# jlko/STOVE

Measured on AMD Instinct MI355X. Metric: frames/s (fwd+bwd) for 3-obj billiards 32x32 T=100, 1/2/4/8 GPU; ELBO delta vs ref, higher is better.
Workload: dtype f32 (encoder GEMMs: fp32 products as 3 sixteen-bit MFMAs on hi/lo-split operands -- half pieces forward, bf16 pieces backward -- fp32 accumulate)

## Files before the change

### include/stove_hip.h

```cpp
#ifndef STOVE_HIP_H
#define STOVE_HIP_H
#include <stddef.h>
#include <stdint.h>

#ifdef __cplusplus
extern "C" {
#endif

int stove_abi_version(void);
const char* stove_error_string(int code);

typedef struct StoveSpnTables {
  const int32_t* obj_scope;
  const int32_t* obj_leaf_slot;
  const float* obj_coef;
  const float* obj_wsum;
  const float* obj_wroot;
  const int32_t* bg_side;
  const float* bg_coef;
  const float* bg_wroot;
  const float* bg_dense;
} StoveSpnTables;

size_t stove_bg_dense_floats(void);
// ... 16 lines not shown

size_t stove_bgspn_saved_floats(int n);
int stove_bgspn_fwd(const StoveSpnTables* t, const float* inputs, const float* marg, float* ell, float* out,
                    int n, void* stream);
size_t stove_bgspn_bwd_ws_bytes(int n);
int stove_bgspn_bwd(const StoveSpnTables* t, const float* inputs, const float* marg, const float* ell, const float* out,
                    const float* dout, float* d_inputs, float* d_marg, StoveSpnTableGrads* g, void* ws, int n,
                    void* stream);

size_t stove_bgspn_saved_floats_d(int n, int n_pix);
int stove_bgspn_fwd_d(const StoveSpnTables* t, const float* inputs, const float* marg, float* ell, float* out, int n, int n_pix, void* stream);
size_t stove_bgspn_bwd_ws_bytes_d(int n, int n_pix);
int stove_bgspn_bwd_d(const StoveSpnTables* t, const float* inputs, const float* marg, const float* ell, const float* out, const float* dout,
                      float* d_inputs, float* d_marg, StoveSpnTableGrads* g, void* ws, int n, int n_pix, void* stream);

size_t stove_scene_saved_floats(int n_frames, int n_obj);
size_t stove_scene_fwd_floats(int n_frames, int n_obj, int with_grad);
int stove_scene_fwd(const StoveSpnTables* t, const float* frames, const float* z, int n_frames, int n_obj, int seq_frames,
                    int seq_stride, float overlap_beta, float* ll, float* parts, float* saved, void* stream);
size_t stove_scene_bwd_ws_bytes(int n_frames, int n_obj);
int stove_scene_bwd(const StoveSpnTables* t, const float* frames, const float* z, int n_frames, int n_obj, int seq_frames,
                    int seq_stride, float overlap_beta, const float* saved, const float* dll, float* dz, StoveSpnTableGrads* g,
                    void* ws, void* stream);
int stove_scene_bwd_overlap(const StoveSpnTables* t, const float* frames, const float* z, int n_frames, int n_obj, int seq_frames,
                    int seq_stride, float overlap_beta, const float* saved, const float* dll, float* dz, StoveSpnTableGrads* g,
                    void* ws, void* stream, void* param_stream);
size_t stove_objspn_saved_floats_any(int n, int R, int G, int S, int D, int Lmax);
size_t stove_objspn_bwd_ws_bytes_any(int n, int R, int G, int S, int D, int Lmax);
int stove_objspn_fwd_any(const float* inputs, const float* marg, const int* lscope, const float* coef, const float* wsum,
                         const float* wroot, float* saved, float* out, int n, int R, int G, int S, int D, int Lmax, void* stream);
int stove_objspn_bwd_any(const float* inputs, const float* marg, const int* lscope, const int* slot, const float* coef,
                         const float* wsum, const float* wroot, const float* saved, const float* dout, float* d_inputs,
                         float* d_marg, float* g_coef, float* g_wsum, float* g_wroot, void* ws, int n, int R, int G, int S, int D,
                         int Lmax, void* stream);
int stove_gauss_ll_fwd(const float* x, const float* marg, float* out, int n, int d, float mean, float scale, void* stream);
int stove_gauss_ll_bwd(const float* x, const float* marg, const float* dout, float* dx, float* dm, int n, int d, float mean, float scale,
                       void* stream);
size_t stove_scene_saved_floats_any(int n_frames, int n_obj, int n_pix, int with_grad);
size_t stove_scene_bwd_ws_bytes_any(int n_frames, int n_obj, int n_pix);
int stove_scene_fwd_any(const StoveSpnTables* t, const float* frames, const float* z, int n_frames, int n_obj, int seq_frames,
                        int seq_stride, int W, int H, int align_corners, float overlap_beta, float* ll, float* parts, float* saved,
                        void* stream, int with_grad);
int stove_scene_bwd_any(const StoveSpnTables* t, const float* frames, const float* z, int n_frames, int n_obj, int seq_frames,
                        int seq_stride, int W, int H, int align_corners, float overlap_beta, const float* saved, const float* dll,
                        float* dz, StoveSpnTableGrads* g, void* ws, void* stream, void* param_stream);
size_t stove_scene_saved_floats_ch(int n_frames, int n_obj, int channels, int W, int H, int R, int G, int S, int D, int Lmax, int with_grad);
size_t stove_scene_bwd_ws_bytes_ch(int n_frames, int n_obj, int channels, int W, int H, int R, int G, int S, int D, int Lmax);
int stove_scene_fwd_ch(const int32_t* lscope, const int32_t* slot, const float* coef, const float* wsum, const float* wroot, int R, int G, int S,
                       int D, int Lmax, const int32_t* bg_side, const float* bg_coef, const float* bg_wroot, size_t bg_coef_floats,
                       const float* frames, const float* z, int n_frames, int n_obj, int seq_frames, int seq_stride, int channels, int W, int H,
                       int pw, int ph, int align_corners, float overlap_beta, float* ll, float* parts, float* saved, void* stream, int with_grad);
int stove_scene_bwd_ch(const int32_t* lscope, const int32_t* slot, const float* coef, const float* wsum, const float* wroot, int R, int G, int S,
                       int D, int Lmax, const int32_t* bg_side, const float* bg_coef, const float* bg_wroot, size_t bg_coef_floats,
                       const float* frames, const float* z, int n_frames, int n_obj, int seq_frames, int seq_stride, int channels, int W, int H,
                       int pw, int ph, int align_corners, float overlap_beta, const float* saved, const float* dll, float* dz, float* g_coef,
                       float* g_wsum, float* g_wroot, float* g_bg_coef, float* g_bg_wroot, void* ws, void* stream, void* param_stream);
int stove_scene_fwd_from(const StoveSpnTables* t, const float* frames, const float* z, int n_frames, int n_obj, int seq_frames,
                         int seq_stride, float overlap_beta, float* ll, float* parts, float* saved, void* stream, void* fork_from,
                         int with_grad);
int stove_scene_bwd_from(const StoveSpnTables* t, const float* frames, const float* z, int n_frames, int n_obj, int seq_frames,
                         int seq_stride, float overlap_beta, const float* saved, const float* dll, float* dz,
                         StoveSpnTableGrads* g, void* ws, void* stream, void* param_stream, void* fork_from);

int stove_glimpse_mean(const float* x_color, const float* z, float* emb, int n_frames, int n_obj, int channels, void* stream);

int stove_objspn_mpe(const StoveSpnTables* t, const float* leaf_means, const float* inputs, float* xw, float* out,
                     int32_t* pick, int n, void* stream);

int stove_render_frames(const float* bg, const float* patches, int frames_per_patch, const float* z, float* out, int n_frames,
                        int n_obj, void* stream);

int stove_scene_glimpses(const float* frames, const float* z, int n_frames, int n_obj, float* tile,
                         float* patches, float* keep, void* stream);

size_t stove_gnn_param_floats(void);
size_t stove_gnn_grad_floats(void);
int stove_gnn_blocks(int B, int N);
int stove_gnn_fwd(const float* s_in, const float* params, float* result, float* pred, int B, int N, int sin_dim,
                  int lim_enc, int elu, void* stream);
size_t stove_gnn_bwd_ws_bytes(int B, int N);
int stove_gnn_bwd(const float* s_in, const float* params, const float* d_result, const float* d_pred, float* d_s_in,
                  float* g_params, void* ws, int B, int N, int sin_dim, int lim_enc, int elu, void* stream);

int stove_gnn_debug_stamps(const float* s_in, const float* params, const float* d_result, float* d_s_in, void* ws,
                           long long* stamps, int B, int N, int sin_dim, int lim_enc, int elu, void* stream);

size_t stove_dynloop_act_floats(int B, int Ts, int N);
int stove_dynloop_fwd(const float* z1, const float* zsup, const float* zsstd, const float* eps, const float* extra,
                      const float* params, float* z, float* zdyn, float* zdstd, float* mean, float* std_, float* pred,
                      float* act, int B, int Ts, int N, int sin_dim, int lim_enc, int elu, float pos_var, float vel_std, float lat_std,
                      void* stream);
size_t stove_dynloop_bwd_ws_bytes(int B, int N);
size_t stove_dynloop_bwd_ws_bytes_ts(int B, int Ts, int N);
int stove_dynloop_bwd(const float* z1, const float* zsup, const float* zsstd, const float* eps, const float* extra,
                      const float* params, const float* z, const float* act, const float* dz, const float* dzdyn,
                      const float* dmean, const float* dstd, const float* dpred, float* dz1, float* dzsup, float* dzsstd, float* dextra,
                      float* g_params, void* ws, int B, int Ts, int N, int sin_dim, int lim_enc, int elu, float pos_var,
                      float vel_std, float lat_std, void* stream);

int stove_dynloop_bwd_overlap(const float* z1, const float* zsup, const float* zsstd, const float* eps, const float* extra,
                              const float* params, const float* z, const float* act, const float* dz, const float* dzdyn,
                              const float* dmean, const float* dstd, const float* dpred, float* dz1, float* dzsup, float* dzsstd,
                              float* dextra, float* g_params, void* ws, int B, int Ts, int N, int sin_dim, int lim_enc, int elu,
                              float pos_var, float vel_std, float lat_std, void* stream, void* param_stream);


size_t stove_reward_head_param_floats(void);
size_t stove_reward_head_saved_floats(int items, int n_obj);
size_t stove_reward_head_bwd_ws_floats(int items);
int stove_reward_head_fwd(const float* pred, const float* params, float* reward, float* saved, int items, int n_obj, void* stream);
int stove_reward_head_bwd(const float* pred, const float* params, const float* reward, const float* saved, const float* d_reward, float* d_pred,
                          float* g_params, float* ws, int items, int n_obj, void* stream);

int stove_small_linear(const float* x, const float* W, const float* b, float* y, int rows, int in_dim, int out_dim, int w_transposed, void* stream);

int stove_rollout_fwd(const float* z_last, const float* extra, const float* params, float* z_pred, float* zstd, float* pred,
                      int B, int num, int A, int N, int sin_dim, int lim_enc, int elu, float pos_var, float vel_std,
                      float lat_std, void* stream);

size_t stove_gnn_param_floats_cl(int cl);
size_t stove_gnn_grad_floats_cl(int cl);
size_t stove_gnn_bwd_ws_bytes_cl(int cl, int B, int N);
int stove_gnn_fwd_cl(const float* s_in, const float* params, float* result, float* pred, int cl, int B, int N, int sin_dim,
                     int lim_enc, int elu, void* stream);
int stove_gnn_bwd_cl(const float* s_in, const float* params, const float* d_result, const float* d_pred, float* d_s_in,
                     float* g_params, void* ws, int cl, int B, int N, int sin_dim, int lim_enc, int elu, void* stream);
int stove_dynloop_fwd_cl(const float* z1, const float* zsup, const float* zsstd, const float* eps, const float* extra,
                         const float* params, float* z, float* zdyn, float* zdstd, float* mean, float* std_, float* pred,
                         int cl, int B, int Ts, int N, int sin_dim, int lim_enc, int elu, float pos_var, float vel_std, float lat_std,
                         void* stream);
int stove_dynloop_bwd_cl(const float* z1, const float* zsup, const float* zsstd, const float* eps, const float* extra,
                         const float* params, const float* z, const float* dz, const float* dzdyn, const float* dmean,
                         const float* dstd, const float* dpred, float* dz1, float* dzsup, float* dzsstd, float* dextra,
                         float* g_params, void* ws, int cl, int B, int Ts, int N, int sin_dim, int lim_enc, int elu, float pos_var,
                         float vel_std, float lat_std, void* stream);
int stove_rollout_fwd_cl(const float* z_last, const float* extra, const float* params, float* z_pred, float* zstd, float* pred,
                         int cl, int B, int num, int A, int N, int sin_dim, int lim_enc, int elu, float pos_var, float vel_std,
                         float lat_std, void* stream);

int stove_match_objects(const float* feat, long long* idx, float* perm, int B, int T, int N, int F, int mode, void* stream);

int stove_supair_state_fwd(const float* codes, const float* span_low, float* zc, float* pos, long long* idx, float* zfix,
                           unsigned char* hits, float* zl, float* sl, float* init6, int n, int T, int o, int skip, int fix,
                           int mode, void* stream);
int stove_supair_state_bwd(const float* zc, const long long* idx, const unsigned char* hits, const float* zfix, const float* g_zfix,
                           const float* g_zl, const float* g_sl, const float* g_init6, const float* span_low, float* gfix_ws,
                           float* g_codes, int n, int T, int o, int skip, void* stream);
int stove_supair_state_fwd2(const float* codes, const float* span_low, float* zc, float* pos, long long* idx, float* zfix,
                            unsigned char* hits, float* zl, float* sl, float* init, int init_ld, const float* lat_noise, int lat_dim,
                            int n, int T, int o, int skip, int fix, int mode, void* stream);
int stove_supair_state_bwd2(const float* zc, const long long* idx, const unsigned char* hits, const float* zfix, const float* g_zfix,
                            const float* g_zl, const float* g_sl, const float* g_init6, int init_ld, const float* span_low, float* gfix_ws,
                            float* g_codes, int n, int T, int o, int skip, void* stream);
int stove_zall_fwd(const float* zfix, const float* zs, float* zall, int n, int T, int o, int skip, void* stream);
int stove_zall_bwd(const float* zfix, const float* zs, const float* g_zall, const float* dz_in, float* g_zfix, float* g_zs, int n, int T, int o,
                   int skip, void* stream);
int stove_elbo_fwd(const float* zs, const float* mean, const float* std_, const float* zdyn, const float* lik, const float* trans_std16,
                   float* part_ws, float* out3, int n, int T, int o, int skip, void* stream);
int stove_elbo_bwd(const float* zs, const float* mean, const float* std_, const float* zdyn, const float* trans_std16, const float* g_out,
                   float* g_zs, float* g_mean, float* g_std, float* g_zdyn, float* g_lik, int n, int T, int o, int skip, void* stream);

void stove_debug_set_stamps(long long* device_buffer);

typedef struct StoveSpnArenaPlan {
  const int32_t* obj_mu;
  const int32_t* obj_rho;
  const int32_t* obj_sum;
  const int32_t* bg_mu;
  const int32_t* bg_rho;
  const int32_t* bg_gidx;
  int32_t obj_root, bg_root;
  float obj_vmin, obj_vmax, bg_vmin, bg_vmax;
} StoveSpnArenaPlan;
int stove_spn_bake(const float* arena, const StoveSpnArenaPlan* plan, float* obj_coef, float* obj_wsum, float* obj_wroot,
                   float* bg_coef, float* bg_wroot, void* stream);
int stove_spn_bake_bwd(const float* arena, const StoveSpnArenaPlan* plan, const StoveSpnTableGrads* g, float* grad_arena, void* stream);
int stove_arena_gather(const float* arena, const int32_t* src, float* image, int n, void* stream);
int stove_arena_scatter_add(const float* gimage, const int32_t* src, float* grad_arena, int n, void* stream);

int stove_sum_chunks(const float* parts, float* out, size_t n, int chunks, void* stream);

int stove_set_fork_stream(int device, void* stream, int restore_default);
int stove_set_overlap(int on);
int stove_set_tile_lds(int mode);
void* stove_event_list_begin(void);
int stove_event_list_end(void* list);
int stove_event_list_destroy(void* list);
int stove_stream_after(void* to, void* from);
int stove_capture_begin(void* stream);
int stove_capture_end(void* stream, void** graph_out, int* n_nodes);
int stove_graph_instantiate(void* graph, void** exec_out);
int stove_graph_launch(void* exec, void* stream);
int stove_graph_destroy(void* exec);

int stove_noise_normal(float* out, size_t n, unsigned long long* state, void* stream);

int stove_bw_transform(const float* x, float* out, int n_frames, int channels, int pixels, void* stream);
int stove_bw_transform_u8(const unsigned char* x, float* out, int n_frames, int channels, int pixels, void* stream);

size_t stove_colsum_ws_floats(int rows, int cols);
int stove_colsum(const float* a, float* out, float* ws, int rows, int cols, void* stream);
size_t stove_small_tn_ws_floats(int rows, int M, int N);
int stove_small_tn(const float* a, const float* b, float* out, float* ws, int rows, int M, int N, void* stream);
int stove_colsum2(const float* a, float* out, float* out2, int accumulate, float* ws, int rows, int cols, void* stream);

size_t stove_flat_adam_ws_bytes(int nseg);
int stove_flat_adam(float* params, const float* grads, float* exp_avg, float* exp_avg_sq, float* max_exp_avg_sq, size_t numel,
                    const int* seg_of4, const unsigned char* seg_trainable, float* seg_steps, int nseg, void* ws, float* grad_norm_out,
                    const float* hyper_dev, float lr, float beta1, float beta2, float eps, float max_norm, int clip, void* stream);

size_t stove_gemm_bf16_ws_floats(int M, int N, int splitk);
int stove_gemm_bf16(const float* A, const float* B, const float* bias, const float* add, float* C, int M, int N, int K, int lda, int ldb, int ldc,
                    int a_kmajor, int b_kmajor, int nsplit, int splitk, int tile, float* ws, void* stream);

int stove_lstm_cell_fwd(const float* gx, const float* gh, const float* c_prev, float* c, float* h, int n, int H, int fast, void* stream);
int stove_lstm_cell_bwd(const float* gx, const float* gh, const float* c_prev, const float* c, const float* dh,
                        const float* dc_in, float* dg, float* dc_out, float* dgx_sum, const float* dg_more, int n_more, int n, int H,
                        int fast, void* stream);
int stove_enc_head_fwd(const float* h, const float* W1, const float* b1, const float* W2, const float* b2, float* h1, float* codes, int rows,
                       int H, int HID, int OUT, int frames, int fc1_split, void* stream);
size_t stove_enc_head_bwd_ws_floats(int rows, int HID);
int stove_enc_head_bwd(const float* dcodes, const float* h1, const float* h, const float* W1, const float* W2, float* gh, float* gW1,
                       float* gb1, float* gW2, float* gb2, int accumulate, float* ws, int rows, int H, int HID, int OUT, int frames, void* stream);

void stove_profile_enable(int on);
size_t stove_profile_report(char* buf, size_t cap);

int stove_fill_words(void* p, uint32_t value, size_t n_words, void* stream);

int stove_selftest_wave_sum(const float* in, float* out, int n_waves, void* stream);

#ifdef __cplusplus
}
#endif
#endif
```

### stove_amd/_lib.py

```python
import ctypes
import os
from ctypes import POINTER, Structure, c_char_p, c_float, c_int, c_size_t, c_void_p

import torch

_HERE = os.path.dirname(os.path.abspath(__file__))
from . import settings as _settings

LIB_PATH = _settings.LIB_OVERRIDE or os.path.join(_HERE, 'libstove_hip.so')
_lib = None
ABI_VERSION = 7

class SpnTables(Structure):
    _fields_ = [('obj_scope', c_void_p), ('obj_leaf_slot', c_void_p), ('obj_coef', c_void_p),
                ('obj_wsum', c_void_p), ('obj_wroot', c_void_p),
                ('bg_side', c_void_p), ('bg_coef', c_void_p), ('bg_wroot', c_void_p), ('bg_dense', c_void_p)]


class SpnTableGrads(Structure):
    _fields_ = [('obj_coef', c_void_p), ('obj_wsum', c_void_p), ('obj_wroot', c_void_p),
                ('bg_coef', c_void_p), ('bg_wroot', c_void_p)]


class SpnArenaPlan(Structure):
    _fields_ = [('obj_mu', c_void_p), ('obj_rho', c_void_p), ('obj_sum', c_void_p),
                ('bg_mu', c_void_p), ('bg_rho', c_void_p), ('bg_gidx', c_void_p),
                ('obj_root', c_int), ('bg_root', c_int),
                ('obj_vmin', c_float), ('obj_vmax', c_float), ('bg_vmin', c_float), ('bg_vmax', c_float)]


def _declare(lib):
    P, I, F, S = c_void_p, c_int, c_float, c_size_t
    T, G = POINTER(SpnTables), POINTER(SpnTableGrads)
    A = POINTER(SpnArenaPlan)
    sig = {
        'stove_abi_version': (I, []),
        'stove_error_string': (c_char_p, [I]),
        'stove_selftest_wave_sum': (I, [P, P, I, P]),
        'stove_objspn_tile_floats': (S, [I]),
        'stove_objspn_fwd': (I, [T, P, P, P, P, I, P]),
        'stove_objspn_bwd_ws_bytes': (S, [I]),
        'stove_objspn_bwd': (I, [T, P, P, P, P, P, P, G, P, I, P]),
        'stove_bgspn_saved_floats': (S, [I]),
        'stove_bgspn_fwd': (I, [T, P, P, P, P, I, P]),
        'stove_bgspn_bwd_ws_bytes': (S, [I]),
        'stove_bgspn_bwd': (I, [T, P, P, P, P, P, P, P, G, P, I, P]),
        'stove_scene_saved_floats': (S, [I, I]),
        'stove_scene_fwd': (I, [T, P, P, I, I, I, I, F, P, P, P, P]),
        'stove_scene_fwd_from': (I, [T, P, P, I, I, I, I, F, P, P, P, P, P, I]),
        'stove_scene_fwd_floats': (S, [I, I, I]),
        'stove_scene_bwd_from': (I, [T, P, P, I, I, I, I, F, P, P, P, G, P, P, P, P]),
        'stove_scene_bwd_ws_bytes': (S, [I, I]),
        'stove_scene_bwd': (I, [T, P, P, I, I, I, I, F, P, P, P, G, P, P]),
        'stove_scene_bwd_overlap': (I, [T, P, P, I, I, I, I, F, P, P, P, G, P, P, P]),
        'stove_gauss_ll_fwd': (I, [P, P, P, I, I, F, F, P]),
        'stove_gauss_ll_bwd': (I, [P, P, P, P, P, I, I, F, F, P]),
        'stove_objspn_saved_floats_any': (S, [I, I, I, I, I, I]),
        'stove_objspn_bwd_ws_bytes_any': (S, [I, I, I, I, I, I]),
        'stove_objspn_fwd_any': (I, [P, P, P, P, P, P, P, P, I, I, I, I, I, I, P]),
        'stove_objspn_bwd_any': (I, [P, P, P, P, P, P, P, P, P, P, P, P, P, P, P, I, I, I, I, I, I, P]),
        'stove_scene_saved_floats_any': (S, [I, I, I, I]),
        'stove_scene_bwd_ws_bytes_any': (S, [I, I, I]),
        'stove_scene_fwd_any': (I, [T, P, P, I, I, I, I, I, I, I, F, P, P, P, P, I]),
        'stove_scene_bwd_any': (I, [T, P, P, I, I, I, I, I, I, I, F, P, P, P, G, P, P, P]),
        'stove_scene_saved_floats_ch': (S, [I] * 11),
        'stove_scene_bwd_ws_bytes_ch': (S, [I] * 10),
        'stove_scene_fwd_ch': (I, [P] * 5 + [I] * 5 + [P, P, P, S, P, P] + [I] * 10 + [F, P, P, P, P, I]),
        'stove_scene_bwd_ch': (I, [P] * 5 + [I] * 5 + [P, P, P, S, P, P] + [I] * 10 + [F] + [P] * 11),
        'stove_scene_glimpses': (I, [P, P, I, I, P, P, P, P]),
        'stove_gnn_param_floats': (S, []),
        'stove_gnn_grad_floats': (S, []),
        'stove_gnn_blocks': (I, [I, I]),
        'stove_gnn_fwd': (I, [P, P, P, P, I, I, I, I, I, P]),
        'stove_gnn_bwd_ws_bytes': (S, [I, I]),
        'stove_gnn_bwd': (I, [P, P, P, P, P, P, P, I, I, I, I, I, P]),
        'stove_dynloop_act_floats': (S, [I, I, I]),
        'stove_dynloop_fwd': (I, [P] * 13 + [I] * 6 + [F] * 3 + [P]),
        'stove_dynloop_bwd_ws_bytes': (S, [I, I]),
        'stove_dynloop_bwd': (I, [P] * 19 + [I] * 6 + [F] * 3 + [P]),
        'stove_dynloop_bwd_overlap': (I, [P] * 19 + [I] * 6 + [F] * 3 + [P, P]),
        'stove_rollout_fwd': (I, [P] * 6 + [I] * 7 + [F] * 3 + [P]),
        'stove_gnn_param_floats_cl': (S, [I]),
        'stove_gnn_grad_floats_cl': (S, [I]),
        'stove_gnn_bwd_ws_bytes_cl': (S, [I, I, I]),
        'stove_gnn_fwd_cl': (I, [P, P, P, P, I, I, I, I, I, I, P]),
        'stove_gnn_bwd_cl': (I, [P, P, P, P, P, P, P, I, I, I, I, I, I, P]),
        'stove_dynloop_fwd_cl': (I, [P] * 12 + [I] * 7 + [F] * 3 + [P]),
        'stove_dynloop_bwd_cl': (I, [P] * 18 + [I] * 7 + [F] * 3 + [P]),
        'stove_rollout_fwd_cl': (I, [P] * 6 + [I] * 8 + [F] * 3 + [P]),
        'stove_match_objects': (I, [P, P, P, I, I, I, I, I, P]),
        'stove_profile_enable': (None, [I]),
        'stove_lstm_cell_fwd': (I, [P, P, P, P, P, I, I, I, P]),
        'stove_lstm_cell_bwd': (I, [P] * 10 + [I, I, I, I, P]),
        'stove_gnn_debug_stamps': (I, [P, P, P, P, P, P, I, I, I, I, I, P]),
        'stove_profile_report': (S, [c_char_p, S]),
        'stove_spn_bake': (I, [P, A, P, P, P, P, P, P]),
        'stove_spn_bake_bwd': (I, [P, A, G, P, P]),
        'stove_debug_set_stamps': (None, [P]),
        'stove_glimpse_mean': (I, [P, P, P, I, I, I, P]),
        'stove_objspn_mpe': (I, [T, P, P, P, P, P, I, P]),
        'stove_render_frames': (I, [P, P, I, P, P, I, I, P]),
        'stove_enc_head_fwd': (I, [P, P, P, P, P, P, P, I, I, I, I, I, I, P]),
        'stove_enc_head_bwd_ws_floats': (S, [I, I]),
        'stove_enc_head_bwd': (I, [P, P, P, P, P, P, P, P, P, P, I, P, I, I, I, I, I, P]),
        'stove_colsum2': (I, [P, P, P, I, P, I, I, P]),
        'stove_small_tn_ws_floats': (S, [I, I, I]),
        'stove_small_tn': (I, [P, P, P, P, I, I, I, P]),
        'stove_dynloop_bwd_ws_bytes_ts': (S, [I, I, I]),
        'stove_bw_transform': (I, [P, P, I, I, I, P]),
        'stove_bw_transform_u8': (I, [P, P, I, I, I, P]),
        'stove_stream_after': (I, [P, P]),
        'stove_small_linear': (I, [P, P, P, P, I, I, I, I, P]),
        'stove_reward_head_param_floats': (S, []),
        'stove_reward_head_saved_floats': (S, [I, I]),
        'stove_reward_head_bwd_ws_floats': (S, [I]),
        'stove_reward_head_fwd': (I, [P, P, P, P, I, I, P]),
        'stove_reward_head_bwd': (I, [P] * 8 + [I, I, P]),
        'stove_set_fork_stream': (I, [I, P, I]),
        'stove_noise_normal': (I, [P, S, P, P]),
        'stove_bgspn_saved_floats_d': (S, [I, I]),
        'stove_bgspn_fwd_d': (I, [T, P, P, P, P, I, I, P]),
        'stove_bgspn_bwd_ws_bytes_d': (S, [I, I]),
        'stove_bgspn_bwd_d': (I, [T, P, P, P, P, P, P, P, G, P, I, I, P]),
        'stove_set_overlap': (I, [I]),
        'stove_set_tile_lds': (I, [I]),
        'stove_event_list_begin': (P, []),
        'stove_event_list_end': (I, [P]),
        'stove_event_list_destroy': (I, [P]),
        'stove_fill_words': (I, [P, ctypes.c_uint32, S, P]),
        'stove_capture_begin': (I, [P]),
        'stove_capture_end': (I, [P, POINTER(c_void_p), POINTER(c_int)]),
        'stove_graph_instantiate': (I, [P, POINTER(c_void_p)]),
        'stove_graph_launch': (I, [P, P]),
        'stove_graph_destroy': (I, [P]),
        'stove_colsum_ws_floats': (S, [I, I]),
        'stove_colsum': (I, [P, P, P, I, I, P]),
        'stove_sum_chunks': (I, [P, P, S, I, P]),
        'stove_flat_adam_ws_bytes': (S, [I]),
        'stove_gemm_bf16_ws_floats': (S, [I, I, I]),
        'stove_gemm_bf16': (I, [P, P, P, P, P] + [I] * 11 + [P, P]),
        'stove_flat_adam': (I, [P] * 5 + [S, P, P, P, I, P, P, P, F, F, F, F, F, I, P]),
        'stove_supair_state_fwd': (I, [P] * 10 + [I] * 6 + [P]),
        'stove_supair_state_bwd': (I, [P] * 11 + [I] * 4 + [P]),
        'stove_bg_dense_floats': (S, []),
        'stove_bg_dense': (I, [P, P, P, P]),
        'stove_supair_state_fwd2': (I, [P] * 10 + [I, P, I] + [I] * 6 + [P]),
        'stove_supair_state_bwd2': (I, [P] * 8 + [I] + [P] * 3 + [I] * 4 + [P]),
        'stove_zall_fwd': (I, [P, P, P, I, I, I, I, P]),
        'stove_zall_bwd': (I, [P, P, P, P, P, P, I, I, I, I, P]),
        'stove_elbo_fwd': (I, [P] * 8 + [I] * 4 + [P]),
        'stove_elbo_bwd': (I, [P] * 11 + [I] * 4 + [P]),
        'stove_arena_gather': (I, [P, P, P, I, P]),
        'stove_arena_scatter_add': (I, [P, P, P, I, P]),
    }
    for name, (res, args) in sig.items():
        fn = getattr(lib, name)
        fn.restype = res
        fn.argtypes = args


def load():
    global _lib
    if _lib is None:
        if not os.path.exists(LIB_PATH):
            raise RuntimeError(
                f'{LIB_PATH} is missing: build it with `python -m stove_amd.build` '
                '(hipcc --offload-arch=gfx950). stove_amd has no CPU fallback.')
        lib = ctypes.CDLL(LIB_PATH)
        _declare(lib)
        if lib.stove_abi_version() != ABI_VERSION:
            raise RuntimeError(f'{LIB_PATH} has ABI version {lib.stove_abi_version()}, this binding needs {ABI_VERSION}: '
                               'rebuild it with `python -m stove_amd.build --force`')
        from . import settings
        lib.stove_set_overlap(1 if settings.OVERLAP else 0)
        if settings.LIB_OVERRIDE:
            import sys
            sys.stderr.write('[stove_amd] STOVE_LIB: loaded %s\n' % LIB_PATH)
        _lib = lib
    return _lib


def check(code, what):
    if code != 0:
        msg = load().stove_error_string(code)
        raise RuntimeError(f'{what} failed: hipError {code} ({msg.decode() if msg else "?"})')


def ptr(t):
    if t is None:
        return None
    if not t.is_cuda:
        raise RuntimeError('stove_amd HIP ops need tensors on a GPU (cuda:N); there is no CPU path')
    if not t.is_contiguous():
        raise RuntimeError('stove_amd HIP ops need contiguous tensors')
    return t.data_ptr()


_FORCED_STREAM = None


def stream():
    return _FORCED_STREAM if _FORCED_STREAM is not None else torch.cuda.current_stream().cuda_stream


def force_stream(handle):
    global _FORCED_STREAM
    prev, _FORCED_STREAM = _FORCED_STREAM, handle
    return prev


def profile_report(wall=False):
    lib = load()
    buf = ctypes.create_string_buffer(1 << 16)
    lib.stove_profile_report(buf, len(buf))
    out = {}
    for line in buf.value.decode().splitlines():
        name, ms, cnt, cover = line.split('\t')
        name = name.strip('()').split('<')[0].split('::')[-1]
        tot, c, w = out.get(name, (0.0, 0, 0.0))
        out[name] = (tot + float(ms), c + int(cnt), w + float(cover))
    return out if wall else {k: v[:2] for k, v in out.items()}
```

### stove_amd/arena.py

```python
import ctypes

import torch
import torch.distributed as dist

from . import _lib, ops
from . import settings as _settings


def _unique_params(module):
    seen, out = set(), []
    for name, p in module.named_parameters():
        if id(p) not in seen:
            seen.add(id(p))
            out.append((name, p))
    return out


class ParamArena:
    ALIGN = 4

    def __init__(self, model, world_size=None):
        named = _unique_params(model)
        if not named:
            raise ValueError('model has no parameters')
        dev, dt = named[0][1].device, named[0][1].dtype
        for n, p in named:
            if p.device != dev or p.dtype != dt:
                raise ValueError('parameter %s is %s/%s, arena is %s/%s' % (n, p.device, p.dtype, dev, dt))
        self.model = model
        self.names = [n for n, _ in named]
        self.params = [p for _, p in named]
        self.offset, off = {}, 0
        for p in self.params:
            self.offset[id(p)] = off
            off += (p.numel() + self.ALIGN - 1) // self.ALIGN * self.ALIGN
        self.numel = off
        self.data = torch.zeros(off, dtype=dt, device=dev)
        self.grad = torch.zeros(off, dtype=dt, device=dev)
        with torch.no_grad():
            for p in self.params:
                o, n = self.offset[id(p)], p.numel()
                self.data[o:o + n].copy_(p.data.reshape(-1))
                p.data = self.data[o:o + n].view(p.shape)
        self._on_gpu_params = dev.type == 'cuda' and dt == torch.float32
        self._bind_grads()
        if world_size is None:
            world_size = dist.get_world_size() if dist.is_initialized() else 1
        self.world_size = world_size
        self._spn = self._gnn = None
        sup = model if hasattr(model, 'obj_spn') else getattr(model, 'sup', None)
        dyn = model if hasattr(model, 'param_image') else getattr(model, 'dyn', None)
        self._on_gpu = dev.type == 'cuda' and dt == torch.float32
        if sup is not None and hasattr(sup, 'obj_spn'):
            self._plan_spn(sup)
            sup._arena = self
        if dyn is not None and hasattr(dyn, 'param_image'):
            self._plan_gnn(dyn)
            dyn._arena = self

    def _bind_grads(self):
        for p in self.params:
            if not p.requires_grad:
                p.grad = None
                if self._on_gpu_params:
                    ops.register_grad_view(p, None)
                continue
            o, n = self.offset[id(p)], p.numel()
            g = p.grad
            if g is None or g.data_ptr() != self.grad.data_ptr() + self.grad.element_size() * o:
                p.grad = self.grad[o:o + n].view(p.shape)
            if self._on_gpu_params:
                ops.register_grad_view(p, p.grad)

    def view_of(self, p, flat=None):
        o = self.offset[id(p)]
        return (self.data if flat is None else flat)[o:o + p.numel()].view(p.shape)

    def check(self):
        es = self.data.element_size()
        for p in (self.params[0], self.params[-1]):
            o = self.offset[id(p)]
            if p.data_ptr() != self.data.data_ptr() + es * o:
                raise RuntimeError('ParamArena: parameter storage was rebound (model.to()/type() after the arena '
                                   'was built?) -- build a new ParamArena')
            if p.requires_grad and (p.grad is None or p.grad.data_ptr() != self.grad.data_ptr() + es * o):
                raise RuntimeError('ParamArena: gradient views were detached -- use arena.zero_grad() instead of '
                                   'optimizer.zero_grad() / p.grad = None')

    def zero_grad(self):
        self.grad.zero_()
        self._bind_grads()

    def drop_prefetched(self):
        self._pre = None

    zero = zero_grad

    def pack(self):
        return self.grad

    def all_reduce(self, force=False):
        if self.world_size <= 1 and not force:
            return
        dist.all_reduce(self.grad, op=dist.ReduceOp.SUM)
        if self.world_size > 1:
            self.grad.div_(self.world_size)

    def sync(self, src=0):
        if self.world_size > 1:
            dist.broadcast(self.data, src)
        self.drop_prefetched()

    def clip_grad_norm_(self, max_norm):
        total = torch.linalg.vector_norm(self.grad)
        self.grad.mul_(torch.clamp(max_norm / (total + 1e-6), max=1.0))
        return total

    def _plan_spn(self, sup):
        obj, bg = sup.obj_spn, sup.bg_spn
        if obj._kind != 'obj' or bg._kind != 'bg' or bg.num_dims != 1024:
            return
        dev = self.data.device
        off = self.offset
        oleaves, osums = list(obj.vector_list[0]), list(obj.vector_list[2])
        lo, so = obj._plan_cpu['leaf_order'].tolist(), obj._plan_cpu['sum_order'].tolist()
        bleaves = list(bg.vector_list[0])

        def i32(v):
            return torch.tensor(v, dtype=torch.int32, device=dev)
        t = {'obj_mu': i32([off[id(oleaves[i].means)] for i in lo]),
             'obj_rho': i32([off[id(oleaves[i].sigma_params)] for i in lo]),
             'obj_sum': i32([off[id(osums[i].params)] for i in so]),
             'bg_mu': i32([off[id(v.means)] for v in bleaves]),
             'bg_rho': i32([off[id(v.sigma_params)] for v in bleaves]),
             'bg_gidx': bg._plan_cpu['gidx'].to(torch.int32).reshape(-1).to(dev)}
        plan = _lib.SpnArenaPlan()
        for k, v in t.items():
            setattr(plan, k, v.data_ptr())
        plan.obj_root = off[id(obj.output_vector.params)]
        plan.bg_root = off[id(bg.output_vector.params)]
        plan.obj_vmin, plan.obj_vmax = obj.args.gauss_min_sigma, obj.args.gauss_max_sigma
        plan.bg_vmin, plan.bg_vmax = bg.args.gauss_min_sigma, bg.args.gauss_max_sigma
        opl, bpl = obj._plan(dev), bg._plan(dev)
        self._spn = {'plan': plan, 'keep': t, 'ints': (opl['scope'], opl['leaf_slot'], bpl['side']),
                     'params': list(obj.parameters()) + list(bg.parameters())}

    @property
    def has_spn(self):
        return self._on_gpu and self._spn is not None

    def prefetch_images(self, cores=(0,)):
        if not self._on_gpu or not _settings.OVERLAP:
            return
        dev = self.data.device
        main, side = torch.cuda.current_stream(dev), ops._side_stream(dev, 'pre')
        side.wait_stream(main)
        with torch.cuda.stream(side):
            pre = {}
            if self.has_spn:
                pre['spn'] = self._bake_spn()
            if self.has_gnn:
                for k in cores:
                    pre[('gnn', k)] = self._gather_gnn(k)
            ev = torch.cuda.Event()
            ev.record(side)
        self._pre = (pre, ev, side)

    def _take(self, key):
        pre = getattr(self, '_pre', None)
        if pre is None or key not in pre[0]:
            return None
        out = pre[0].pop(key)
        torch.cuda.current_stream(self.data.device).wait_event(pre[1])
        for t in (out if isinstance(out, tuple) else (out,)):
            t.record_stream(torch.cuda.current_stream(self.data.device))
        return out

    def spn_tables(self):
        self.check()
        bufs = self._take('spn')
        if bufs is None:
            bufs = self._bake_spn()
        oc, ow, orr, bc, bw, dense = bufs
        scope, slot, side = self._spn['ints']
        return ((oc.view(24, 25, 10, 3), ow.view(12, 100, 10), orr.view(6, 100), scope, slot),
                (bc.view(3, 1024, 6, 3), bw.view(3, 36), side, dense))

    def _bake_spn(self):
        lib = _lib.load()
        dev = self.data.device
        with torch.cuda.device(dev):
            buf = torch.empty(18000 + 12000 + 600 + 55296 + 108, dtype=torch.float32, device=dev)
            oc, ow, orr, bc, bw = torch.split(buf, [18000, 12000, 600, 55296, 108])
            _lib.check(lib.stove_spn_bake(self.data.data_ptr(), ctypes.byref(self._spn['plan']), oc.data_ptr(), ow.data_ptr(),
                                          orr.data_ptr(), bc.data_ptr(), bw.data_ptr(), _lib.stream()), 'stove_spn_bake')
            dense = torch.empty(lib.stove_bg_dense_floats(), dtype=torch.float32, device=dev)
            _lib.check(lib.stove_bg_dense(self._spn['ints'][2].data_ptr(), bc.data_ptr(), dense.data_ptr(), _lib.stream()), 'stove_bg_dense')
        return oc, ow, orr, bc, bw, dense

    def spn_sink(self, grads):
        req = [p.requires_grad for p in self._spn['params']]
        if not any(req):
            return
        if not all(req):
            raise RuntimeError('ParamArena: the SPN parameters must be frozen or trainable together')
        self.check()
        lib = _lib.load()
        g = _lib.SpnTableGrads()
        g.obj_coef, g.obj_wsum, g.obj_wroot, g.bg_coef, g.bg_wroot = [x.data_ptr() for x in grads]
        with torch.cuda.device(self.data.device):
            _lib.check(lib.stove_spn_bake_bwd(self.data.data_ptr(), ctypes.byref(self._spn['plan']), ctypes.byref(g),
                                              self.grad.data_ptr(), _lib.stream()), 'stove_spn_bake_bwd')

    def _plan_gnn(self, dyn):
        dev = self.data.device

        def index_of(p):
            return (self.offset[id(p)] + torch.arange(p.numel(), dtype=torch.float64)).view(p.shape)
        self._gnn = {}
        for k in range(3):
            w, v, wt = dyn.param_image(k, leaf=index_of, pad_value=-1.0)
            if dyn.c.cl == 32:
                pf, pt = ops.gnn_pack_perms(torch.device('cpu'))
                image = torch.cat([w, wt, v, w[pf], wt[pt]])
            else:
                image = torch.cat([w, wt, v])
            self._gnn[k] = (image.to(torch.int32).to(dev), torch.cat([w, v]).to(torch.int32).to(dev))
        self._gnn_params = [p for n, p in dyn.named_parameters()
                            if n.split('.')[0] in ('state_enc', 'self_cores', 'rel_cores', 'att_net', 'affector', 'out')]

    @property
    def has_gnn(self):
        return self._on_gpu and self._gnn is not None

    def gnn_image(self, core_idx=0):
        self.check()
        img = self._take(('gnn', core_idx))
        return img if img is not None else self._gather_gnn(core_idx)

    def _gather_gnn(self, core_idx):
        lib = _lib.load()
        src = self._gnn[core_idx][0]
        with torch.cuda.device(self.data.device):
            img = torch.empty(src.numel(), dtype=torch.float32, device=self.data.device)
            _lib.check(lib.stove_arena_gather(self.data.data_ptr(), src.data_ptr(), img.data_ptr(), src.numel(), _lib.stream()),
                       'stove_arena_gather')
        return img

    def gnn_sink(self, g, core_idx=0):
        req = [p.requires_grad for p in self._gnn_params]
        if not any(req):
            return
        if not all(req):
            raise RuntimeError('ParamArena: the GNN core parameters must be frozen or trainable together')
        self.check()
        lib = _lib.load()
        src = self._gnn[core_idx][1]
        with torch.cuda.device(self.data.device):
            _lib.check(lib.stove_arena_scatter_add(g.data_ptr(), src.data_ptr(), self.grad.data_ptr(), src.numel(), _lib.stream()),
                       'stove_arena_scatter_add')
```

### stove_amd/csrc/arena.hip

```cpp
#include "common.h"

namespace stove {

struct SpnArenaPlan {
  const int* obj_mu;
  const int* obj_rho;
  const int* obj_sum;
  const int* bg_mu;
  const int* bg_rho;
  const int* bg_gidx;
  int obj_root, bg_root;
  float obj_vmin, obj_vmax, bg_vmin, bg_vmax;
};

__device__ __forceinline__ void leaf_coef(float mu, float rho, float vmin, float vmax, float* abc) {
  const float v = vmin + (vmax - vmin) * (1.0f / (1.0f + expf(-rho)));
  const float iv = 1.0f / v;
  abc[0] = -0.5f * iv;
  abc[1] = mu * iv;
  abc[2] = -0.5f * mu * mu * iv - 0.5f * logf(6.283185307179586f * v);
}
__device__ __forceinline__ void leaf_coef_bwd(float mu, float rho, float vmin, float vmax, const float* g, float* dmu, float* drho) {
  const float s = 1.0f / (1.0f + expf(-rho));
  const float v = vmin + (vmax - vmin) * s;
  const float iv = 1.0f / v;
  *dmu = g[1] * iv - g[2] * mu * iv;
  const float dv = g[0] * 0.5f * iv * iv - g[1] * mu * iv * iv + g[2] * (0.5f * mu * mu * iv * iv - 0.5f * iv);
  *drho = dv * (vmax - vmin) * s * (1.0f - s);
}

constexpr int kAObjLeaves = 24, kAObjS = 25, kAObjG = 10, kAObjSums = 12, kAObjK = 10;
constexpr int kABgR = 3, kABgPix = 1024, kABgG = 6;
constexpr int kAObjCoef = kAObjLeaves * kAObjS * kAObjG;
constexpr int kABgCoef = kABgR * kABgPix * kABgG;
constexpr int kASoftBlocks = (kAObjSums * kAObjK + 2 + 3) / 4;

__device__ __forceinline__ void softmax_col(const float* __restrict__ p, float* __restrict__ w, int n, int ld) {
  const int lane = lane_id();
  float m = -3.0e38f;
  for (int k = lane; k < n; k += 64) m = fmaxf(m, p[k * ld]);
  for (int o = 32; o > 0; o >>= 1) m = fmaxf(m, __shfl_xor(m, o));
  float s = 0.0f;
  for (int k = lane; k < n; k += 64) s += expf(p[k * ld] - m);
  s = wave_sum(s);
  const float inv = 1.0f / s;
  for (int k = lane; k < n; k += 64) w[k * ld] = expf(p[k * ld] - m) * inv;
}
__device__ __forceinline__ void softmax_col_bwd(const float* __restrict__ p, const float* __restrict__ g, float* __restrict__ dp, int n, int ld) {
  const int lane = lane_id();
  float m = -3.0e38f;
  for (int k = lane; k < n; k += 64) m = fmaxf(m, p[k * ld]);
  for (int o = 32; o > 0; o >>= 1) m = fmaxf(m, __shfl_xor(m, o));
  float s = 0.0f, d = 0.0f;
  for (int k = lane; k < n; k += 64) {
    const float e = expf(p[k * ld] - m);
    s += e;
    d = fmaf(e, g[k * ld], d);
  }
  s = wave_sum(s);
  d = wave_sum(d);
  const float inv = 1.0f / s, dot = d * inv;
  for (int k = lane; k < n; k += 64) dp[k * ld] += expf(p[k * ld] - m) * inv * (g[k * ld] - dot);
}

__global__ __launch_bounds__(256) void spn_bake_k(const float* __restrict__ arena, SpnArenaPlan pl, float* __restrict__ obj_coef,
                                                  float* __restrict__ obj_wsum, float* __restrict__ obj_wroot,
                                                  float* __restrict__ bg_coef, float* __restrict__ bg_wroot, int n_elem_blocks) {
  if ((int)blockIdx.x < n_elem_blocks) {
    const int t = blockIdx.x * 256 + threadIdx.x;
    if (t < kAObjCoef) {
      const int q = t / (kAObjS * kAObjG), rem = t % (kAObjS * kAObjG);
      leaf_coef(arena[pl.obj_mu[q] + rem], arena[pl.obj_rho[q] + rem], pl.obj_vmin, pl.obj_vmax, obj_coef + (size_t)t * 3);
    } else if (t < kAObjCoef + kABgCoef) {
      const int u = t - kAObjCoef;
      const int rp = u / kABgG, g = u % kABgG;
      const int gi = pl.bg_gidx[rp];
      const int leaf = gi >> 9, row = gi & 511;
      leaf_coef(arena[pl.bg_mu[leaf] + row * kABgG + g], arena[pl.bg_rho[leaf] + row * kABgG + g], pl.bg_vmin, pl.bg_vmax,
                bg_coef + (size_t)u * 3);
    }
    return;
  }
  const int col = ((int)blockIdx.x - n_elem_blocks) * 4 + wave_id();
  if (col < kAObjSums * kAObjK + 2) {
    if (col < kAObjSums * kAObjK) {
      const int node = col / kAObjK, s = col % kAObjK;
      softmax_col(arena + pl.obj_sum[node] + s, obj_wsum + (size_t)node * 100 * kAObjK + s, 100, kAObjK);
    } else if (col == kAObjSums * kAObjK) {
      softmax_col(arena + pl.obj_root, obj_wroot, 600, 1);
    } else {
      softmax_col(arena + pl.bg_root, bg_wroot, kABgR * kABgG * kABgG, 1);
    }
  }
}

__global__ __launch_bounds__(256) void spn_bake_bwd_k(const float* __restrict__ arena, SpnArenaPlan pl,
                                                      const float* __restrict__ g_obj_coef, const float* __restrict__ g_obj_wsum,
                                                      const float* __restrict__ g_obj_wroot, const float* __restrict__ g_bg_coef,
                                                      const float* __restrict__ g_bg_wroot, float* __restrict__ garena,
                                                      int n_elem_blocks) {
  if ((int)blockIdx.x < n_elem_blocks) {
    const int t = blockIdx.x * 256 + threadIdx.x;
    if (t < kAObjCoef) {
      const int q = t / (kAObjS * kAObjG), rem = t % (kAObjS * kAObjG);
      float dmu, drho;
      leaf_coef_bwd(arena[pl.obj_mu[q] + rem], arena[pl.obj_rho[q] + rem], pl.obj_vmin, pl.obj_vmax, g_obj_coef + (size_t)t * 3, &dmu, &drho);
      garena[pl.obj_mu[q] + rem] += dmu;
      garena[pl.obj_rho[q] + rem] += drho;
    } else if (t < kAObjCoef + kABgCoef) {
      const int u = t - kAObjCoef;
      const int rp = u / kABgG, g = u % kABgG;
      const int gi = pl.bg_gidx[rp];
      const int leaf = gi >> 9, row = gi & 511;
      const int om = pl.bg_mu[leaf] + row * kABgG + g, orh = pl.bg_rho[leaf] + row * kABgG + g;
      float dmu, drho;
      leaf_coef_bwd(arena[om], arena[orh], pl.bg_vmin, pl.bg_vmax, g_bg_coef + (size_t)u * 3, &dmu, &drho);
      garena[om] += dmu;
      garena[orh] += drho;
    }
    return;
  }
  const int col = ((int)blockIdx.x - n_elem_blocks) * 4 + wave_id();
  if (col < kAObjSums * kAObjK + 2) {
    if (col < kAObjSums * kAObjK) {
      const int node = col / kAObjK, s = col % kAObjK;
      softmax_col_bwd(arena + pl.obj_sum[node] + s, g_obj_wsum + (size_t)node * 100 * kAObjK + s, garena + pl.obj_sum[node] + s, 100, kAObjK);
    } else if (col == kAObjSums * kAObjK) {
      softmax_col_bwd(arena + pl.obj_root, g_obj_wroot, garena + pl.obj_root, 600, 1);
    } else {
      softmax_col_bwd(arena + pl.bg_root, g_bg_wroot, garena + pl.bg_root, kABgR * kABgG * kABgG, 1);
    }
  }
}

__global__ void arena_gather_k(const float* __restrict__ arena, const int* __restrict__ src, float* __restrict__ image, int n) {
  const int i = blockIdx.x * blockDim.x + threadIdx.x;
  if (i < n) image[i] = src[i] >= 0 ? arena[src[i]] : 0.0f;
}
__global__ void arena_scatter_add_k(const float* __restrict__ gimage, const int* __restrict__ src, float* __restrict__ garena, int n) {
  const int i = blockIdx.x * blockDim.x + threadIdx.x;
  if (i < n && src[i] >= 0) garena[src[i]] += gimage[i];
}

}

namespace stove {

struct AdamHyper {
  float lr, b1, b2, eps, max_norm;
};
constexpr int ADAM_SCAN_BLOCKS = 256;

__global__ __launch_bounds__(256) void grad_scan_k(const float* __restrict__ g, const int* __restrict__ seg_of4, int* __restrict__ flags,
                                                   float* __restrict__ part, int n4) {
  float acc = 0.0f;
  for (int i = blockIdx.x * 256 + threadIdx.x; i < n4; i += ADAM_SCAN_BLOCKS * 256) {
    const float4 v = reinterpret_cast<const float4*>(g)[i];
    acc += v.x * v.x + v.y * v.y + v.z * v.z + v.w * v.w;
    if (v.x != 0.0f || v.y != 0.0f || v.z != 0.0f || v.w != 0.0f) flags[seg_of4[i]] = 1;
  }
  __shared__ float red[4];
  acc = wave_sum(acc);
  if ((threadIdx.x & 63) == 0) red[threadIdx.x >> 6] = acc;
  __syncthreads();
  if (threadIdx.x == 0) part[blockIdx.x] = (red[0] + red[1]) + (red[2] + red[3]);
}

__global__ __launch_bounds__(256) void flat_adam_k(float* __restrict__ p, const float* __restrict__ g, float* __restrict__ m, float* __restrict__ v,
                                                   float* __restrict__ vmax, const int* __restrict__ seg_of4,
                                                   const unsigned char* __restrict__ trainable, const float* __restrict__ steps,
                                                   const int* __restrict__ flags, const float* __restrict__ part, float* __restrict__ norm_out,
                                                   const float* __restrict__ hyper_dev, AdamHyper k, int clip, int n4) {
  if (hyper_dev != nullptr) {
    k.lr = hyper_dev[0]; k.b1 = hyper_dev[1]; k.b2 = hyper_dev[2]; k.eps = hyper_dev[3]; k.max_norm = hyper_dev[4];
  }
  __shared__ float s_norm;
  if (threadIdx.x < 64) {
    float t = (part[threadIdx.x] + part[threadIdx.x + 64]) + (part[threadIdx.x + 128] + part[threadIdx.x + 192]);
    t = wave_sum(t);
    if (threadIdx.x == 0) {
      s_norm = sqrtf(t);
      if (blockIdx.x == 0 && norm_out != nullptr) norm_out[0] = s_norm;
    }
  }
  __syncthreads();
  const int i = blockIdx.x * 256 + threadIdx.x;
  if (i >= n4) return;
  const int seg = seg_of4[i];
  if (trainable[seg] == 0 || flags[seg] == 0) return;
  const float coef = clip ? fminf(1.0f, k.max_norm / (s_norm + 1e-6f)) : 1.0f;
  const double t = (double)steps[seg] + 1.0;
  const float bc1 = (float)(1.0 - pow((double)k.b1, t));
  const float sqrt_bc2 = (float)sqrt(1.0 - pow((double)k.b2, t));
  const float4 g4 = reinterpret_cast<const float4*>(g)[i];
  float4 p4 = reinterpret_cast<float4*>(p)[i], m4 = reinterpret_cast<float4*>(m)[i], v4 = reinterpret_cast<float4*>(v)[i];
  float4 x4 = vmax != nullptr ? reinterpret_cast<float4*>(vmax)[i] : v4;
  const float step = k.lr / bc1;
#define STOVE_ADAM1(c)                                           \
  {                                                              \
    const float gg = g4.c * coef;                                \
    m4.c = m4.c + (1.0f - k.b1) * (gg - m4.c);                   \
    v4.c = k.b2 * v4.c + (1.0f - k.b2) * gg * gg;                \
    x4.c = vmax != nullptr ? fmaxf(x4.c, v4.c) : v4.c;           \
    p4.c -= step * m4.c / (sqrtf(x4.c) / sqrt_bc2 + k.eps);      \
  }
  STOVE_ADAM1(x) STOVE_ADAM1(y) STOVE_ADAM1(z) STOVE_ADAM1(w)
#undef STOVE_ADAM1
  reinterpret_cast<float4*>(p)[i] = p4;
  reinterpret_cast<float4*>(m)[i] = m4;
  reinterpret_cast<float4*>(v)[i] = v4;
  if (vmax != nullptr) reinterpret_cast<float4*>(vmax)[i] = x4;
}

__global__ void adam_tick_k(const unsigned char* __restrict__ trainable, float* __restrict__ steps, int* __restrict__ flags, int nseg, int sticky) {
  const int s = blockIdx.x * blockDim.x + threadIdx.x;
  if (s >= nseg) return;
  if (trainable[s] != 0 && flags[s] != 0) steps[s] += 1.0f;
  if (!sticky) flags[s] = 0;
}

__global__ void sum_chunks4_k(const float* __restrict__ part, float* __restrict__ out, int n4, int chunks, int accumulate = 0,
                              const float* __restrict__ bias4 = nullptr, int cols4 = 0, const float* __restrict__ add4 = nullptr) {
  const int i = blockIdx.x * blockDim.x + threadIdx.x;
  if (i >= n4) return;
  float4 a = reinterpret_cast<const float4*>(part)[i];
  if (add4 != nullptr) {
    const float4 b = reinterpret_cast<const float4*>(add4)[i];
    a.x += b.x; a.y += b.y; a.z += b.z; a.w += b.w;
  }
  if (bias4 != nullptr) {
    const float4 b = reinterpret_cast<const float4*>(bias4)[i % cols4];
    a.x += b.x; a.y += b.y; a.z += b.z; a.w += b.w;
  }
  if (accumulate) {
    const float4 o = reinterpret_cast<const float4*>(out)[i];
    a.x += o.x; a.y += o.y; a.z += o.z; a.w += o.w;
  }
  for (int c = 1; c < chunks; ++c) {
    const float4 b = reinterpret_cast<const float4*>(part)[(size_t)c * n4 + i];
    a.x += b.x; a.y += b.y; a.z += b.z; a.w += b.w;
  }
  reinterpret_cast<float4*>(out)[i] = a;
}

__global__ __launch_bounds__(256) void sum_chunks4_par_k(const float* __restrict__ part, float* __restrict__ out, int n4, int chunks, int accumulate) {
  __shared__ float4 red[4][64];
  const int e = threadIdx.x & 63, q = threadIdx.x >> 6;
  const int i = blockIdx.x * 64 + e;
  float4 a = {0.0f, 0.0f, 0.0f, 0.0f};
  if (i < n4)
    for (int c = q; c < chunks; c += 4) {
      const float4 b = reinterpret_cast<const float4*>(part)[(size_t)c * n4 + i];
      a.x += b.x; a.y += b.y; a.z += b.z; a.w += b.w;
    }
  red[q][e] = a;
  __syncthreads();
  if (q == 0 && i < n4) {
    float4 t = red[0][e];
#pragma unroll
    for (int k = 1; k < 4; ++k) {
      t.x += red[k][e].x; t.y += red[k][e].y; t.z += red[k][e].z; t.w += red[k][e].w;
    }
    if (accumulate) {
      const float4 o = reinterpret_cast<const float4*>(out)[i];
      t.x += o.x; t.y += o.y; t.z += o.z; t.w += o.w;
    }
    reinterpret_cast<float4*>(out)[i] = t;
  }
}

__global__ __launch_bounds__(256) void small_tn_part_k(const float* __restrict__ a, const float* __restrict__ b, float* __restrict__ part,
                                                        int rows, int M, int N, int rows_per_chunk) {
  const int t = threadIdx.x;
  if (t >= M * N) return;
  const int m = t / N, n = t % N;
  const int r0 = blockIdx.x * rows_per_chunk;
  const int r1 = r0 + rows_per_chunk < rows ? r0 + rows_per_chunk : rows;
  float s0 = 0.0f, s1 = 0.0f;
  int r = r0;
  for (; r + 1 < r1; r += 2) {
    s0 = fmaf(a[(size_t)r * M + m], b[(size_t)r * N + n], s0);
    s1 = fmaf(a[(size_t)(r + 1) * M + m], b[(size_t)(r + 1) * N + n], s1);
  }
  if (r < r1) s0 = fmaf(a[(size_t)r * M + m], b[(size_t)r * N + n], s0);
  part[(size_t)blockIdx.x * M * N + t] = s0 + s1;
}

__global__ __launch_bounds__(256) void colsum_part_k(const float* __restrict__ a, float* __restrict__ part, int rows, int cols4, int rows_per_chunk) {
  const int c4 = blockIdx.y * 256 + threadIdx.x;
  if (c4 >= cols4) return;
  const int r0 = blockIdx.x * rows_per_chunk;
  const int r1 = r0 + rows_per_chunk < rows ? r0 + rows_per_chunk : rows;
  float4 s0 = {0.0f, 0.0f, 0.0f, 0.0f}, s1 = s0;
  int r = r0;
  for (; r + 1 < r1; r += 2) {
    const float4 u = reinterpret_cast<const float4*>(a)[(size_t)r * cols4 + c4];
    const float4 v = reinterpret_cast<const float4*>(a)[(size_t)(r + 1) * cols4 + c4];
    s0.x += u.x; s0.y += u.y; s0.z += u.z; s0.w += u.w;
    s1.x += v.x; s1.y += v.y; s1.z += v.z; s1.w += v.w;
  }
  if (r < r1) {
    const float4 u = reinterpret_cast<const float4*>(a)[(size_t)r * cols4 + c4];
    s0.x += u.x; s0.y += u.y; s0.z += u.z; s0.w += u.w;
  }
  s0.x += s1.x; s0.y += s1.y; s0.z += s1.z; s0.w += s1.w;
  reinterpret_cast<float4*>(part)[(size_t)blockIdx.x * cols4 + c4] = s0;
}

__global__ __launch_bounds__(256) void colsum_narrow_part_k(const float* __restrict__ a, float* __restrict__ part, int rows, int cols, int cpad,
                                                            int rows_per_chunk) {
  __shared__ float red[256];
  const int c = threadIdx.x % cpad, rr = threadIdx.x / cpad, nslot = 256 / cpad;
  const int r0 = blockIdx.x * rows_per_chunk;
  const int r1 = r0 + rows_per_chunk < rows ? r0 + rows_per_chunk : rows;
  float s = 0.0f;
  if (c < cols)
    for (int r = r0 + rr; r < r1; r += nslot) s += a[(size_t)r * cols + c];
  red[threadIdx.x] = s;
  __syncthreads();
  if (rr == 0 && c < cols) {
    float t = 0.0f;
    for (int q = 0; q < nslot; ++q) t += red[q * cpad + c];
    part[(size_t)blockIdx.x * cols + c] = t;
  }
}

__global__ void bw_transform_k(const float* __restrict__ x, float* __restrict__ out, int N, int C, int P4) {
  const int i = blockIdx.x * blockDim.x + threadIdx.x;
  if (i >= N * P4) return;
  const int n = i / P4, p = i % P4;
  float4 s = reinterpret_cast<const float4*>(x)[((size_t)n * C) * P4 + p];
  for (int c = 1; c < C; ++c) {
    const float4 v = reinterpret_cast<const float4*>(x)[((size_t)n * C + c) * P4 + p];
    s.x += v.x; s.y += v.y; s.z += v.z; s.w += v.w;
  }
  s.x = fminf(fmaxf(s.x, 0.0f), 1.0f);
  s.y = fminf(fmaxf(s.y, 0.0f), 1.0f);
  s.z = fminf(fmaxf(s.z, 0.0f), 1.0f);
  s.w = fminf(fmaxf(s.w, 0.0f), 1.0f);
  reinterpret_cast<float4*>(out)[i] = s;
}

__global__ void bw_transform_u8_k(const unsigned char* __restrict__ x, float* __restrict__ out, int N, int C, int P4) {
  const int i = blockIdx.x * blockDim.x + threadIdx.x;
  if (i >= N * P4) return;
  const int n = i / P4, p = i % P4;
  float4 s = make_float4(0.f, 0.f, 0.f, 0.f);
  for (int c = 0; c < C; ++c) {
    const uchar4 v = reinterpret_cast<const uchar4*>(x)[((size_t)n * C + c) * P4 + p];
    const float4 f = make_float4((float)v.x / 255.0f, (float)v.y / 255.0f, (float)v.z / 255.0f, (float)v.w / 255.0f);
    if (c == 0) s = f;
    else { s.x += f.x; s.y += f.y; s.z += f.z; s.w += f.w; }
  }
  s.x = fminf(fmaxf(s.x, 0.0f), 1.0f);
  s.y = fminf(fmaxf(s.y, 0.0f), 1.0f);
  s.z = fminf(fmaxf(s.z, 0.0f), 1.0f);
  s.w = fminf(fmaxf(s.w, 0.0f), 1.0f);
  reinterpret_cast<float4*>(out)[i] = s;
}

}
```

### stove_amd/csrc/capi.hip

```cpp
#include "../../include/stove_hip.h"
#include <algorithm>

#include "common.h"
#include <string.h>
#include <stdlib.h>
#include <math.h>
#include <atomic>
#include <type_traits>
#include "validate.h"
static_assert(stove_validate::kStoveInvalidValue == (int)hipErrorInvalidValue, "validate.h returns hipErrorInvalidValue");
#define STOVE_VALIDATE(expr)                      \
  do {                                            \
    const int v__ = stove_validate::expr;         \
    if (v__) return v__;                          \
  } while (0)
#include "spn_obj.hip"
#include "spn_obj_generic.hip"
#include "spn_bg.hip"
#include "spn_bg_generic.hip"
#include "scene.hip"
#include "scene_fused.hip"
#include "scene_colour.hip"
#include "gnn.hip"
#include "match.hip"
// ... 931 lines not shown
#define STOVE_ROLL_LAUNCH(ELU_)                         \
  do {                                                  \
    if (N == 3) STOVE_ROLL_LAUNCH_N(4, ELU_, 3);        \
    else if (N <= 4) STOVE_ROLL_LAUNCH_N(4, ELU_, 0);   \
    else STOVE_ROLL_LAUNCH_N(6, ELU_, 0);               \
  } while (0)
    if (elu) STOVE_ROLL_LAUNCH(true);
    else STOVE_ROLL_LAUNCH(false);
#undef STOVE_ROLL_LAUNCH
#undef STOVE_ROLL_LAUNCH_N
    STOVE_LAUNCH_CHECK();
    return 0;
  }
  int rc = gnn_lds_attr((const void*)rollout_fwd_k);
  if (rc) return rc;
  STOVE_LAUNCH(rollout_fwd_k, dim3(stove_gnn_blocks(B, N)), dim3(256), kGnnLdsFloats * sizeof(float), (hipStream_t)stream,
                     z_last, extra, params, z_pred, zstd, pred, B, num, A < 1 ? 1 : A, N, gnn_group_for(B, N), sin_dim, lim_enc, elu, kc);
  STOVE_LAUNCH_CHECK();
  return 0;
}

size_t stove_gnn_param_floats_cl(int cl) { return cl == 16 ? GC<16>::kParams : (cl == 64 ? GC<64>::kParams : 0); }
size_t stove_gnn_grad_floats_cl(int cl) { return cl == 16 ? GC<16>::kGrads : (cl == 64 ? GC<64>::kGrads : 0); }
size_t stove_gnn_bwd_ws_bytes_cl(int cl, int B, int N) {
  if (B < 1 || N < 1 || N > 6) return 0;
  if (cl == 16) return (size_t)cl_blocks<16>(B, N) * GC<16>::kGrads * sizeof(float);
  if (cl == 64) return (size_t)cl_blocks<64>(B, N) * GC<64>::kGrads * sizeof(float);
  return 0;
}

int stove_gnn_fwd_cl(const float* s_in, const float* params, float* result, float* pred, int cl, int B, int N, int sin_dim,
                     int lim_enc, int elu, void* stream) {
  STOVE_VALIDATE(gnn_fwd_cl(s_in, params, result, cl, B, N, sin_dim));
  if (B == 0) return 0;
  return with_cl(cl, [&](auto w) {
    constexpr int CL = decltype(w)::value;
    int rc = cl_lds_attr<CL>((const void*)gnn_cl_step_fwd_k<CL>);
    if (rc) return rc;
    STOVE_LAUNCH(gnn_cl_step_fwd_k<CL>, dim3(cl_blocks<CL>(B, N)), dim3(256), GC<CL>::kLdsFloats * sizeof(float), (hipStream_t)stream,
                 s_in, params, result, pred, B, N, cl_group_for<CL>(B, N), sin_dim, lim_enc, elu);
    STOVE_LAUNCH_CHECK();
    return 0;
  });
}

int stove_gnn_bwd_cl(const float* s_in, const float* params, const float* d_result, const float* d_pred, float* d_s_in,
                     float* g_params, void* ws, int cl, int B, int N, int sin_dim, int lim_enc, int elu, void* stream) {
  hipStream_t st = (hipStream_t)stream;
  STOVE_VALIDATE(gnn_bwd_cl(s_in, params, d_result, d_s_in, g_params, ws, cl, B, N, sin_dim));
  return with_cl(cl, [&](auto w) {
    constexpr int CL = decltype(w)::value;
    if (B == 0) return (int)hipMemsetAsync(g_params, 0, GC<CL>::kGrads * sizeof(float), st);
    int rc = cl_lds_attr<CL>((const void*)gnn_cl_step_bwd_k<CL>);
    if (rc) return rc;
    const int nb = cl_blocks<CL>(B, N);
    STOVE_LAUNCH(gnn_cl_step_bwd_k<CL>, dim3(nb), dim3(256), GC<CL>::kLdsFloats * sizeof(float), st, s_in, params, d_result, d_pred,
                 d_s_in, (float*)ws, B, N, cl_group_for<CL>(B, N), sin_dim, lim_enc, elu);
    STOVE_LAUNCH_CHECK();
    STOVE_LAUNCH(reduce_chunks_k, dim3((GC<CL>::kGrads + 31) / 32), dim3(256), 0, st, (const float*)ws, g_params, GC<CL>::kGrads, nb, 0);
    STOVE_LAUNCH_CHECK();
    return 0;
  });
}

int stove_dynloop_fwd_cl(const float* z1, const float* zsup, const float* zsstd, const float* eps, const float* extra,
                         const float* params, float* z, float* zdyn, float* zdstd, float* mean, float* std_, float* pred,
                         int cl, int B, int Ts, int N, int sin_dim, int lim_enc, int elu, float pos_var, float vel_std, float lat_std,
                         void* stream) {
  STOVE_VALIDATE(dynloop_fwd_cl(z1, zsup, zsstd, eps, extra, params, z, zdyn, zdstd, mean, std_, cl, B, Ts, N, sin_dim));
  if (B == 0 || Ts == 0) return 0;
  LoopConst kc{pos_var, vel_std, lat_std};
  return with_cl(cl, [&](auto w) {
    constexpr int CL = decltype(w)::value;
    int rc = cl_lds_attr<CL>((const void*)gnn_cl_loop_fwd_k<CL>);
    if (rc) return rc;
    STOVE_LAUNCH(gnn_cl_loop_fwd_k<CL>, dim3(cl_blocks<CL>(B, N)), dim3(256), GC<CL>::kLdsFloats * sizeof(float), (hipStream_t)stream,
                 z1, zsup, zsstd, eps, extra, params, z, zdyn, zdstd, mean, std_, pred, B, Ts, N, cl_group_for<CL>(B, N), sin_dim, lim_enc,
                 elu, kc);
    STOVE_LAUNCH_CHECK();
    return 0;
  });
}

int stove_dynloop_bwd_cl(const float* z1, const float* zsup, const float* zsstd, const float* eps, const float* extra,
                         const float* params, const float* z, const float* dz, const float* dzdyn, const float* dmean,
                         const float* dstd, const float* dpred, float* dz1, float* dzsup, float* dzsstd, float* dextra,
                         float* g_params, void* ws, int cl, int B, int Ts, int N, int sin_dim, int lim_enc, int elu, float pos_var,
                         float vel_std, float lat_std, void* stream) {
  hipStream_t st = (hipStream_t)stream;
  STOVE_VALIDATE(dynloop_bwd_cl(z1, zsup, zsstd, eps, extra, params, z, dz1, dzsup, dzsstd, dextra, g_params, ws, cl, B, Ts, N, sin_dim));
  LoopConst kc{pos_var, vel_std, lat_std};
  return with_cl(cl, [&](auto w) {
    constexpr int CL = decltype(w)::value;
    if (B == 0 || Ts == 0) return (int)hipMemsetAsync(g_params, 0, GC<CL>::kGrads * sizeof(float), st);
    int rc = cl_lds_attr<CL>((const void*)gnn_cl_loop_bwd_k<CL>);
    if (rc) return rc;
    const int nb = cl_blocks<CL>(B, N);
    STOVE_LAUNCH(gnn_cl_loop_bwd_k<CL>, dim3(nb), dim3(256), GC<CL>::kLdsFloats * sizeof(float), st, z1, zsup, zsstd, eps, extra, params, z,
                 dz, dzdyn, dmean, dstd, dpred, dz1, dzsup, dzsstd, dextra, (float*)ws, B, Ts, N, cl_group_for<CL>(B, N), sin_dim, lim_enc,
                 elu, kc);
    STOVE_LAUNCH_CHECK();
    STOVE_LAUNCH(reduce_chunks_k, dim3((GC<CL>::kGrads + 31) / 32), dim3(256), 0, st, (const float*)ws, g_params, GC<CL>::kGrads, nb, 0);
    STOVE_LAUNCH_CHECK();
    return 0;
  });
}

int stove_rollout_fwd_cl(const float* z_last, const float* extra, const float* params, float* z_pred, float* zstd, float* pred,
                         int cl, int B, int num, int A, int N, int sin_dim, int lim_enc, int elu, float pos_var, float vel_std,
                         float lat_std, void* stream) {
  STOVE_VALIDATE(rollout_fwd_cl(z_last, extra, params, z_pred, cl, B, num, A, N, sin_dim));
  if (B == 0 || num == 0) return 0;
  LoopConst kc{pos_var, vel_std, lat_std};
  return with_cl(cl, [&](auto w) {
    constexpr int CL = decltype(w)::value;
    int rc = cl_lds_attr<CL>((const void*)gnn_cl_rollout_k<CL>);
    if (rc) return rc;
    STOVE_LAUNCH(gnn_cl_rollout_k<CL>, dim3(cl_blocks<CL>(B, N)), dim3(256), GC<CL>::kLdsFloats * sizeof(float), (hipStream_t)stream,
                 z_last, extra, params, z_pred, zstd, pred, B, num, A < 1 ? 1 : A, N, cl_group_for<CL>(B, N), sin_dim, lim_enc, elu, kc);
    STOVE_LAUNCH_CHECK();
    return 0;
  });
}

static SpnArenaPlan arena_plan(const StoveSpnArenaPlan* p) {
  SpnArenaPlan q;
  q.obj_mu = p->obj_mu; q.obj_rho = p->obj_rho; q.obj_sum = p->obj_sum;
  q.bg_mu = p->bg_mu; q.bg_rho = p->bg_rho; q.bg_gidx = p->bg_gidx;
  q.obj_root = p->obj_root; q.bg_root = p->bg_root;
  q.obj_vmin = p->obj_vmin; q.obj_vmax = p->obj_vmax; q.bg_vmin = p->bg_vmin; q.bg_vmax = p->bg_vmax;
  return q;
}

int stove_spn_bake(const float* arena, const StoveSpnArenaPlan* plan, float* obj_coef, float* obj_wsum, float* obj_wroot,
                   float* bg_coef, float* bg_wroot, void* stream) {
  const int nb = (kAObjCoef + kABgCoef + 255) / 256;
  STOVE_LAUNCH(spn_bake_k, dim3(nb + kASoftBlocks), dim3(256), 0, (hipStream_t)stream, arena, arena_plan(plan), obj_coef, obj_wsum, obj_wroot,
               bg_coef, bg_wroot, nb);
  STOVE_LAUNCH_CHECK();
  return 0;
}

int stove_spn_bake_bwd(const float* arena, const StoveSpnArenaPlan* plan, const StoveSpnTableGrads* g, float* grad_arena, void* stream) {
  const int nb = (kAObjCoef + kABgCoef + 255) / 256;
  STOVE_LAUNCH(spn_bake_bwd_k, dim3(nb + kASoftBlocks), dim3(256), 0, (hipStream_t)stream, arena, arena_plan(plan), (const float*)g->obj_coef,
               (const float*)g->obj_wsum, (const float*)g->obj_wroot, (const float*)g->bg_coef, (const float*)g->bg_wroot, grad_arena, nb);
  STOVE_LAUNCH_CHECK();
  return 0;
}

int stove_arena_gather(const float* arena, const int32_t* src, float* image, int n, void* stream) {
  if (n == 0) return 0;
  STOVE_LAUNCH(arena_gather_k, dim3((n + 255) / 256), dim3(256), 0, (hipStream_t)stream, arena, src, image, n);
  STOVE_LAUNCH_CHECK();
  return 0;
}

int stove_arena_scatter_add(const float* gimage, const int32_t* src, float* grad_arena, int n, void* stream) {
  if (n == 0) return 0;
  STOVE_LAUNCH(arena_scatter_add_k, dim3((n + 255) / 256), dim3(256), 0, (hipStream_t)stream, gimage, src, grad_arena, n);
  STOVE_LAUNCH_CHECK();
  return 0;
}

int stove_sum_chunks(const float* parts, float* out, size_t n, int chunks, void* stream) {
  if (n == 0) return 0;
  if (n % 4 != 0 || chunks < 1) return (int)hipErrorInvalidValue;
  const int n4 = (int)(n / 4);
  STOVE_LAUNCH(sum_chunks4_k, dim3((n4 + 255) / 256), dim3(256), 0, (hipStream_t)stream, parts, out, n4, chunks, 0);
  STOVE_LAUNCH_CHECK();
  return 0;
}

size_t stove_gemm_bf16_ws_floats(int M, int N, int splitk) { return splitk > 1 ? (size_t)splitk * M * N : 0; }

int stove_gemm_bf16(const float* A, const float* B, const float* bias, const float* add, float* C, int M, int N, int K, int lda,
                    int ldb, int ldc, int a_kmajor, int b_kmajor, int nsplit, int splitk, int tile, float* ws, void* stream) {
  hipStream_t st = (hipStream_t)stream;
  STOVE_VALIDATE(gemm(A, B, C, M, N, K, lda, ldb, ldc, a_kmajor, b_kmajor, nsplit, splitk, ws));
  if (M == 0 || N == 0) return 0;
  if (K <= 0 || splitk < 1 || nsplit < 1 || nsplit > 3 || tile < 0 || (tile > 3 && (tile < 11 || tile > 15))) return (int)hipErrorInvalidValue;
  if (tile == 11 && !a_kmajor && !b_kmajor && nsplit == 2) return gemm_launch<false, false, 2, 256, 128, 1>(A, B, bias, add, C, M, N, K, lda, ldb, ldc, 1, st);
  if (tile == 12 && !a_kmajor && !b_kmajor && nsplit == 2) return gemm_launch<false, false, 2, 256, 128, 2>(A, B, bias, add, C, M, N, K, lda, ldb, ldc, 1, st);
  if (tile == 13 && !a_kmajor && !b_kmajor && nsplit == 2) return gemm_launch<false, false, 2, 256, 256, 1, false, 64, 128>(A, B, bias, add, C, M, N, K, lda, ldb, ldc, 1, st);
  if (tile == 14 && !a_kmajor && !b_kmajor && nsplit == 2) return gemm_launch<false, false, 2, 256, 256, 2, false, 64, 128>(A, B, bias, add, C, M, N, K, lda, ldb, ldc, 1, st);
  if (tile == 15 && !a_kmajor && !b_kmajor && nsplit == 2) return gemm_launch<false, false, 2, 256, 256, 3, false, 64, 128>(A, B, bias, add, C, M, N, K, lda, ldb, ldc, 1, st);
  if (tile > 3) tile = 1;
  auto odd = [](const void* p, int ld, int extent) { return ((uintptr_t)p & 15) != 0 || (ld & 3) != 0 || (extent & 3) != 0; };
  const int scalar_bits = (odd(A, lda, a_kmajor ? M : K) ? 1 : 0) | (odd(B, ldb, b_kmajor ? N : K) ? 2 : 0) |
                          ((odd(C, ldc, N) || (bias != nullptr && ((uintptr_t)bias & 15)) || (add != nullptr && ((uintptr_t)add & 15))) ? 4 : 0);
  const bool acc_c = splitk > 1 && add != nullptr && add == C;
  if (acc_c) add = nullptr;
  const float* sum_add = (splitk > 1 && splitk < 16 && add != nullptr && (((uintptr_t)add & 15) == 0)) ? add : nullptr;
  if (sum_add != nullptr) add = nullptr;
  const float* sum_bias = splitk > 1 ? bias : nullptr;
  if (splitk > 1 && splitk < 16) bias = nullptr;
  if (splitk > 1 && (ws == nullptr || bias != nullptr || add != nullptr || ldc != N || (scalar_bits & 4))) return (int)hipErrorInvalidValue;
  if (scalar_bits & 2) return (int)hipErrorInvalidValue;
  float* out = splitk > 1 ? ws : C;
  const int ldo = splitk > 1 ? N : ldc;
  if (tile == 0) tile = 1;
  int rc;
  if (nsplit == 3) {
    if (a_kmajor || b_kmajor || scalar_bits) return (int)hipErrorInvalidValue;
    rc = tile == 3 ? gemm_launch<false, false, 2, 256, 256, 0, false, 64, 128, true>(A, B, bias, add, out, M, N, K, lda, ldb, ldo, splitk, st, scalar_bits)
       : tile == 1 ? gemm_launch<false, false, 2, 256, 128, 0, false, 64, 64, true>(A, B, bias, add, out, M, N, K, lda, ldb, ldo, splitk, st, scalar_bits)
                   : gemm_launch<false, false, 2, 128, 128, 0, false, 64, 64, true>(A, B, bias, add, out, M, N, K, lda, ldb, ldo, splitk, st, scalar_bits);
  } else if (scalar_bits & 1) {
    if (!b_kmajor) return (int)hipErrorInvalidValue;
    if (a_kmajor) rc = nsplit == 2 ? gemm_launch<true, true, 2, 128, 128, 0, true>(A, B, bias, add, out, M, N, K, lda, ldb, ldo, splitk, st, scalar_bits)
                                   : gemm_launch<true, true, 1, 128, 128, 0, true>(A, B, bias, add, out, M, N, K, lda, ldb, ldo, splitk, st, scalar_bits);
    else rc = nsplit == 2 ? gemm_launch<false, true, 2, 128, 128, 0, true>(A, B, bias, add, out, M, N, K, lda, ldb, ldo, splitk, st, scalar_bits)
                          : gemm_launch<false, true, 1, 128, 128, 0, true>(A, B, bias, add, out, M, N, K, lda, ldb, ldo, splitk, st, scalar_bits);
  } else {
#define STOVE_GEMM_TILE(AK, BK_, NS)                                                                                \
  rc = tile == 3 ? gemm_launch<AK, BK_, NS, 256, 256, 0, false, 64, 128>(A, B, bias, add, out, M, N, K, lda, ldb, ldo, splitk, st, scalar_bits)           \
     : tile == 1 ? gemm_launch<AK, BK_, NS, 256, 128>(A, B, bias, add, out, M, N, K, lda, ldb, ldo, splitk, st, scalar_bits)           \
                 : gemm_launch<AK, BK_, NS, 128, 128>(A, B, bias, add, out, M, N, K, lda, ldb, ldo, splitk, st, scalar_bits)
#define STOVE_GEMM_CASE(AK, BK_)             \
  do {                                       \
    if (nsplit == 2) {                       \
      STOVE_GEMM_TILE(AK, BK_, 2);           \
    } else {                                 \
      STOVE_GEMM_TILE(AK, BK_, 1);           \
    }                                        \
  } while (0)
  if (!a_kmajor && !b_kmajor) STOVE_GEMM_CASE(false, false);
  else if (!a_kmajor && b_kmajor) STOVE_GEMM_CASE(false, true);
  else if (a_kmajor && b_kmajor) STOVE_GEMM_CASE(true, true);
  else STOVE_GEMM_CASE(true, false);
  }
#undef STOVE_GEMM_CASE
#undef STOVE_GEMM_TILE
  if (rc) return rc;
  if (splitk > 1) {
    const int n4 = (int)((size_t)M * N / 4);
    if (splitk >= 16)
      STOVE_LAUNCH(sum_chunks4_par_k, dim3((n4 + 63) / 64), dim3(256), 0, st, (const float*)ws, C, n4, splitk, acc_c ? 1 : 0);
    else
      STOVE_LAUNCH(sum_chunks4_k, dim3((n4 + 255) / 256), dim3(256), 0, st, (const float*)ws, C, n4, splitk, acc_c ? 1 : 0, sum_bias, N / 4, sum_add);
    STOVE_LAUNCH_CHECK();
  }
  return 0;
}

size_t stove_reward_head_param_floats(void) { return (size_t)kRhParams; }
size_t stove_reward_head_saved_floats(int items, int n_obj) { return (size_t)items * ((size_t)n_obj * 32 + 32 + 16 + 8); }
static int reward_head_blocks(int items) {
  const int b = (items + kRhWaves - 1) / kRhWaves;
  return b < 1 ? 1 : (b > 256 ? 256 : b);
}
size_t stove_reward_head_bwd_ws_floats(int items) { return (size_t)reward_head_blocks(items) * kRhWaves * kRhParams; }

int stove_reward_head_fwd(const float* pred, const float* params, float* reward, float* saved, int items, int n_obj, void* stream) {
  if (items == 0) return 0;
  if (n_obj < 1 || pred == nullptr || params == nullptr || reward == nullptr || saved == nullptr) return (int)hipErrorInvalidValue;
  float* H0 = saved;
  float* Q = H0 + (size_t)items * n_obj * 32;
  float* A1 = Q + (size_t)items * 32;
  float* A2 = A1 + (size_t)items * 16;
  STOVE_LAUNCH(reward_head_fwd_k, dim3(reward_head_blocks(items)), dim3(64 * kRhWaves), 0, (hipStream_t)stream, pred, params, reward, H0, Q, A1, A2,
               items, n_obj);
  STOVE_LAUNCH_CHECK();
  return 0;
}

int stove_reward_head_bwd(const float* pred, const float* params, const float* reward, const float* saved, const float* d_reward, float* d_pred,
                          float* g_params, float* ws, int items, int n_obj, void* stream) {
  hipStream_t st = (hipStream_t)stream;
  if (items == 0) {
    (void)hipMemsetAsync(g_params, 0, kRhParams * sizeof(float), st);
    return 0;
  }
  if (n_obj < 1 || ws == nullptr || d_pred == nullptr || g_params == nullptr) return (int)hipErrorInvalidValue;
  const float* H0 = saved;
  const float* Q = H0 + (size_t)items * n_obj * 32;
  const float* A1 = Q + (size_t)items * 32;
  const float* A2 = A1 + (size_t)items * 16;
  const int blocks = reward_head_blocks(items);
  STOVE_LAUNCH(reward_head_bwd_k, dim3(blocks), dim3(64 * kRhWaves), 0, st, pred, params, reward, H0, Q, A1, A2, d_reward, d_pred, ws, items, n_obj);
  STOVE_LAUNCH_CHECK();
  STOVE_LAUNCH(reduce_chunks_k, dim3((kRhParams + 31) / 32), dim3(256), 0, st, (const float*)ws, g_params, kRhParams, blocks * kRhWaves, 0);
  STOVE_LAUNCH_CHECK();
  return 0;
}

int stove_small_linear(const float* x, const float* W, const float* b, float* y, int rows, int in_dim, int out_dim, int w_transposed, void* stream) {
  if (rows == 0) return 0;
  if (in_dim < 1 || out_dim < 1 || in_dim > 64 || out_dim > 64) return (int)hipErrorInvalidValue;
  const size_t total = (size_t)rows * out_dim;
  if ((total + 255) / 256 > 0x7fffffffULL) return (int)hipErrorInvalidValue;
  STOVE_LAUNCH(small_linear_k, dim3((unsigned)((total + 255) / 256)), dim3(256), 0, (hipStream_t)stream, x, W, b, y, rows, in_dim, out_dim, w_transposed);
  STOVE_LAUNCH_CHECK();
  return 0;
}

int stove_stream_after(void* to, void* from) { return (int)stream_after((hipStream_t)to, (hipStream_t)from); }

void* stove_event_list_begin(void) {
  std::lock_guard<std::mutex> g(event_list_mu());
  auto* v = new std::vector<hipEvent_t>();
  event_list_current() = v;
  return (void*)v;
}
int stove_event_list_end(void* list) {
  std::lock_guard<std::mutex> g(event_list_mu());
  if (event_list_current() == (std::vector<hipEvent_t>*)list) event_list_current() = nullptr;
  return list == nullptr ? 0 : (int)((std::vector<hipEvent_t>*)list)->size();
}
int stove_event_list_destroy(void* list) {
  if (list == nullptr) return 0;
  std::lock_guard<std::mutex> g(event_list_mu());
  auto* v = (std::vector<hipEvent_t>*)list;
  if (event_list_current() == v) event_list_current() = nullptr;
  hipError_t e = hipSuccess;
  for (hipEvent_t ev : *v) {
    const hipError_t d = hipEventDestroy(ev);
    if (e == hipSuccess) e = d;
  }
  delete v;
  return (int)e;
}

int stove_fill_words(void* p, uint32_t value, size_t n_words, void* stream) {
  if (n_words == 0) return 0;
  const size_t blocks = (n_words + 256 * 8 - 1) / (256 * 8);
  STOVE_LAUNCH(fill_words_k, dim3((unsigned)(blocks < 65536 ? blocks : 65536)), dim3(256), 0, (hipStream_t)stream, (uint32_t*)p, value, n_words);
  STOVE_LAUNCH_CHECK();
  return 0;
}

int stove_capture_begin(void* stream) { return (int)hipStreamBeginCapture((hipStream_t)stream, hipStreamCaptureModeRelaxed); }

int stove_capture_end(void* stream, void** graph_out, int* n_nodes) {
  hipGraph_t g = nullptr;
  if (graph_out == nullptr) return (int)hipErrorInvalidValue;
  *graph_out = nullptr;
  hipError_t e = hipStreamEndCapture((hipStream_t)stream, &g);
  if (e != hipSuccess) return (int)e;
  size_t n = 0;
  e = hipGraphGetNodes(g, nullptr, &n);
  if (n_nodes != nullptr) *n_nodes = (int)n;
  *graph_out = (void*)g;
  return (int)e;
}

int stove_graph_instantiate(void* graph, void** exec_out) {
  if (exec_out == nullptr) return (int)hipErrorInvalidValue;
  *exec_out = nullptr;
  if (graph == nullptr) return 0;
  hipGraph_t g = (hipGraph_t)graph;
  size_t n = 0;
  hipError_t e = hipGraphGetNodes(g, nullptr, &n);
  if (e == hipSuccess && n > 0) {
    hipGraphExec_t x = nullptr;
    e = hipGraphInstantiate(&x, g, nullptr, nullptr, 0);
    if (e == hipSuccess) *exec_out = (void*)x;
  }
  const hipError_t d = hipGraphDestroy(g);
  return (int)(e != hipSuccess ? e : d);
}

int stove_graph_launch(void* exec, void* stream) { return (int)hipGraphLaunch((hipGraphExec_t)exec, (hipStream_t)stream); }

int stove_graph_destroy(void* exec) { return exec == nullptr ? 0 : (int)hipGraphExecDestroy((hipGraphExec_t)exec); }

int stove_bw_transform(const float* x, float* out, int n_frames, int channels, int pixels, void* stream) {
  if (n_frames == 0) return 0;
  if (pixels % 4 != 0 || channels < 1) return (int)hipErrorInvalidValue;
  const long long total = (long long)n_frames * (pixels / 4);
  if (total > 0x7fffffffLL) return (int)hipErrorInvalidValue;
  STOVE_LAUNCH(bw_transform_k, dim3((unsigned)((total + 255) / 256)), dim3(256), 0, (hipStream_t)stream, x, out, n_frames, channels, pixels / 4);
  STOVE_LAUNCH_CHECK();
  return 0;
}

int stove_bw_transform_u8(const unsigned char* x, float* out, int n_frames, int channels, int pixels, void* stream) {
  if (n_frames == 0) return 0;
  if (pixels % 4 != 0 || channels < 1) return (int)hipErrorInvalidValue;
  const long long total = (long long)n_frames * (pixels / 4);
  if (total > 0x7fffffffLL) return (int)hipErrorInvalidValue;
  STOVE_LAUNCH(bw_transform_u8_k, dim3((unsigned)((total + 255) / 256)), dim3(256), 0, (hipStream_t)stream, x, out, n_frames, channels, pixels / 4);
  STOVE_LAUNCH_CHECK();
  return 0;
}

size_t stove_colsum_ws_floats(int rows, int cols) {
  const int chunks = rows < 512 ? (rows < 1 ? 1 : rows) : 512;
  return (size_t)(chunks + 16) * cols;
}

static int colsum_level(const float* a, float* part, int rows, int cols, int max_chunks, hipStream_t st) {
  const int chunks = rows < max_chunks ? rows : max_chunks;
  const int per = (rows + chunks - 1) / chunks;
  const int used = (rows + per - 1) / per;
  if (cols <= 64) {
    int cpad = 1;
    while (cpad < cols) cpad <<= 1;
    STOVE_LAUNCH(colsum_narrow_part_k, dim3(used), dim3(256), 0, st, a, part, rows, cols, cpad, per);
  } else {
    STOVE_LAUNCH(colsum_part_k, dim3(used, (cols / 4 + 255) / 256), dim3(256), 0, st, a, part, rows, cols / 4, per);
  }
  return used;
}

int stove_colsum(const float* a, float* out, float* ws, int rows, int cols, void* stream) { return stove_colsum2(a, out, nullptr, 0, ws, rows, cols, stream); }

int stove_colsum2(const float* a, float* out, float* out2, int accumulate, float* ws, int rows, int cols, void* stream) {
  hipStream_t st = (hipStream_t)stream;
  if (cols <= 0 || (cols % 4 != 0 && cols > 64)) return (int)hipErrorInvalidValue;
  if (rows == 0) {
    if (!accumulate) {
      hipMemsetAsync(out, 0, sizeof(float) * cols, st);
      if (out2 != nullptr) hipMemsetAsync(out2, 0, sizeof(float) * cols, st);
    }
    return 0;
  }
  int used = colsum_level(a, ws, rows, cols, 512, st);
  STOVE_LAUNCH_CHECK();
  const float* src = ws;
  if (used > 16) {
    float* ws2 = ws + (size_t)(rows < 512 ? rows : 512) * cols;
    used = colsum_level(ws, ws2, used, cols, 16, st);
    STOVE_LAUNCH_CHECK();
    src = ws2;
  }
  STOVE_LAUNCH(reduce_chunks_k, dim3((cols + 31) / 32), dim3(256), 0, st, src, out, cols, used, accumulate, out2);
  STOVE_LAUNCH_CHECK();
  return 0;
}

static int small_tn_chunks(int rows) { return rows < 64 ? 1 : (rows / 64 < 512 ? rows / 64 : 512); }
size_t stove_small_tn_ws_floats(int rows, int M, int N) { return (size_t)small_tn_chunks(rows) * M * N; }

int stove_small_tn(const float* a, const float* b, float* out, float* ws, int rows, int M, int N, void* stream) {
  hipStream_t st = (hipStream_t)stream;
  if (M < 1 || N < 1 || M * N > 256) return (int)hipErrorInvalidValue;
  if (rows == 0) {
    hipMemsetAsync(out, 0, sizeof(float) * M * N, st);
    return 0;
  }
  const int chunks = small_tn_chunks(rows), per = (rows + chunks - 1) / chunks;
  STOVE_LAUNCH(small_tn_part_k, dim3(chunks), dim3(256), 0, st, a, b, ws, rows, M, N, per);
  STOVE_LAUNCH_CHECK();
  STOVE_LAUNCH(reduce_chunks_k, dim3((M * N + 31) / 32), dim3(256), 0, st, (const float*)ws, out, M * N, chunks, 0);
  STOVE_LAUNCH_CHECK();
  return 0;
}

size_t stove_flat_adam_ws_bytes(int nseg) { return (size_t)nseg * sizeof(int) + ADAM_SCAN_BLOCKS * sizeof(float); }

int stove_flat_adam(float* params, const float* grads, float* exp_avg, float* exp_avg_sq, float* max_exp_avg_sq, size_t numel,
                    const int* seg_of4, const unsigned char* seg_trainable, float* seg_steps, int nseg, void* ws, float* grad_norm_out,
                    const float* hyper_dev, float lr, float beta1, float beta2, float eps, float max_norm, int clip, void* stream) {
  if (numel == 0 || nseg == 0) return 0;
  if (numel % 4 != 0 || ws == nullptr || seg_of4 == nullptr || seg_trainable == nullptr || seg_steps == nullptr)
    return (int)hipErrorInvalidValue;
  AdamHyper k;
  k.lr = lr; k.b1 = beta1; k.b2 = beta2; k.eps = eps; k.max_norm = max_norm;
  const int n4 = (int)(numel / 4);
  hipStream_t st = (hipStream_t)stream;
  float* part = reinterpret_cast<float*>(ws);
  int* flags = reinterpret_cast<int*>(part + ADAM_SCAN_BLOCKS);
  STOVE_LAUNCH(grad_scan_k, dim3(ADAM_SCAN_BLOCKS), dim3(256), 0, st, grads, seg_of4, flags, part, n4);
  STOVE_LAUNCH(flat_adam_k, dim3((n4 + 255) / 256), dim3(256), 0, st, params, grads, exp_avg, exp_avg_sq, max_exp_avg_sq, seg_of4,
               seg_trainable, (const float*)seg_steps, (const int*)flags, (const float*)part, grad_norm_out, hyper_dev, k, clip & 1, n4);
  STOVE_LAUNCH(adam_tick_k, dim3((nseg + 255) / 256), dim3(256), 0, st, seg_trainable, seg_steps, flags, nseg, (clip >> 1) & 1);
  STOVE_LAUNCH_CHECK();
  return 0;
}

static ZpConst zp_const(const float* span_low) {
  ZpConst k;
  for (int d = 0; d < 8; ++d) {
    k.span[d] = span_low[d];
    k.low[d] = span_low[8 + d];
  }
  return k;
}

int stove_supair_state_fwd(const float* codes, const float* span_low, float* zc, float* pos, long long* idx, float* zfix,
                           unsigned char* hits, float* zl, float* sl, float* init6, int n, int T, int o, int skip, int fix,
                           int mode, void* stream) {
  return stove_supair_state_fwd2(codes, span_low, zc, pos, idx, zfix, hits, zl, sl, init6, 6, nullptr, 0, n, T, o, skip, fix, mode, stream);
}

int stove_supair_state_fwd2(const float* codes, const float* span_low, float* zc, float* pos, long long* idx, float* zfix,
                            unsigned char* hits, float* zl, float* sl, float* init, int init_ld, const float* lat_noise, int lat_dim,
                            int n, int T, int o, int skip, int fix, int mode, void* stream) {
  if (init_ld < 6 + (lat_noise != nullptr ? lat_dim : 0) || lat_dim < 0) return (int)hipErrorInvalidValue;
  float* init6 = init;
  hipStream_t st = (hipStream_t)stream;
  if (n == 0) return 0;
  if (T < 2 || skip < 1 || skip >= T || o < 1 || o > kMatchN) return (int)hipErrorInvalidValue;
  const int M = n * T * o;
  if (codes != nullptr) {
    STOVE_LAUNCH(zp_constrain_k, dim3((M * 8 + 255) / 256), dim3(256), 0, st, codes, zp_const(span_low), zc, pos, M);
    STOVE_LAUNCH_CHECK();
    int rc = stove_match_objects(pos, idx, nullptr, n, T, o, 2, mode, stream);
    if (rc) return rc;
  }
  STOVE_LAUNCH(supair_state_fwd_k, dim3((M + 255) / 256), dim3(256), 0, st, (const float*)zc, (const long long*)idx, zfix, hits, zl, sl,
               init6, n, T, o, skip, fix, init_ld, lat_noise, lat_dim);
  STOVE_LAUNCH_CHECK();
  return 0;
}

int stove_supair_state_bwd(const float* zc, const long long* idx, const unsigned char* hits, const float* zfix, const float* g_zfix,
                           const float* g_zl, const float* g_sl, const float* g_init6, const float* span_low, float* gfix_ws,
                           float* g_codes, int n, int T, int o, int skip, void* stream) {
  return stove_supair_state_bwd2(zc, idx, hits, zfix, g_zfix, g_zl, g_sl, g_init6, 6, span_low, gfix_ws, g_codes, n, T, o, skip, stream);
}

int stove_supair_state_bwd2(const float* zc, const long long* idx, const unsigned char* hits, const float* zfix, const float* g_zfix,
                            const float* g_zl, const float* g_sl, const float* g_init6, int init_ld, const float* span_low, float* gfix_ws,
                            float* g_codes, int n, int T, int o, int skip, void* stream) {
  hipStream_t st = (hipStream_t)stream;
  if (n == 0) return 0;
  const int M = n * T * o;
  (void)gfix_ws;
  STOVE_LAUNCH(supair_state_bwd_k, dim3((M + 255) / 256), dim3(256), 0, st, zc, idx, hits, zfix, g_zfix, g_zl, g_sl, g_init6, zp_const(span_low),
               g_codes, n, T, o, skip, init_ld);
  STOVE_LAUNCH_CHECK();
  return 0;
}

int stove_noise_normal(float* out, size_t n, unsigned long long* state, void* stream) {
  if (n == 0) return 0;
  if (((uintptr_t)out & 15) != 0 || state == nullptr) return (int)hipErrorInvalidValue;
  const size_t threads = (n + 3) / 4;
  if ((threads + 255) / 256 > 0x7fffffffULL) return (int)hipErrorInvalidValue;
  STOVE_LAUNCH(noise_normal_k, dim3((unsigned)((threads + 255) / 256)), dim3(256), 0, (hipStream_t)stream, out, n, (const unsigned long long*)state);
  STOVE_LAUNCH(noise_tick_k, dim3(1), dim3(1), 0, (hipStream_t)stream, state);
  STOVE_LAUNCH_CHECK();
  return 0;
}

int stove_zall_fwd(const float* zfix, const float* zs, float* zall, int n, int T, int o, int skip, void* stream) {
  if (n == 0) return 0;
  const int M = n * (T - 1) * o;
  STOVE_LAUNCH(zall_fwd_k, dim3((M + 255) / 256), dim3(256), 0, (hipStream_t)stream, zfix, zs, zall, n, T, o, skip);
  STOVE_LAUNCH_CHECK();
  return 0;
}

int stove_zall_bwd(const float* zfix, const float* zs, const float* g_zall, const float* dz_in, float* g_zfix, float* g_zs, int n, int T, int o,
                   int skip, void* stream) {
  if (n == 0) return 0;
  const int M = n * T * o + n * (T - skip) * o;
  STOVE_LAUNCH(zall_bwd_k, dim3((M + 255) / 256), dim3(256), 0, (hipStream_t)stream, zfix, zs, g_zall, dz_in, g_zfix, g_zs, n, T, o, skip);
  STOVE_LAUNCH_CHECK();
  return 0;
}

static TransStd trans_std(const float* s16) {
  TransStd t;
  for (int d = 0; d < 16; ++d) t.s[d] = s16[d];
  return t;
}

int stove_elbo_fwd(const float* zs, const float* mean, const float* std_, const float* zdyn, const float* lik, const float* trans_std16,
                   float* part_ws, float* out3, int n, int T, int o, int skip, void* stream) {
  hipStream_t st = (hipStream_t)stream;
  if (n == 0 || skip < 1 || skip >= T) return (int)hipErrorInvalidValue;
  STOVE_LAUNCH(elbo_part_k, dim3(n), dim3(256), 0, st, zs, mean, std_, zdyn, lik, trans_std(trans_std16), part_ws, T, o, skip);
  STOVE_LAUNCH_CHECK();
  STOVE_LAUNCH(elbo_final_k, dim3(1), dim3(256), 0, st, (const float*)part_ws, out3, n, T, skip);
  STOVE_LAUNCH_CHECK();
  return 0;
}

int stove_elbo_bwd(const float* zs, const float* mean, const float* std_, const float* zdyn, const float* trans_std16, const float* g_out,
                   float* g_zs, float* g_mean, float* g_std, float* g_zdyn, float* g_lik, int n, int T, int o, int skip, void* stream) {
  if (n == 0) return 0;
  const size_t M = (size_t)n * (T - skip) * o * 18 + (size_t)n * (T - 1);
  STOVE_LAUNCH(elbo_bwd_k, dim3((unsigned)((M + 255) / 256)), dim3(256), 0, (hipStream_t)stream, zs, mean, std_, zdyn, trans_std(trans_std16), g_out,
               g_zs, g_mean, g_std, g_zdyn, g_lik, n, T, o, skip);
  STOVE_LAUNCH_CHECK();
  return 0;
}

static int enc_head_groups(int rows) {
  const int tiles = (rows + 15) / 16;
  int g = (tiles + 3) / 4;
  return g < 1 ? 1 : (g > 102 ? 102 : g);
}

int stove_enc_head_fwd(const float* h, const float* W1, const float* b1, const float* W2, const float* b2, float* h1, float* codes, int rows,
                       int H, int HID, int OUT, int frames, int fc1_split, void* stream) {
  if (H != kEhH || HID < 1 || HID > kEhHid || OUT != kEhOut || frames < 0 || (frames > 0 && rows % frames != 0)) return (int)hipErrorInvalidValue;
  if (rows == 0) return 0;
  static_assert(2 * kEhHid * kEhLdB == sizeof(float) * kEhHid * kEhLd, "the two bf16 images of W1 take the fp32 image's place");
  const size_t lds = sizeof(float) * kEhHid * kEhLd;
  const int tiles = (rows + 15) / 16;
  const int grid = (tiles + 3) / 4 < 512 ? (tiles + 3) / 4 : 512;
  int rc;
  if (fc1_split) {
    rc = (int)hipFuncSetAttribute((const void*)enc_head_fwd_k<true>, hipFuncAttributeMaxDynamicSharedMemorySize, (int)lds);
    if (rc) return rc;
    STOVE_LAUNCH((enc_head_fwd_k<true>), dim3(grid), dim3(256), lds, (hipStream_t)stream, h, W1, b1, W2, b2, h1, codes, rows, HID, frames);
  } else {
    rc = (int)hipFuncSetAttribute((const void*)enc_head_fwd_k<false>, hipFuncAttributeMaxDynamicSharedMemorySize, (int)lds);
    if (rc) return rc;
    STOVE_LAUNCH((enc_head_fwd_k<false>), dim3(grid), dim3(256), lds, (hipStream_t)stream, h, W1, b1, W2, b2, h1, codes, rows, HID, frames);
  }
  STOVE_LAUNCH_CHECK();
  return 0;
}

size_t stove_enc_head_bwd_ws_floats(int rows, int HID) { return (size_t)enc_head_groups(rows) * eh_part_floats(HID); }

int stove_enc_head_bwd(const float* dcodes, const float* h1, const float* h, const float* W1, const float* W2, float* gh, float* gW1,
                       float* gb1, float* gW2, float* gb2, int accumulate, float* ws, int rows, int H, int HID, int OUT, int frames, void* stream) {
  if (H != kEhH || HID < 1 || HID > kEhHid || OUT != kEhOut || frames < 0 || (frames > 0 && rows % frames != 0)) return (int)hipErrorInvalidValue;
  hipStream_t st = (hipStream_t)stream;
  const int P = eh_part_floats(HID);
  if (rows == 0) {
    if (!accumulate) {
      hipMemsetAsync(gW1, 0, sizeof(float) * HID * kEhH, st);
      hipMemsetAsync(gW2, 0, sizeof(float) * kEhOut * HID, st);
      hipMemsetAsync(gb1, 0, sizeof(float) * HID, st);
      hipMemsetAsync(gb2, 0, sizeof(float) * kEhOut, st);
    }
    return 0;
  }
  const int groups = enc_head_groups(rows);
  const size_t lds = sizeof(float) * kEhBwdLds;
  int rc;
  if (HID <= 50) {
    rc = (int)hipFuncSetAttribute((const void*)enc_head_bwd_k<14>, hipFuncAttributeMaxDynamicSharedMemorySize, (int)lds);
    if (rc) return rc;
    STOVE_LAUNCH(enc_head_bwd_k<14>, dim3(groups * 5), dim3(256), lds, st, dcodes, h1, h, W1, W2, gh, ws, rows, HID, groups, frames);
  } else {
    rc = (int)hipFuncSetAttribute((const void*)enc_head_bwd_k<16>, hipFuncAttributeMaxDynamicSharedMemorySize, (int)lds);
    if (rc) return rc;
    STOVE_LAUNCH(enc_head_bwd_k<16>, dim3(groups * 5), dim3(256), lds, st, dcodes, h1, h, W1, W2, gh, ws, rows, HID, groups, frames);
  }
  STOVE_LAUNCH_CHECK();
  (void)P;
  STOVE_LAUNCH(enc_head_reduce_k, dim3((eh_part_floats(HID) + 31) / 32), dim3(256), 0, st, (const float*)ws, gW1, gW2, gb1, gb2, HID, groups, accumulate);
  STOVE_LAUNCH_CHECK();
  return 0;
}

int stove_lstm_cell_fwd(const float* gx, const float* gh, const float* c_prev, float* c, float* h, int n, int H, int fast, void* stream) {
  if (n == 0) return 0;
  if (H % 4) return (int)hipErrorInvalidValue;
  const size_t total = (size_t)n * (H / 4);
  const int grid = (int)((total + 255) / 256 < 8192 ? (total + 255) / 256 : 8192);
  if (fast) STOVE_LAUNCH(lstm_cell_fwd_k<true>, dim3(grid), dim3(256), 0, (hipStream_t)stream, gx, gh, c_prev, c, h, n, H);
  else STOVE_LAUNCH(lstm_cell_fwd_k<false>, dim3(grid), dim3(256), 0, (hipStream_t)stream, gx, gh, c_prev, c, h, n, H);
  STOVE_LAUNCH_CHECK();
  return 0;
}

int stove_lstm_cell_bwd(const float* gx, const float* gh, const float* c_prev, const float* c, const float* dh,
                        const float* dc_in, float* dg, float* dc_out, float* dgx_sum, const float* dg_more, int n_more, int n, int H,
                        int fast, void* stream) {
  if (n == 0) return 0;
  if (H % 4 || n_more < 0 || (n_more > 0 && dg_more == nullptr)) return (int)hipErrorInvalidValue;
  const size_t more_stride = (size_t)n * 4 * H;
  const size_t total = (size_t)n * (H / 4);
  const int grid = (int)((total + 255) / 256 < 8192 ? (total + 255) / 256 : 8192);
  if (fast) STOVE_LAUNCH(lstm_cell_bwd_k<true>, dim3(grid), dim3(256), 0, (hipStream_t)stream, gx, gh, c_prev, c, dh, dc_in, dg, dc_out, dgx_sum, dg_more,
                         n_more, more_stride, n, H);
  else STOVE_LAUNCH(lstm_cell_bwd_k<false>, dim3(grid), dim3(256), 0, (hipStream_t)stream, gx, gh, c_prev, c, dh, dc_in, dg, dc_out, dgx_sum, dg_more,
                    n_more, more_stride, n, H);
  STOVE_LAUNCH_CHECK();
  return 0;
}

void stove_profile_enable(int on) {
  std::lock_guard<std::mutex> g(prof_mu());
  prof_on() = on != 0;
}

size_t stove_profile_report(char* buf, size_t cap) {
  std::lock_guard<std::mutex> g(prof_mu());
  struct Agg {
    std::string name;
    double total = 0.0;
    long count = 0;
    std::vector<std::pair<double, double>> spans;
  };
  std::vector<Agg> agg;
  auto& recs = prof_recs();
  for (auto& r : recs) (void)hipEventSynchronize(r.b);
  for (auto& r : recs) {
    float ms = 0.0f, t0 = 0.0f;
    (void)hipEventElapsedTime(&ms, r.a, r.b);
    (void)hipEventElapsedTime(&t0, recs.front().a, r.a);
    Agg* e = nullptr;
    for (auto& x : agg)
      if (x.name == r.name) {
        e = &x;
        break;
      }
    if (e == nullptr) {
      agg.push_back(Agg());
      e = &agg.back();
      e->name = r.name;
    }
    e->total += ms;
    e->count += 1;
    e->spans.push_back({(double)t0, (double)t0 + ms});
  }
  for (auto& r : recs) {
    (void)hipEventDestroy(r.a);
    (void)hipEventDestroy(r.b);
  }
  recs.clear();
  std::string out;
  for (auto& e : agg) {
    std::sort(e.spans.begin(), e.spans.end());
    double wall = 0.0, lo = 0.0, hi = -1.0;
    for (auto& sp : e.spans) {
      if (hi < lo || sp.first > hi) {
        if (hi >= lo) wall += hi - lo;
        lo = sp.first;
        hi = sp.second;
// ... 44 lines not shown
```

### stove_amd/csrc/match.hip

```cpp
#include "common.h"

namespace stove {

constexpr int kMatchN = 8, kMatchF = 8;

template <int TN, int TF>
__global__ __launch_bounds__(64) void match_objects_k(const float* __restrict__ feat, long long* __restrict__ idx_out,
                                                      float* __restrict__ perm_out, int B, int T, int Nrt, int Frt, int mode) {
  const int N = TN > 0 ? TN : Nrt;
  const int F = TF > 0 ? TF : Frt;
  extern __shared__ float mlds[];
  const int b = blockIdx.x;
  const int n_feat = T * N * F;
  int* ibuf = reinterpret_cast<int*>(mlds + n_feat);
  for (int i = threadIdx.x; i < n_feat; i += 64) mlds[i] = feat[(size_t)b * n_feat + i];
  __syncthreads();
  if (threadIdx.x == 0) {
  constexpr int MN = TN > 0 ? TN : kMatchN, MF = TF > 0 ? TF : kMatchF;
  float prev[MN][MF], cur[MN][MF], err[MN][MN];
  const float* fb = mlds;
  _Pragma("unroll") for (int a = 0; a < N; ++a) {
    _Pragma("unroll") for (int f = 0; f < F; ++f) prev[a][f] = (fb[a * F + f] + 1.0f) * 0.5f;
    ibuf[a] = a;
  }
// ... 156 lines not shown
    e = fmaf(d, d, e);
  }
  return e;
}
__device__ __forceinline__ bool greedy_rounds(float (&e)[kMatchN][kMatchN], int N, int* assign) {
  bool tie = false;
  for (int round = 0; round < N; ++round) {
    float bv = __builtin_inff();
    int ba = 0, bj = 0, cnt = 0;
#pragma unroll
    for (int a = 0; a < kMatchN; ++a)
#pragma unroll
      for (int j = 0; j < kMatchN; ++j) {
        if (a < N && j < N) {
          const float v = e[a][j];
          cnt = v < bv ? 1 : (v == bv ? cnt + 1 : cnt);
          if (v < bv) {
            bv = v;
            ba = a;
            bj = j;
          }
        }
      }
    tie = tie || (cnt > 1 && bv < 3.0e38f);
    assign[ba] = bj;
#pragma unroll
    for (int a = 0; a < kMatchN; ++a)
#pragma unroll
      for (int j = 0; j < kMatchN; ++j)
        if (a == ba || j == bj) e[a][j] = 3.0e38f;
  }
  return tie;
}
__device__ __forceinline__ unsigned char* greedy_scratch(long long* idx_out, int b, int T, int N) {
  return reinterpret_cast<unsigned char*>(idx_out + (size_t)(b + 1) * T * N) - (size_t)T * N - T;
}
__global__ __launch_bounds__(256) void match_greedy_frames_k(const float* __restrict__ feat, long long* __restrict__ idx_out, int B, int T, int N, int F) {
  const int i = blockIdx.x * blockDim.x + threadIdx.x;
  if (i >= B * T) return;
  const int b = i / T, t = i % T;
  unsigned char* sc = greedy_scratch(idx_out, b, T, N);
  if (t == 0) {
    for (int a = 0; a < N; ++a) sc[a] = (unsigned char)a;
    sc[(size_t)T * N] = 0;
    return;
  }
  const float* prev = feat + ((size_t)b * T + t - 1) * N * F;
  const float* cur = prev + (size_t)N * F;
  float e[kMatchN][kMatchN];
#pragma unroll
  for (int a = 0; a < kMatchN; ++a)
#pragma unroll
    for (int j = 0; j < kMatchN; ++j) e[a][j] = (a < N && j < N) ? match_err(prev + a * F, cur + j * F, F) : 3.0e38f;
  int assign[kMatchN];
#pragma unroll
  for (int a = 0; a < kMatchN; ++a) assign[a] = 0;
  const bool tie = greedy_rounds(e, N, assign);
#pragma unroll
  for (int a = 0; a < kMatchN; ++a)
    if (a < N) sc[(size_t)t * N + a] = (unsigned char)assign[a];
  sc[(size_t)T * N + t] = tie ? 1 : 0;
}
__global__ __launch_bounds__(64) void match_greedy_compose_k(const float* __restrict__ feat, long long* __restrict__ idx_out, int B, int T, int N, int F) {
  extern __shared__ unsigned char glds[];
  const int b = blockIdx.x, lane = threadIdx.x;
  const unsigned char* sc = greedy_scratch(idx_out, b, T, N);
  const int nsc = T * N + T;
  for (int i = lane; i < nsc; i += 64) glds[i] = sc[i];
  int* ibuf = reinterpret_cast<int*>(glds + ((nsc + 3) & ~3));
  __shared__ int slot[kMatchN];
  __syncthreads();
  int r = lane < N ? lane : 0;
  if (lane < N) ibuf[lane] = r;
  for (int t = 1; t < T; ++t) {
    if (glds[T * N + t] == 0) {
      r = glds[t * N + r];
    } else {
      if (lane < N) slot[lane] = r;
      __syncthreads();
      if (lane == 0) {
        const float* prev = feat + ((size_t)b * T + t - 1) * N * F;
        const float* cur = prev + (size_t)N * F;
        float e[kMatchN][kMatchN];
#pragma unroll
        for (int a = 0; a < kMatchN; ++a)
#pragma unroll
          for (int j = 0; j < kMatchN; ++j) e[a][j] = (a < N && j < N) ? match_err(prev + slot[a < N ? a : 0] * F, cur + j * F, F) : 3.0e38f;
        int assign[kMatchN];
#pragma unroll
        for (int a = 0; a < kMatchN; ++a) assign[a] = 0;
        greedy_rounds(e, N, assign);
#pragma unroll
        for (int a = 0; a < kMatchN; ++a)
          if (a < N) slot[a] = assign[a];
      }
      __syncthreads();
      if (lane < N) r = slot[lane];
      __syncthreads();
    }
    if (lane < N) ibuf[t * N + lane] = r;
  }
  __syncthreads();
  for (int i = lane; i < T * N; i += 64) idx_out[(size_t)b * T * N + i] = ibuf[i];
}

struct Perm3 {
  int p0, p1, p2;
};
__device__ __forceinline__ Perm3 perm3_of(int k) {
  Perm3 r;
  r.p0 = k >> 1;
  const int lo = r.p0 == 0 ? 1 : 0, hi = r.p0 == 2 ? 1 : 2;
  r.p1 = (k & 1) ? hi : lo;
  r.p2 = (k & 1) ? lo : hi;
  return r;
}
__device__ __forceinline__ int perm3_id(const Perm3& p) { return 2 * p.p0 + (p.p1 > p.p2 ? 1 : 0); }
__device__ __forceinline__ float sel3(int i, float a, float b, float c) { return i == 0 ? a : (i == 1 ? b : c); }
__device__ __forceinline__ Perm3 match3_step(const float (&D)[3][3], const Perm3& p) {
  float e[3][3];
#pragma unroll
  for (int j = 0; j < 3; ++j) {
    e[0][j] = sel3(p.p0, D[0][j], D[1][j], D[2][j]);
    e[1][j] = sel3(p.p1, D[0][j], D[1][j], D[2][j]);
    e[2][j] = sel3(p.p2, D[0][j], D[1][j], D[2][j]);
  }
  int idx[3];
#pragma unroll
  for (int a = 0; a < 3; ++a) {
    int best = 0;
    if (e[a][1] < e[a][best]) best = 1;
    if (e[a][2] < sel3(best, e[a][0], e[a][1], e[a][2])) best = 2;
    idx[a] = best;
  }
  if (idx[0] == idx[1] || idx[0] == idx[2] || idx[1] == idx[2]) {
#pragma unroll
    for (int a = 0; a < 3; ++a) {
      int best = 0;
      if (e[a][1] < e[a][0]) best = 1;
      if (e[a][2] < sel3(best, e[a][0], e[a][1], e[a][2])) best = 2;
      idx[a] = best;
#pragma unroll
      for (int r = 0; r < 3; ++r) {
        e[r][0] = best == 0 ? 1e12f : e[r][0];
        e[r][1] = best == 1 ? 1e12f : e[r][1];
        e[r][2] = best == 2 ? 1e12f : e[r][2];
      }
    }
  }
  return Perm3{idx[0], idx[1], idx[2]};
}

template <int F>
__global__ __launch_bounds__(64) void match3_table_k(const float* __restrict__ feat, long long* __restrict__ idx_out, int B, int T) {
  extern __shared__ float mlds[];
  const int b = blockIdx.x, lane = threadIdx.x;
  const int n_feat = T * 3 * F;
  int* ibuf = reinterpret_cast<int*>(mlds + n_feat);
  for (int i = lane; i < n_feat; i += 64) mlds[i] = feat[(size_t)b * n_feat + i];
  __syncthreads();
  const int chunk = (T - 1 + 63) / 64;
  const int t0 = 1 + lane * chunk, t1 = t0 + chunk < T ? t0 + chunk : T;
  auto table = [&](int t, float (&D)[3][3]) {
    float pv[3][F], cv[3][F];
#pragma unroll
    for (int i = 0; i < 3; ++i)
#pragma unroll
      for (int f = 0; f < F; ++f) {
        pv[i][f] = (mlds[((t - 1) * 3 + i) * F + f] + 1.0f) * 0.5f;
        cv[i][f] = (mlds[(t * 3 + i) * F + f] + 1.0f) * 0.5f;
      }
#pragma unroll
    for (int i = 0; i < 3; ++i)
#pragma unroll
      for (int j = 0; j < 3; ++j) {
        float sacc = 0.0f;
#pragma unroll
        for (int f = 0; f < F; ++f) {
          const float d = pv[i][f] - cv[j][f];
          sacc += d * d;
        }
        D[i][j] = sacc;
      }
  };
  int cur[6] = {0, 1, 2, 3, 4, 5};
  for (int t = t0; t < t1; ++t) {
    float D[3][3];
    table(t, D);
#pragma unroll
    for (int k = 0; k < 6; ++k) cur[k] = perm3_id(match3_step(D, perm3_of(cur[k])));
  }
  unsigned m = 0;
#pragma unroll
  for (int k = 0; k < 6; ++k) m |= (unsigned)cur[k] << (3 * k);
#pragma unroll
  for (int d = 1; d < 64; d <<= 1) {
    const unsigned o = (unsigned)__builtin_amdgcn_ds_bpermute(((lane - d) & 63) * 4, (int)m);
    if (lane >= d) {
      unsigned n = 0;
#pragma unroll
      for (int k = 0; k < 6; ++k) n |= ((m >> (3 * ((o >> (3 * k)) & 7u))) & 7u) << (3 * k);
      m = n;
    }
  }
  const unsigned before = (unsigned)__builtin_amdgcn_ds_bpermute(((lane - 1) & 63) * 4, (int)m);
  Perm3 p = perm3_of(lane == 0 ? 0 : (int)(before & 7u));
  if (lane == 0) {
    ibuf[0] = 0;
    ibuf[1] = 1;
    ibuf[2] = 2;
  }
  for (int t = t0; t < t1; ++t) {
    float D[3][3];
    table(t, D);
    p = match3_step(D, p);
    ibuf[t * 3 + 0] = p.p0;
    ibuf[t * 3 + 1] = p.p1;
    ibuf[t * 3 + 2] = p.p2;
  }
  __syncthreads();
  for (int i = lane; i < T * 3; i += 64) idx_out[(size_t)b * T * 3 + i] = ibuf[i];
}

}
```

### stove_amd/csrc/state.hip

```cpp
#include "common.h"

namespace stove {

struct ZpConst {
  float span[8], low[8];
};

__global__ void zp_constrain_k(const float* __restrict__ codes, ZpConst kc, float* __restrict__ zc, float* __restrict__ pos, int M) {
  const int i = blockIdx.x * blockDim.x + threadIdx.x;
  if (i >= M * 8) return;
  const int d = i & 7;
  const float v = fmaf(kc.span[d], sigmoidf_(codes[i]), kc.low[d]);
  zc[i] = v;
  if (d == 2 || d == 3) pos[(i >> 3) * 2 + d - 2] = v;
}

__device__ __forceinline__ void load8(const float* __restrict__ p, float* v) {
  const float4 a = *reinterpret_cast<const float4*>(p), b = *reinterpret_cast<const float4*>(p + 4);
  v[0] = a.x; v[1] = a.y; v[2] = a.z; v[3] = a.w; v[4] = b.x; v[5] = b.y; v[6] = b.z; v[7] = b.w;
}

__device__ __forceinline__ int fixed_state(const float* __restrict__ zc, const long long* __restrict__ idx, int b, int t, int k, int T,
                                           int o, int fix, float* out) {
  const size_t row = (size_t)b * T + t;
  float cur[8];
  load8(zc + (row * o + idx[row * o + k]) * 8, cur);
  int hit = 0;
  if (fix && t >= 1 && t <= T - 2) {
    float pv[8], nx[8];
    load8(zc + ((row - 1) * o + idx[(row - 1) * o + k]) * 8, pv);
    load8(zc + ((row + 1) * o + idx[(row + 1) * o + k]) * 8, nx);
#pragma unroll
    for (int a = 0; a < 2; ++a)
      if (fabsf(cur[a] - pv[a]) > 0.095f && fabsf(nx[a] - cur[a]) > 0.095f) hit |= 1 << a;
#pragma unroll
    for (int d = 0; d < 8; ++d)
      if (hit & (1 << (d & 1))) cur[d] = 0.5f * (pv[d] + nx[d]);
  }
#pragma unroll
  for (int d = 0; d < 8; ++d) out[d] = cur[d];
  return hit;
}

__global__ void supair_state_fwd_k(const float* __restrict__ zc, const long long* __restrict__ idx, float* __restrict__ zfix,
                                   unsigned char* __restrict__ hits, float* __restrict__ zl, float* __restrict__ sl,
                                   float* __restrict__ init6, int n, int T, int o, int skip, int fix, int init_ld,
                                   const float* __restrict__ lat_noise, int lat_dim) {
  const int i = blockIdx.x * blockDim.x + threadIdx.x;
  if (i >= n * T * o) return;
  const int k = i % o, t = (i / o) % T, b = i / (o * T);
  float cur[8], pv[8];
  const int hit = fixed_state(zc, idx, b, t, k, T, o, fix, cur);
  hits[i] = (unsigned char)hit;
#pragma unroll
  for (int d = 0; d < 8; ++d) zfix[(size_t)i * 8 + d] = cur[d];
  if (t < skip - 1 || t < 1) return;
  fixed_state(zc, idx, b, t - 1, k, T, o, fix, pv);
  float z6[6], s6[6];
#pragma unroll
  for (int d = 0; d < 4; ++d) {
    z6[d] = cur[d];
    s6[d] = cur[4 + d];
  }
#pragma unroll
  for (int a = 0; a < 2; ++a) {
    z6[4 + a] = cur[2 + a] - pv[2 + a];
    s6[4 + a] = sqrtf(cur[6 + a] * cur[6 + a] + pv[6 + a] * pv[6 + a]);
  }
  if (t == skip - 1) {
#pragma unroll
    for (int d = 0; d < 6; ++d) init6[((size_t)b * o + k) * init_ld + d] = z6[d];
    if (lat_noise != nullptr)
      for (int d = 0; d < lat_dim; ++d) init6[((size_t)b * o + k) * init_ld + 6 + d] = 0.01f * lat_noise[((size_t)b * o + k) * lat_dim + d];
  } else {
    const size_t r = (((size_t)b * (T - skip) + (t - skip)) * o + k) * 6;
#pragma unroll
    for (int d = 0; d < 6; ++d) {
      zl[r + d] = z6[d];
      sl[r + d] = s6[d];
    }
  }
}

__device__ __forceinline__ void g6_at(const float* __restrict__ g_zl, const float* __restrict__ g_sl, const float* __restrict__ g_init6,
                                      int b, int t, int k, int T, int o, int skip, float* gz, float* gs, int init_ld) {
#pragma unroll
  for (int d = 0; d < 6; ++d) gz[d] = gs[d] = 0.0f;
  if (t < 1 || t > T - 1) return;
  if (t == skip - 1) {
    if (g_init6 != nullptr)
#pragma unroll
      for (int d = 0; d < 6; ++d) gz[d] = g_init6[((size_t)b * o + k) * init_ld + d];
  } else if (t >= skip) {
    const size_t r = (((size_t)b * (T - skip) + (t - skip)) * o + k) * 6;
#pragma unroll
    for (int d = 0; d < 6; ++d) {
      if (g_zl != nullptr) gz[d] = g_zl[r + d];
      if (g_sl != nullptr) gs[d] = g_sl[r + d];
    }
  }
}

__device__ __forceinline__ void supair_gfix(const float* __restrict__ zfix, const float* __restrict__ g_zfix, const float* __restrict__ g_zl,
                                            const float* __restrict__ g_sl, const float* __restrict__ g_init6, size_t i, int T, int o, int skip,
                                            int init_ld, float (&g)[8]) {
  const int k = (int)(i % o), t = (int)((i / o) % T), b = (int)(i / ((size_t)o * T));
#pragma unroll
  for (int d = 0; d < 8; ++d) g[d] = g_zfix != nullptr ? g_zfix[i * 8 + d] : 0.0f;
  float gz[6], gs[6], gzn[6], gsn[6];
  g6_at(g_zl, g_sl, g_init6, b, t, k, T, o, skip, gz, gs, init_ld);
  g6_at(g_zl, g_sl, g_init6, b, t + 1, k, T, o, skip, gzn, gsn, init_ld);
#pragma unroll
  for (int d = 0; d < 4; ++d) {
    g[d] += gz[d];
    g[4 + d] += gs[d];
  }
  float cur[8];
  load8(zfix + i * 8, cur);
#pragma unroll
  for (int a = 0; a < 2; ++a) {
    g[2 + a] += gz[4 + a] - gzn[4 + a];
    if (gs[4 + a] != 0.0f) {
      const float p = zfix[(i - o) * 8 + 6 + a];
      g[6 + a] += gs[4 + a] * cur[6 + a] / sqrtf(cur[6 + a] * cur[6 + a] + p * p);
    }
    if (gsn[4 + a] != 0.0f) {
      const float q = zfix[(i + o) * 8 + 6 + a];
      g[6 + a] += gsn[4 + a] * cur[6 + a] / sqrtf(q * q + cur[6 + a] * cur[6 + a]);
    }
  }
}

__global__ void supair_state_bwd_k(const float* __restrict__ zc, const long long* __restrict__ idx, const unsigned char* __restrict__ hits,
                                   const float* __restrict__ zfix, const float* __restrict__ g_zfix, const float* __restrict__ g_zl,
                                   const float* __restrict__ g_sl, const float* __restrict__ g_init6, ZpConst kc, float* __restrict__ g_codes,
                                   int n, int T, int o, int skip, int init_ld) {
  const int i = blockIdx.x * blockDim.x + threadIdx.x;
  if (i >= n * T * o) return;
  const int j = i % o, t = (i / o) % T, b = i / (o * T);
  const size_t row = (size_t)b * T + t;
  float acc[8] = {0, 0, 0, 0, 0, 0, 0, 0};
  for (int k = 0; k < o; ++k) {
    if ((int)idx[row * o + k] != j) continue;
    const size_t e = row * o + k;
    const int h0 = hits[e];
    const int hp = (t >= 1) ? hits[e - o] : 0, hn = (t <= T - 2) ? hits[e + o] : 0;
    float g0[8], gp[8], gn[8];
    supair_gfix(zfix, g_zfix, g_zl, g_sl, g_init6, e, T, o, skip, init_ld, g0);
    if (hp) supair_gfix(zfix, g_zfix, g_zl, g_sl, g_init6, e - o, T, o, skip, init_ld, gp);
    if (hn) supair_gfix(zfix, g_zfix, g_zl, g_sl, g_init6, e + o, T, o, skip, init_ld, gn);
#pragma unroll
    for (int d = 0; d < 8; ++d) {
      const int bit = 1 << (d & 1);
      float v = (h0 & bit) ? 0.0f : g0[d];
      if (hp & bit) v += 0.5f * gp[d];
      if (hn & bit) v += 0.5f * gn[d];
      acc[d] += v;
    }
  }
#pragma unroll
  for (int d = 0; d < 8; ++d) {
    const float s = (zc[(size_t)i * 8 + d] - kc.low[d]) / kc.span[d];
    g_codes[(size_t)i * 8 + d] = acc[d] * kc.span[d] * s * (1.0f - s);
  }
}

__global__ void zall_fwd_k(const float* __restrict__ zfix, const float* __restrict__ zs, float* __restrict__ zall, int n, int T, int o, int skip) {
  const int i = blockIdx.x * blockDim.x + threadIdx.x;
  if (i >= n * (T - 1) * o) return;
  const int k = i % o, j = (i / o) % (T - 1), b = i / (o * (T - 1));
  const float* src = (j < skip - 1) ? zfix + (((size_t)b * T + 1 + j) * o + k) * 8 : zs + (((size_t)b * (T - skip) + (j - (skip - 1))) * o + k) * 18;
  const float sx = src[0];
  zall[(size_t)i * 4] = sx;
  zall[(size_t)i * 4 + 1] = sx * src[1];
  zall[(size_t)i * 4 + 2] = src[2];
  zall[(size_t)i * 4 + 3] = src[3];
}
__global__ void zall_bwd_k(const float* __restrict__ zfix, const float* __restrict__ zs, const float* __restrict__ g_zall,
                           const float* __restrict__ dz_in, float* __restrict__ g_zfix, float* __restrict__ g_zs, int n, int T, int o, int skip) {
  const int i = blockIdx.x * blockDim.x + threadIdx.x;
  const int nfix = n * T * o, nzs = n * (T - skip) * o;
  if (i < nfix) {
    const int k = i % o, t = (i / o) % T, b = i / (o * T);
    float g[8] = {0, 0, 0, 0, 0, 0, 0, 0};
    if (t >= 1 && t < skip) {
      const size_t a = (((size_t)b * (T - 1) + (t - 1)) * o + k) * 4;
      const float* src = zfix + (size_t)i * 8;
      g[0] = g_zall[a] + g_zall[a + 1] * src[1];
      g[1] = g_zall[a + 1] * src[0];
      g[2] = g_zall[a + 2];
      g[3] = g_zall[a + 3];
    }
#pragma unroll
    for (int d = 0; d < 8; ++d) g_zfix[(size_t)i * 8 + d] = g[d];
  } else if (i < nfix + nzs) {
    const int q = i - nfix;
    const int k = q % o, ts = (q / o) % (T - skip), b = q / (o * (T - skip));
    const size_t a = (((size_t)b * (T - 1) + (skip - 1 + ts)) * o + k) * 4;
    const float* src = zs + (size_t)q * 18;
    float* g = g_zs + (size_t)q * 18;
    float v[4];
    v[0] = g_zall[a] + g_zall[a + 1] * src[1];
    v[1] = g_zall[a + 1] * src[0];
    v[2] = g_zall[a + 2];
    v[3] = g_zall[a + 3];
    if (dz_in == nullptr) {
#pragma unroll
      for (int d = 0; d < 18; ++d) g[d] = d < 4 ? v[d] : 0.0f;
    } else {
      const float* gi = dz_in + (size_t)q * 18;
#pragma unroll
      for (int d = 0; d < 18; ++d) g[d] = d < 4 ? v[d] + gi[d] : gi[d];
    }
  }
}

__device__ __forceinline__ void philox_round(uint32_t& c0, uint32_t& c1, uint32_t& c2, uint32_t& c3, uint32_t k0, uint32_t k1) {
  const uint64_t p0 = (uint64_t)0xD2511F53u * c0, p1 = (uint64_t)0xCD9E8D57u * c2;
  const uint32_t n0 = (uint32_t)(p1 >> 32) ^ c1 ^ k0, n2 = (uint32_t)(p0 >> 32) ^ c3 ^ k1;
  c1 = (uint32_t)p1;
  c3 = (uint32_t)p0;
  c0 = n0;
  c2 = n2;
}
__device__ __forceinline__ float u01(uint32_t r) { return ((float)(r >> 8) + 0.5f) * (1.0f / 16777216.0f); }
__global__ __launch_bounds__(256) void noise_normal_k(float* __restrict__ out, size_t n, const unsigned long long* __restrict__ state) {
  const size_t i = (size_t)blockIdx.x * blockDim.x + threadIdx.x;
  if (4 * i >= n) return;
  const unsigned long long seed = state[0], call = state[1];
  uint32_t c0 = (uint32_t)call, c1 = (uint32_t)(call >> 32), c2 = (uint32_t)i, c3 = (uint32_t)(i >> 32);
  uint32_t k0 = (uint32_t)seed, k1 = (uint32_t)(seed >> 32);
#pragma unroll
  for (int r = 0; r < 10; ++r) {
    philox_round(c0, c1, c2, c3, k0, k1);
    k0 += 0x9E3779B9u;
    k1 += 0xBB67AE85u;
  }
  const float r0 = sqrtf(-1.3862943611198906f * __builtin_amdgcn_logf(u01(c0))), r1 = sqrtf(-1.3862943611198906f * __builtin_amdgcn_logf(u01(c2)));
  const float a0 = u01(c1), a1 = u01(c3);
  const float v[4] = {r0 * __builtin_amdgcn_cosf(a0), r0 * __builtin_amdgcn_sinf(a0), r1 * __builtin_amdgcn_cosf(a1), r1 * __builtin_amdgcn_sinf(a1)};
  if (4 * i + 3 < n) {
    *reinterpret_cast<float4*>(out + 4 * i) = float4{v[0], v[1], v[2], v[3]};
  } else {
    for (size_t e = 4 * i; e < n; ++e) out[e] = v[e - 4 * i];
  }
}
__global__ void noise_tick_k(unsigned long long* __restrict__ state) { state[1] += 1ull; }

struct TransStd {
  float s[16];
};
__global__ __launch_bounds__(256) void elbo_part_k(const float* __restrict__ zs, const float* __restrict__ mean, const float* __restrict__ stdv,
                                                   const float* __restrict__ zdyn, const float* __restrict__ lik, TransStd ts_,
                                                   float* __restrict__ part, int T, int o, int skip) {
  const int b = blockIdx.x, Ts = T - skip, rows = Ts * o;
  float tr = 0.0f, lq = 0.0f, lk = 0.0f, ls = 0.0f;
  for (int r = threadIdx.x; r < rows; r += blockDim.x) {
    const size_t e = (size_t)b * rows + r;
    const float* z = zs + e * 18;
    const float* m = mean + e * 18;
    const float* s = stdv + e * 18;
    const float* zd = zdyn + e * 16;
#pragma unroll
    for (int q = 0; q < 18; ++q) {
      const float u = (z[q] - m[q]) / s[q];
      lq += -0.5f * u * u - logf(s[q]) - 0.5f * kLog2Pi;
    }
#pragma unroll
    for (int d = 0; d < 16; ++d) {
      const float u = (z[2 + d] - zd[d]) / ts_.s[d];
      tr += -0.5f * u * u - logf(ts_.s[d]) - 0.5f * kLog2Pi;
    }
  }
  for (int j = threadIdx.x; j < T - 1; j += blockDim.x) {
    const float v = lik[(size_t)b * (T - 1) + j];
    if (j < skip - 1) ls += v;
    else lk += v;
  }
  __shared__ float red[4][4];
  float v4[4] = {tr - lq + lk, ls, tr, lq};
#pragma unroll
  for (int c = 0; c < 4; ++c) {
    const float w = wave_sum(v4[c]);
    if (lane_id() == 0) red[c][wave_id()] = w;
  }
  __syncthreads();
  if (threadIdx.x < 4) part[b * 4 + threadIdx.x] = (red[threadIdx.x][0] + red[threadIdx.x][1]) + (red[threadIdx.x][2] + red[threadIdx.x][3]);
}
__global__ __launch_bounds__(256) void elbo_final_k(const float* __restrict__ part, float* __restrict__ out, int n, int T, int skip) {
  float a[4] = {0, 0, 0, 0};
  for (int b = threadIdx.x; b < n; b += blockDim.x)
#pragma unroll
    for (int c = 0; c < 4; ++c) a[c] += part[b * 4 + c];
  __shared__ float red[4][4];
#pragma unroll
  for (int c = 0; c < 4; ++c) {
    const float w = wave_sum(a[c]);
    if (lane_id() == 0) red[c][wave_id()] = w;
  }
  __syncthreads();
  if (threadIdx.x == 0) {
    float s[4];
#pragma unroll
    for (int c = 0; c < 4; ++c) s[c] = (red[c][0] + red[c][1]) + (red[c][2] + red[c][3]);
    const float nt = (float)n * (float)(T - skip);
    out[0] = s[0] / nt + (skip > 1 ? s[1] / ((float)n * (float)(skip - 1)) : 0.0f);
    out[1] = s[2] / nt;
    out[2] = s[3] / nt;
  }
}
__global__ __launch_bounds__(256) void elbo_bwd_k(const float* __restrict__ zs, const float* __restrict__ mean, const float* __restrict__ stdv,
                                                  const float* __restrict__ zdyn, TransStd ts_, const float* __restrict__ gout, float* __restrict__ g_zs,
                                                  float* __restrict__ g_mean, float* __restrict__ g_std, float* __restrict__ g_zdyn, float* __restrict__ g_lik,
                                                  int n, int T, int o, int skip) {
  const size_t i = (size_t)blockIdx.x * blockDim.x + threadIdx.x;
  const size_t rows = (size_t)n * (T - skip) * o, ne = rows * 18;
  const float g = gout[0];
  const float c1 = g / ((float)n * (float)(T - skip));
  if (i < ne) {
    const size_t r = i / 18;
    const int q = (int)(i - r * 18);
    const float z = zs[i];
    const float is = 1.0f / stdv[i], u = (z - mean[i]) * is;
    float gz = c1 * u * is;
    g_mean[i] = -c1 * u * is;
    g_std[i] = -c1 * (u * u - 1.0f) * is;
    if (q >= 2) {
      const float it = 1.0f / ts_.s[q - 2], v = (z - zdyn[r * 16 + q - 2]) * it;
      gz -= c1 * v * it;
      g_zdyn[r * 16 + q - 2] = c1 * v * it;
    }
    g_zs[i] = gz;
  } else if (i < ne + (size_t)n * (T - 1)) {
    const size_t e = i - ne;
    const int j = (int)(e % (T - 1));
    g_lik[e] = (j < skip - 1) ? g / ((float)n * (float)(skip - 1)) : c1;
  }
}

}
```

### stove_amd/csrc/validate.h

```cpp
#pragma once
#include <stddef.h>
#include <stdint.h>

#include "../../include/stove_hip.h"

namespace stove_validate {

constexpr int kStoveInvalidValue = 1;
constexpr int kMaxObjects = 8;

inline bool null_any() { return false; }
template <typename T, typename... Rest>
inline bool null_any(const T* p, const Rest*... rest) { return p == nullptr || null_any(rest...); }
inline bool misaligned16(const void* p) { return (reinterpret_cast<uintptr_t>(p) & 15) != 0; }

inline int obj_tables(const StoveSpnTables* t) {
  if (t == nullptr || null_any(t->obj_scope, t->obj_coef, t->obj_wsum, t->obj_wroot)) return kStoveInvalidValue;
  return 0;
}
inline int bg_tables(const StoveSpnTables* t) {
  if (t == nullptr || null_any(t->bg_side, t->bg_coef, t->bg_wroot)) return kStoveInvalidValue;
  return 0;
}
inline int table_grads(const StoveSpnTableGrads* g, bool obj, bool bg) {
// ... 32 lines not shown
  if (null_any(inputs, ell, out, dout)) return kStoveInvalidValue;
  if (d_marg != nullptr && marg == nullptr) return kStoveInvalidValue;
  return 0;
}

inline int frame_map(int n_frames, int seq_frames, int seq_stride) {
  if (seq_frames == 0) return 0;
  if (seq_frames < 0 || seq_stride < seq_frames || n_frames % seq_frames != 0) return kStoveInvalidValue;
  return 0;
}
inline int scene_fwd(const StoveSpnTables* t, const float* frames, const float* z, int n_frames, int n_obj, int seq_frames, int seq_stride,
                     const float* ll, const float* saved) {
  if (n_frames < 0 || n_obj < 1 || n_obj > kMaxObjects || frame_map(n_frames, seq_frames, seq_stride)) return kStoveInvalidValue;
  if (n_frames == 0) return 0;
  if (obj_tables(t) || bg_tables(t) || null_any(frames, z, ll, saved)) return kStoveInvalidValue;
  return 0;
}
inline int scene_bwd(const StoveSpnTables* t, const float* frames, const float* z, int n_frames, int n_obj, int seq_frames, int seq_stride,
                     const float* saved, const float* dll, const float* dz, const StoveSpnTableGrads* g, const void* ws) {
  if (n_frames < 0 || n_obj < 1 || n_obj > kMaxObjects || frame_map(n_frames, seq_frames, seq_stride)) return kStoveInvalidValue;
  if (n_frames == 0) return 0;
  if (obj_tables(t) || t->obj_leaf_slot == nullptr || bg_tables(t) || null_any(frames, z, saved, dll, dz) || ws == nullptr ||
      table_grads(g, true, true))
    return kStoveInvalidValue;
  return 0;
}

inline bool obj_any_bad(int R, int G, int S, int D, int Lmax) {
  return R < 1 || R > 8 || G < 1 || G > 16 || S < 1 || S > 16 || D < 4 || D > 1024 || Lmax < 1 || Lmax > D;
}
inline bool scene_ch_bad(int R, int G, int S, int D, int Lmax, size_t bg_coef_floats, int n_frames, int n_obj, int seq_frames, int seq_stride,
                        int channels, int W, int H, int pw, int ph) {
  if (n_frames < 0 || n_obj < 1 || n_obj > kMaxObjects || frame_map(n_frames, seq_frames, seq_stride)) return true;
  if (channels < 1 || channels > 4 || W < 2 || H < 2 || pw < 2 || ph < 2 || obj_any_bad(R, G, S, D, Lmax)) return true;
  return (long long)D != (long long)channels * pw * ph || bg_coef_floats != (size_t)3 * channels * W * H * 6 * 3;
}
inline int scene_ch_fwd(const int32_t* lscope, const float* coef, const float* wsum, const float* wroot, int R, int G, int S, int D, int Lmax,
                        const int32_t* bg_side, const float* bg_coef, const float* bg_wroot, size_t bg_coef_floats, const float* frames,
                        const float* z, int n_frames, int n_obj, int seq_frames, int seq_stride, int channels, int W, int H, int pw, int ph,
                        const float* ll, const float* saved) {
  if (scene_ch_bad(R, G, S, D, Lmax, bg_coef_floats, n_frames, n_obj, seq_frames, seq_stride, channels, W, H, pw, ph)) return kStoveInvalidValue;
  if (n_frames == 0) return 0;
  if (lscope == nullptr || bg_side == nullptr || null_any(coef, wsum, wroot, bg_coef, bg_wroot, frames, z, ll, saved)) return kStoveInvalidValue;
  return 0;
}
inline int scene_ch_bwd(const int32_t* lscope, const int32_t* slot, const float* coef, const float* wsum, const float* wroot, int R, int G, int S,
                        int D, int Lmax, const int32_t* bg_side, const float* bg_coef, const float* bg_wroot, size_t bg_coef_floats,
                        const float* frames, const float* z, int n_frames, int n_obj, int seq_frames, int seq_stride, int channels, int W, int H,
                        int pw, int ph, const float* saved, const float* dll, const float* dz, const float* g_coef, const float* g_wsum,
                        const float* g_wroot, const float* g_bg_coef, const float* g_bg_wroot, const void* ws) {
  if (scene_ch_bad(R, G, S, D, Lmax, bg_coef_floats, n_frames, n_obj, seq_frames, seq_stride, channels, W, H, pw, ph)) return kStoveInvalidValue;
  if (n_frames == 0) return 0;
  if (lscope == nullptr || slot == nullptr || bg_side == nullptr || ws == nullptr ||
      null_any(coef, wsum, wroot, bg_coef, bg_wroot, frames, z, saved, dll, dz, g_coef, g_wsum, g_wroot, g_bg_coef, g_bg_wroot))
    return kStoveInvalidValue;
  return 0;
}

inline int gnn_shape(int B, int N, int sin_dim) {
  if (B < 0 || N < 1 || N > kMaxObjects || sin_dim < 16 || sin_dim > 32) return kStoveInvalidValue;
  return 0;
}
inline int gnn_fwd(const float* s_in, const float* params, const float* result, int B, int N, int sin_dim) {
  if (gnn_shape(B, N, sin_dim)) return kStoveInvalidValue;
  if (B == 0) return 0;
  return null_any(s_in, params, result) ? kStoveInvalidValue : 0;
}
inline int gnn_bwd(const float* s_in, const float* params, const float* d_result, const float* d_s_in, const float* g_params, const void* ws,
                   int B, int N, int sin_dim) {
  if (gnn_shape(B, N, sin_dim)) return kStoveInvalidValue;
  if (B == 0) return 0;
  return (null_any(s_in, params, d_result, d_s_in, g_params) || ws == nullptr) ? kStoveInvalidValue : 0;
}
inline int dynloop_fwd(const float* z1, const float* zsup, const float* zsstd, const float* eps, const float* extra, const float* params,
                       const float* z, const float* zdyn, const float* zdstd, const float* mean, const float* std_, int B, int Ts, int N,
                       int sin_dim) {
  if (gnn_shape(B, N, sin_dim) || Ts < 0) return kStoveInvalidValue;
  if (B == 0 || Ts == 0) return 0;
  if (null_any(z1, zsup, zsstd, eps, params, z, zdyn, zdstd, mean, std_)) return kStoveInvalidValue;
  if (sin_dim > 16 && extra == nullptr) return kStoveInvalidValue;
  return 0;
}
inline int dynloop_bwd(const float* z1, const float* zsup, const float* zsstd, const float* eps, const float* extra, const float* params,
                       const float* z, const float* dz1, const float* dzsup, const float* dzsstd, const float* dextra, const float* g_params,
                       const void* ws, int B, int Ts, int N, int sin_dim) {
  if (gnn_shape(B, N, sin_dim) || B == 0 || Ts <= 0) return kStoveInvalidValue;
  if (null_any(z1, zsup, zsstd, eps, params, z, dz1, dzsup, dzsstd, g_params) || ws == nullptr) return kStoveInvalidValue;
  if (sin_dim > 16 && (extra == nullptr || dextra == nullptr)) return kStoveInvalidValue;
  return 0;
}
inline int rollout_fwd(const float* z_last, const float* extra, const float* params, const float* z_pred, int B, int num, int A, int N,
                       int sin_dim) {
  if (gnn_shape(B, N, sin_dim) || num < 0) return kStoveInvalidValue;
  if (B == 0 || num == 0) return 0;
  if (null_any(z_last, params, z_pred)) return kStoveInvalidValue;
  if (sin_dim > 16 && (extra == nullptr || A < 1)) return kStoveInvalidValue;
  return 0;
}

constexpr int kMaxObjectsCl = 6;
inline bool gnn_cl_bad(int cl, int B, int N, int sin_dim) {
  return (cl != 16 && cl != 64) || B < 0 || N < 1 || N > kMaxObjectsCl || sin_dim < cl / 2 || sin_dim > cl;
}
inline int gnn_fwd_cl(const float* s_in, const float* params, const float* result, int cl, int B, int N, int sin_dim) {
  if (gnn_cl_bad(cl, B, N, sin_dim)) return kStoveInvalidValue;
  if (B == 0) return 0;
  return null_any(s_in, params, result) ? kStoveInvalidValue : 0;
}
inline int gnn_bwd_cl(const float* s_in, const float* params, const float* d_result, const float* d_s_in, const float* g_params,
                      const void* ws, int cl, int B, int N, int sin_dim) {
  if (gnn_cl_bad(cl, B, N, sin_dim) || g_params == nullptr) return kStoveInvalidValue;
  if (B == 0) return 0;
  return (null_any(s_in, params, d_result, d_s_in) || ws == nullptr) ? kStoveInvalidValue : 0;
}
inline int dynloop_fwd_cl(const float* z1, const float* zsup, const float* zsstd, const float* eps, const float* extra, const float* params,
                          const float* z, const float* zdyn, const float* zdstd, const float* mean, const float* std_, int cl, int B, int Ts,
                          int N, int sin_dim) {
  if (gnn_cl_bad(cl, B, N, sin_dim) || Ts < 0) return kStoveInvalidValue;
  if (B == 0 || Ts == 0) return 0;
  if (null_any(z1, zsup, zsstd, eps, params, z, zdyn, zdstd, mean, std_)) return kStoveInvalidValue;
  if (sin_dim > cl / 2 && extra == nullptr) return kStoveInvalidValue;
  return 0;
}
inline int dynloop_bwd_cl(const float* z1, const float* zsup, const float* zsstd, const float* eps, const float* extra, const float* params,
                          const float* z, const float* dz1, const float* dzsup, const float* dzsstd, const float* dextra,
                          const float* g_params, const void* ws, int cl, int B, int Ts, int N, int sin_dim) {
  if (gnn_cl_bad(cl, B, N, sin_dim) || Ts < 0 || g_params == nullptr) return kStoveInvalidValue;
  if (B == 0 || Ts == 0) return 0;
  if (null_any(z1, zsup, zsstd, eps, params, z, dz1, dzsup, dzsstd) || ws == nullptr) return kStoveInvalidValue;
  if (sin_dim > cl / 2 && (extra == nullptr || dextra == nullptr)) return kStoveInvalidValue;
  return 0;
}
inline int rollout_fwd_cl(const float* z_last, const float* extra, const float* params, const float* z_pred, int cl, int B, int num, int A,
                          int N, int sin_dim) {
  if (gnn_cl_bad(cl, B, N, sin_dim) || num < 0) return kStoveInvalidValue;
  if (B == 0 || num == 0) return 0;
  if (null_any(z_last, params, z_pred)) return kStoveInvalidValue;
  if (sin_dim > cl / 2 && (extra == nullptr || A < 1)) return kStoveInvalidValue;
  return 0;
}

inline int gemm(const float* A, const float* B, const float* C, int M, int N, int K, int lda, int ldb, int ldc, int a_kmajor, int b_kmajor,
                int nsplit, int splitk, const float* ws) {
  if (M < 0 || N < 0) return kStoveInvalidValue;
  if (M == 0 || N == 0) return 0;
  if (K <= 0 || splitk < 1 || nsplit < 1 || nsplit > 3) return kStoveInvalidValue;
  if (null_any(A, B, C)) return kStoveInvalidValue;
  if (lda < (a_kmajor ? M : K) || ldb < (b_kmajor ? N : K) || ldc < N) return kStoveInvalidValue;
  if (misaligned16(B) || (ldb & 3) != 0 || ((b_kmajor ? N : K) & 3) != 0) return kStoveInvalidValue;
  if (splitk > 1 && (ws == nullptr || ldc != N)) return kStoveInvalidValue;
  return 0;
}

}
```

### stove_amd/ops.py

```python
import ctypes
import math

import torch

from . import _lib
from . import settings as _settings
from ._lib import SpnTableGrads, SpnTables, check, ptr, stream


def _f32(t):
    if t is None:
        return None
    if not t.is_cuda:
        raise RuntimeError('stove_amd HIP ops need tensors on a GPU (cuda:N); there is no CPU path')
    if t.dtype != torch.float32:
        raise RuntimeError('stove_amd HIP kernels compute in float32; got %s' % t.dtype)
    return t.contiguous()


def _tables(obj=None, bg=None, bg_dense=None):
    t = SpnTables()
    if obj is not None:
        t.obj_scope, t.obj_leaf_slot, t.obj_coef, t.obj_wsum, t.obj_wroot = [ptr(x) for x in obj]
    if bg is not None:
# ... 701 lines not shown
        lib = _lib.load()
        z1, zsup, zsstd, eps = _f32(z1), _f32(zsup), _f32(zsstd), _f32(eps)
        extra = _f32(extra)
        B, Ts, N = zsup.shape[:3]
        D = cl // 2
        sd = D + (extra.shape[-1] if extra is not None else 0)
        dev = z1.device
        params = _gnn_image_cl(_f32(w_img), _f32(v_img), _f32(wt_img), cl)
        with torch.cuda.device(dev):
            def out(d):
                return torch.empty(B, Ts, N, d, dtype=torch.float32, device=dev)
            z, zdyn, zdstd, mean, std = out(D + 2), out(D), out(D), out(D + 2), out(D + 2)
            pred = out(cl) if want_pred else None
            check(lib.stove_dynloop_fwd_cl(ptr(z1), ptr(zsup), ptr(zsstd), ptr(eps), ptr(extra), ptr(params), ptr(z), ptr(zdyn),
                                           ptr(zdstd), ptr(mean), ptr(std), ptr(pred), cl, B, Ts, N, sd, int(lim_enc), int(elu),
                                           *[float(c) for c in consts], stream()), 'stove_dynloop_fwd_cl')
        ctx.save_for_backward(z1, zsup, zsstd, eps, extra, params, z)
        ctx.cfg = (cl, int(lim_enc), int(elu), tuple(float(c) for c in consts), sd)
        ctx.sink = sink
        ctx.set_materialize_grads(False)
        ctx.mark_non_differentiable(zdstd)
        if pred is None:
            pred = z.new_zeros(0)
            ctx.mark_non_differentiable(pred)
        return z, zdyn, zdstd, mean, std, pred

    @staticmethod
    def backward(ctx, dz, dzdyn, _dzdstd, dmean, dstd, dpred):
        lib = _lib.load()
        z1, zsup, zsstd, eps, extra, params, z = ctx.saved_tensors
        cl, lim_enc, elu, consts, sd = ctx.cfg
        B, Ts, N = zsup.shape[:3]
        dev = z1.device

        def up(g):
            return None if g is None or g.numel() == 0 else _f32(g)
        with torch.cuda.device(dev):
            dz1 = torch.empty_like(z1)
            dzsup, dzsstd = torch.empty_like(zsup), torch.empty_like(zsstd)
            dextra = torch.empty_like(extra) if extra is not None else None
            g = torch.empty(lib.stove_gnn_grad_floats_cl(cl), dtype=torch.float32, device=dev)
            ws = _ws(lib.stove_gnn_bwd_ws_bytes_cl(cl, B, N), dev)
            check(lib.stove_dynloop_bwd_cl(ptr(z1), ptr(zsup), ptr(zsstd), ptr(eps), ptr(extra), ptr(params), ptr(z),
                                           ptr(up(dz)), ptr(up(dzdyn)), ptr(up(dmean)), ptr(up(dstd)), ptr(up(dpred)),
                                           ptr(dz1), ptr(dzsup), ptr(dzsstd), ptr(dextra), ptr(g), ptr(ws),
                                           cl, B, Ts, N, sd, lim_enc, elu, *consts, stream()), 'stove_dynloop_bwd_cl')
        if ctx.sink is not None:
            ctx.sink(g)
            return (dz1, dzsup, dzsstd, None, dextra) + (None,) * 9
        W = gnn_w_floats(cl)
        return (dz1, dzsup, dzsstd, None, dextra, g[:W], g[W:]) + (None,) * 7


def _sunk(t, sink):
    if sink is not None and not t.requires_grad and torch.is_grad_enabled():
        return t.detach().requires_grad_()
    return t


def gnn_step(s_in, image, lim_enc=2, elu=False, sink=None, cl=32):
    _check_image_cl(image, cl)
    if cl != 32:
        return _GnnStepClFn.apply(_sunk(s_in, sink), image[0], image[1], image[2], cl, lim_enc, elu, sink)
    return _GnnStepFn.apply(_sunk(s_in, sink), image[0], image[1], image[2], lim_enc, elu, sink)


def dyn_loop(z1, zsup, zsstd, eps, extra, image, lim_enc, elu, consts, want_pred=False, sink=None):
    cl = 2 * (z1.shape[-1] - 2)
    if cl != 32:
        _check_image_cl(image, cl)
        return _DynLoopClFn.apply(_sunk(z1, sink), zsup, zsstd, eps, extra, image[0], image[1], image[2], cl, lim_enc, elu, consts,
                                  want_pred, sink)
    return _DynLoopFn.apply(_sunk(z1, sink), zsup, zsstd, eps, extra, image[0], image[1], image[2], lim_enc, elu, consts,
                            want_pred, sink)


@torch.no_grad()
def rollout(z_last, extra, image, num, lim_enc, elu, consts, want_std=False, want_pred=False):
    lib = _lib.load()
    z_last, extra = _f32(z_last), _f32(extra)
    B, N = z_last.shape[:2]
    A = extra.shape[1] if extra is not None else 1
    cl = 2 * (z_last.shape[-1] - 2)
    if cl != 32:
        _check_image_cl(image, cl)
        D = cl // 2
        sd = D + (extra.shape[-1] if extra is not None else 0)
        dev = z_last.device
        params = _gnn_image_cl(_f32(image[0]), _f32(image[1]), _f32(image[2]), cl)
        with torch.cuda.device(dev):
            z_pred = torch.empty(B, num, N, D + 2, dtype=torch.float32, device=dev)
            zstd = torch.empty(B, num, N, D, dtype=torch.float32, device=dev) if want_std else None
            pred = torch.empty(B, num, N, cl, dtype=torch.float32, device=dev) if want_pred else None
            check(lib.stove_rollout_fwd_cl(ptr(z_last), ptr(extra), ptr(params), ptr(z_pred), ptr(zstd), ptr(pred), cl, B, num, A, N, sd,
                                           int(lim_enc), int(elu), *[float(c) for c in consts], stream()), 'stove_rollout_fwd_cl')
        return z_pred, zstd, pred
    sd = 16 + (extra.shape[-1] if extra is not None else 0)
    dev = z_last.device
    params = _gnn_image(_f32(image[0]), _f32(image[1]), _f32(image[2]))
    with torch.cuda.device(dev):
        z_pred = torch.empty(B, num, N, 18, dtype=torch.float32, device=dev)
        zstd = torch.empty(B, num, N, 16, dtype=torch.float32, device=dev) if want_std else None
        pred = torch.empty(B, num, N, 32, dtype=torch.float32, device=dev) if want_pred else None
        check(lib.stove_rollout_fwd(ptr(z_last), ptr(extra), ptr(params), ptr(z_pred), ptr(zstd), ptr(pred), B, num, A, N, sd,
                                    int(lim_enc), int(elu), *[float(c) for c in consts], stream()), 'stove_rollout_fwd')
    return z_pred, zstd, pred


MATCH_MODES = {'3_only': 0, 'greedy': 1, 'volatile': 2, '3_only_serial': 3}


@torch.no_grad()
def match_objects(feat, mode):
    lib = _lib.load()
    feat = _f32(feat.detach())
    B, T, N, Fd = feat.shape
    dev = feat.device
    with torch.cuda.device(dev):
        idx = torch.empty(B, T, N, dtype=torch.int64, device=dev)
        perm = None
        check(lib.stove_match_objects(ptr(feat), ptr(idx), ptr(perm), B, T, N, Fd, MATCH_MODES[mode], stream()),
              'stove_match_objects')
    return idx, perm


def _host_floats(vals, n):
    vals = [float(v) for v in vals]
    if len(vals) != n:
        raise ValueError('expected %d floats, got %d' % (n, len(vals)))
    return (ctypes.c_float * n)(*vals)


class _SupairStateFn(torch.autograd.Function):

    @staticmethod
    def forward(ctx, codes, span_low, n, T, o, skip, fix, mode, lat_noise=None):
        lib = _lib.load()
        codes = _f32(codes)
        dev = codes.device
        Ts = T - skip
        kc = _host_floats(span_low, 16)
        lat_dim = 0
        if lat_noise is not None:
            lat_noise = _f32(lat_noise).reshape(n, o, -1)
            lat_dim = lat_noise.shape[-1]
        ld = 6 + lat_dim
        with torch.cuda.device(dev):
            def f(*shape):
                return torch.empty(*shape, dtype=torch.float32, device=dev)
            zc, pos, zfix = f(n, T, o, 8), f(n, T, o, 2), f(n, T, o, 8)
            idx = torch.empty(n, T, o, dtype=torch.int64, device=dev)
            hits = torch.empty(n, T, o, dtype=torch.uint8, device=dev)
            zl, sl, init6 = f(n, Ts, o, 6), f(n, Ts, o, 6), f(n, o, ld)
            check(lib.stove_supair_state_fwd2(ptr(codes), kc, ptr(zc), ptr(pos), ptr(idx), ptr(zfix), ptr(hits), ptr(zl), ptr(sl),
                                              ptr(init6), ld, ptr(lat_noise) if lat_noise is not None else None, lat_dim, n, T, o, skip,
                                              int(bool(fix)), MATCH_MODES[mode], stream()), 'stove_supair_state_fwd2')
        ctx.save_for_backward(zc, idx, hits, zfix)
        ctx.init_ld = ld
        ctx.cfg = (tuple(span_low), n, T, o, skip, codes.shape)
        ctx.set_materialize_grads(False)
        ctx.mark_non_differentiable(idx)
        return zfix, zl, sl, init6, idx

    @staticmethod
    def backward(ctx, g_zfix, g_zl, g_sl, g_init6, _g_idx):
        lib = _lib.load()
        zc, idx, hits, zfix = ctx.saved_tensors
        span_low, n, T, o, skip, shape = ctx.cfg
        dev = zc.device
        kc = _host_floats(span_low, 16)
        gs = [None if g is None else _f32(g) for g in (g_zfix, g_zl, g_sl, g_init6)]
        with torch.cuda.device(dev):
            ws = torch.empty(n * T * o * 8, dtype=torch.float32, device=dev)
            g_codes = torch.empty(shape, dtype=torch.float32, device=dev)
            check(lib.stove_supair_state_bwd2(ptr(zc), ptr(idx), ptr(hits), ptr(zfix), ptr(gs[0]), ptr(gs[1]), ptr(gs[2]), ptr(gs[3]),
                                              ctx.init_ld, kc, ptr(ws), ptr(g_codes), n, T, o, skip, stream()), 'stove_supair_state_bwd2')
        return g_codes, None, None, None, None, None, None, None, None


class _ZallFn(torch.autograd.Function):

    @staticmethod
    def forward(ctx, zfix, zs, n, T, o, skip):
        lib = _lib.load()
        zfix, zs = _f32(zfix), _f32(zs)
        dev = zfix.device
        with torch.cuda.device(dev):
            zall = torch.empty(n * (T - 1) * o, 4, dtype=torch.float32, device=dev)
            check(lib.stove_zall_fwd(ptr(zfix), ptr(zs), ptr(zall), n, T, o, skip, stream()), 'stove_zall_fwd')
        ctx.save_for_backward(zfix, zs)
        ctx.cfg = (n, T, o, skip)
        ctx.set_materialize_grads(False)
        return zall, zs.view_as(zs)

    @staticmethod
    def backward(ctx, g_zall, g_pass):
        lib = _lib.load()
        zfix, zs = ctx.saved_tensors
        n, T, o, skip = ctx.cfg
        if g_zall is None:
            return None, g_pass, None, None, None, None
        with torch.cuda.device(zfix.device):
            g_zfix, g_zs = torch.empty_like(zfix), torch.empty_like(zs)
            check(lib.stove_zall_bwd(ptr(zfix), ptr(zs), ptr(_f32(g_zall)), ptr(_f32(g_pass)) if g_pass is not None else None, ptr(g_zfix), ptr(g_zs),
                                     n, T, o, skip, stream()), 'stove_zall_bwd')
        return g_zfix, g_zs, None, None, None, None


class _ElboFn(torch.autograd.Function):

    @staticmethod
    def forward(ctx, zs, mean, std, zdyn, lik, trans_std, n, T, o, skip):
        lib = _lib.load()
        zs, mean, std, zdyn, lik = _f32(zs), _f32(mean), _f32(std), _f32(zdyn), _f32(lik)
        dev = zs.device
        ts = _host_floats(trans_std, 16)
        with torch.cuda.device(dev):
            part = torch.empty(n * 4, dtype=torch.float32, device=dev)
            out3 = torch.empty(3, dtype=torch.float32, device=dev)
            check(lib.stove_elbo_fwd(ptr(zs), ptr(mean), ptr(std), ptr(zdyn), ptr(lik), ts, ptr(part), ptr(out3), n, T, o, skip, stream()),
                  'stove_elbo_fwd')
        ctx.save_for_backward(zs, mean, std, zdyn)
        ctx.cfg = (tuple(trans_std), n, T, o, skip, lik.shape)
        stats = out3[1:]
        ctx.set_materialize_grads(False)
        ctx.mark_non_differentiable(stats)
        return out3[0], stats

    @staticmethod
    def backward(ctx, g_elbo, _g_stats):
        lib = _lib.load()
        zs, mean, std, zdyn = ctx.saved_tensors
        trans_std, n, T, o, skip, lik_shape = ctx.cfg
        ts = _host_floats(trans_std, 16)
        dev = zs.device
        if g_elbo is None:
            return (None,) * 10
        with torch.cuda.device(dev):
            g = _f32(g_elbo).reshape(1)
            g_zs, g_mean, g_std, g_zdyn = (torch.empty_like(t) for t in (zs, mean, std, zdyn))
            g_lik = torch.empty(lik_shape, dtype=torch.float32, device=dev)
            check(lib.stove_elbo_bwd(ptr(zs), ptr(mean), ptr(std), ptr(zdyn), ts, ptr(g), ptr(g_zs), ptr(g_mean), ptr(g_std), ptr(g_zdyn),
                                     ptr(g_lik), n, T, o, skip, stream()), 'stove_elbo_bwd')
        return g_zs, g_mean, g_std, g_zdyn, g_lik, None, None, None, None, None


def supair_state(codes, span_low, n, T, o, skip, fix, mode, lat_noise=None):
    return _SupairStateFn.apply(codes, tuple(float(v) for v in span_low), int(n), int(T), int(o), int(skip), bool(fix), mode, lat_noise)


def zall(zfix, zs, n, T, o, skip):
    return _ZallFn.apply(zfix, zs, int(n), int(T), int(o), int(skip))


def elbo(zs, mean, std, zdyn, lik, trans_std, n, T, o, skip):
    return _ElboFn.apply(zs, mean, std, zdyn, lik, tuple(float(v) for v in trans_std), int(n), int(T), int(o), int(skip))


@torch.no_grad()
def bw_transform(x):
    lib = _lib.load()
    if not x.is_cuda:
        raise RuntimeError('stove_amd HIP ops need tensors on a GPU (cuda:N); there is no CPU path')
    u8 = x.dtype == torch.uint8
    x = x.contiguous() if u8 else _f32(x)
    n, T, C, w, h = x.shape
    with torch.cuda.device(x.device):
        out = torch.empty(n, T, 1, w, h, dtype=torch.float32, device=x.device)
        if u8:
            check(lib.stove_bw_transform_u8(ptr(x), ptr(out), n * T, C, w * h, stream()), 'stove_bw_transform_u8')
        else:
            check(lib.stove_bw_transform(ptr(x), ptr(out), n * T, C, w * h, stream()), 'stove_bw_transform')
    return out


def colsum(a):
    lib = _lib.load()
    rows, cols = a.shape
    if cols % 4 != 0 and cols > 64:
        return a.sum(0)
    with torch.cuda.device(a.device):
        out = torch.empty(cols, dtype=torch.float32, device=a.device)
        ws = torch.empty(lib.stove_colsum_ws_floats(rows, cols) + 1, dtype=torch.float32, device=a.device)
        check(lib.stove_colsum(ptr(a), ptr(out), ptr(ws), rows, cols, stream()), 'stove_colsum')
    return out


def small_tn(a, b):
    lib = _lib.load()
    rows, M, N = a.shape[0], a.shape[1], b.shape[1]
    with torch.cuda.device(a.device):
        out = torch.empty(M, N, dtype=torch.float32, device=a.device)
        ws = torch.empty(lib.stove_small_tn_ws_floats(rows, M, N) + 1, dtype=torch.float32, device=a.device)
        check(lib.stove_small_tn(ptr(a), ptr(b), ptr(out), ptr(ws), rows, M, N, stream()), 'stove_small_tn')
    return out


class _LinearFn(torch.autograd.Function):

    @staticmethod
    def _narrow(x, weight):
        return x.is_cuda and x.dtype == torch.float32 and weight.dtype == torch.float32 and weight.shape[0] <= 64 and weight.shape[1] <= 64

    @staticmethod
    def forward(ctx, x, weight, bias):
        ctx.save_for_backward(x, weight)
        if _LinearFn._narrow(x, weight):
            lib = _lib.load()
            y = torch.empty(x.shape[0], weight.shape[0], dtype=torch.float32, device=x.device)
            with torch.cuda.device(x.device):
                check(lib.stove_small_linear(ptr(_f32(x)), ptr(_f32(weight)), ptr(_f32(bias)), ptr(y), x.shape[0], weight.shape[1], weight.shape[0], 0,
                                             stream()), 'stove_small_linear')
            return y
        return torch.addmm(bias, x, weight.t())

    @staticmethod
    def backward(ctx, g):
        x, weight = ctx.saved_tensors
        g = g.contiguous()
        gx = None
        if ctx.needs_input_grad[0]:
            if _LinearFn._narrow(x, weight):
                lib = _lib.load()
                gx = torch.empty_like(x)
                with torch.cuda.device(x.device):
                    check(lib.stove_small_linear(ptr(_f32(g)), ptr(_f32(weight)), None, ptr(gx), g.shape[0], weight.shape[0], weight.shape[1], 1,
                                                 stream()), 'stove_small_linear')
            else:
                gx = torch.mm(g, weight)
        gw = None
        if ctx.needs_input_grad[1]:
            if g.shape[1] * x.shape[1] <= 256 and g.shape[0] >= 2048 and g.dtype == torch.float32 and x.dtype == torch.float32 and g.is_cuda:
                gw = small_tn(g, x.contiguous())
            else:
                gw = _splitk_tn(g, x)
        gb = colsum(g) if ctx.needs_input_grad[2] else None
        return gx, gw, gb


class _RewardHeadFn(torch.autograd.Function):

    @staticmethod
    def forward(ctx, pred, *params):
        lib = _lib.load()
        pred = _f32(pred)
        items, o = pred.shape[0], pred.shape[1]
        dev = pred.device
        flat = torch.cat([_f32(p).reshape(-1) for p in params])
        if flat.numel() != lib.stove_reward_head_param_floats():
            raise RuntimeError('reward head: unexpected parameter shapes')
        with torch.cuda.device(dev):
            reward = torch.empty(items, dtype=torch.float32, device=dev)
            saved = torch.empty(lib.stove_reward_head_saved_floats(items, o) + 1, dtype=torch.float32, device=dev)
            check(lib.stove_reward_head_fwd(ptr(pred), ptr(flat), ptr(reward), ptr(saved), items, o, stream()), 'stove_reward_head_fwd')
        ctx.save_for_backward(pred, flat, reward, saved)
        ctx.shapes = [tuple(p.shape) for p in params]
        return reward

    @staticmethod
    def backward(ctx, d_reward):
        lib = _lib.load()
        pred, flat, reward, saved = ctx.saved_tensors
        items, o = pred.shape[0], pred.shape[1]
        dev = pred.device
        with torch.cuda.device(dev):
            d_pred = torch.empty_like(pred)
            g = torch.empty_like(flat)
            ws = torch.empty(lib.stove_reward_head_bwd_ws_floats(items) + 1, dtype=torch.float32, device=dev)
            check(lib.stove_reward_head_bwd(ptr(pred), ptr(flat), ptr(reward), ptr(saved), ptr(_f32(d_reward)), ptr(d_pred), ptr(g), ptr(ws),
                                            items, o, stream()), 'stove_reward_head_bwd')
        grads, off = [], 0
        for shp in ctx.shapes:
            n = 1
            for d in shp:
# ... 381 lines not shown
```

### stove_amd/optim.py

```python
import torch

from . import _lib


class FlatAdam(torch.optim.Optimizer):

    def __init__(self, arena, lr=1e-3, betas=(0.9, 0.999), eps=1e-8, amsgrad=False, strict_zero_grad=False):
        if arena.data.dtype != torch.float32 or not arena.data.is_cuda:
            raise RuntimeError('FlatAdam needs a float32 ParamArena on a GPU')
        super().__init__(arena.params, dict(lr=lr, betas=betas, eps=eps, amsgrad=amsgrad, weight_decay=0))
        self.arena = arena
        self.strict_zero_grad = bool(strict_zero_grad)
        self._steps = 0
        names = ['exp_avg', 'exp_avg_sq'] + (['max_exp_avg_sq'] if amsgrad else [])
        self._flat = {k: torch.zeros_like(arena.data) for k in names}
        dev = arena.data.device
        nseg = len(arena.params)
        seg = torch.zeros(arena.numel // 4, dtype=torch.int32)
        bounds = [arena.offset[id(p)] // 4 for p in arena.params] + [arena.numel // 4]
        for s_, (lo, hi) in enumerate(zip(bounds[:-1], bounds[1:])):
            seg[lo:hi] = s_
        self._seg_of4 = seg.to(dev)
        self._seg_steps = torch.zeros(nseg, dtype=torch.float32, device=dev)
        self._trainable_key, self._trainable = None, None
        self._ws = torch.zeros(_lib.load().stove_flat_adam_ws_bytes(nseg), dtype=torch.uint8, device=dev)
        self._norm = torch.zeros(1, dtype=torch.float32, device=dev)
        self._bind()

    def _bind(self):
        steps = self._seg_steps.cpu().tolist()
        for p, t in zip(self.arena.params, steps):
            st = self.state[p]
            st['step'] = torch.tensor(float(t))
            for k, flat in self._flat.items():
                st[k] = self.arena.view_of(p, flat)

    def _trainable_dev(self):
        key = tuple(p.requires_grad for p in self.arena.params)
        if key != self._trainable_key:
            self._trainable = torch.tensor(key, dtype=torch.uint8).to(self.arena.data.device)
            self._trainable_key = key
        return self._trainable

    def hyper(self, max_norm=None):
        g = self.param_groups[0]
        return [float(g['lr']), float(g['betas'][0]), float(g['betas'][1]), float(g['eps']), float(max_norm or 0.0)]

    @torch.no_grad()
    def step(self, closure=None, max_norm=None, hyper_dev=None):
        if closure is not None:
            raise NotImplementedError('closures are not supported')
        ar = self.arena
        ar.check()
        group = self.param_groups[0]
        vmax = self._flat.get('max_exp_avg_sq')
        if hyper_dev is None:
            self._steps += 1
        ar.drop_prefetched()
        with torch.cuda.device(ar.data.device):
            _lib.check(_lib.load().stove_flat_adam(
                ar.data.data_ptr(), ar.grad.data_ptr(), self._flat['exp_avg'].data_ptr(), self._flat['exp_avg_sq'].data_ptr(),
                None if vmax is None else vmax.data_ptr(), ar.numel, self._seg_of4.data_ptr(), self._trainable_dev().data_ptr(),
                self._seg_steps.data_ptr(), len(ar.params), self._ws.data_ptr(), self._norm.data_ptr(),
                None if hyper_dev is None else hyper_dev.data_ptr(), float(group['lr']), float(group['betas'][0]),
                float(group['betas'][1]), float(group['eps']), float(max_norm) if max_norm is not None else 0.0,
                (1 if max_norm is not None else 0) | (2 if self.strict_zero_grad else 0), _lib.stream()), 'stove_flat_adam')
        return self._norm if max_norm is not None else None

    def count_step(self):
        self._steps += 1

    def state_dict(self):
        self._bind()
        return super().state_dict()

    def load_state_dict(self, state_dict):
        super().load_state_dict(state_dict)
        steps = []
        with torch.no_grad():
            for p in self.arena.params:
                st = self.state.get(p, {})
                for k, flat in self._flat.items():
                    view = self.arena.view_of(p, flat)
                    if k in st:
                        view.copy_(st[k])
                    else:
                        view.zero_()
                steps.append(float(st['step']) if 'step' in st else 0.0)
        self._seg_steps.copy_(torch.tensor(steps, dtype=torch.float32))
        self.arena.drop_prefetched()
        self._steps = int(max(steps)) if steps else 0
        self._bind()
```

Before: 9.050 million.

## Fuse SPN bake, dense table, gather, ELBO reduce and Adam tick into fewer launches

Adds fused kernels that merge several small launches. One kernel does the SPN bake, the background dense-table build and the arena gather. The ELBO partial sums and the final reduction now run in one launch, with the last block doing the finish via an atomic ticket. The Adam step-counter tick is folded into the Adam kernel the same way, and a specialised supair state kernel (fwd3) handles o=3. The aim is to cut kernel-launch and dependency overhead in a launch-bound step, at the cost of ticket-based cross-block synchronisation and extra code paths.

```diff
diff --git a/include/stove_hip.h b/include/stove_hip.h
--- a/include/stove_hip.h
+++ b/include/stove_hip.h
@@ -192,11 +192,16 @@
 int stove_supair_state_bwd2(const float* zc, const long long* idx, const unsigned char* hits, const float* zfix, const float* g_zfix,
                             const float* g_zl, const float* g_sl, const float* g_init6, int init_ld, const float* span_low, float* gfix_ws,
                             float* g_codes, int n, int T, int o, int skip, void* stream);
+int stove_supair_state_fwd3(const float* codes, const float* span_low, float* zc, float* pos, long long* idx, float* zfix,
+                            unsigned char* hits, float* zl, float* sl, float* init, int init_ld, const float* lat_noise, int lat_dim,
+                            int n, int T, int skip, int fix, void* stream);
 int stove_zall_fwd(const float* zfix, const float* zs, float* zall, int n, int T, int o, int skip, void* stream);
 int stove_zall_bwd(const float* zfix, const float* zs, const float* g_zall, const float* dz_in, float* g_zfix, float* g_zs, int n, int T, int o,
                    int skip, void* stream);
 int stove_elbo_fwd(const float* zs, const float* mean, const float* std_, const float* zdyn, const float* lik, const float* trans_std16,
                    float* part_ws, float* out3, int n, int T, int o, int skip, void* stream);
+int stove_elbo_fwd2(const float* zs, const float* mean, const float* std_, const float* zdyn, const float* lik, const float* trans_std16,
+                    float* part_ws, unsigned* ticket, float* out3, int n, int T, int o, int skip, void* stream);
 int stove_elbo_bwd(const float* zs, const float* mean, const float* std_, const float* zdyn, const float* trans_std16, const float* g_out,
                    float* g_zs, float* g_mean, float* g_std, float* g_zdyn, float* g_lik, int n, int T, int o, int skip, void* stream);
 
@@ -217,6 +222,8 @@
 int stove_spn_bake_bwd(const float* arena, const StoveSpnArenaPlan* plan, const StoveSpnTableGrads* g, float* grad_arena, void* stream);
 int stove_arena_gather(const float* arena, const int32_t* src, float* image, int n, void* stream);
 int stove_arena_scatter_add(const float* gimage, const int32_t* src, float* grad_arena, int n, void* stream);
+int stove_step_head(const float* arena, const StoveSpnArenaPlan* plan, float* obj_coef, float* obj_wsum, float* obj_wroot, float* bg_coef,
+                    float* bg_wroot, const int32_t* bg_side, float* bg_dense, const int32_t* src, float* image, int n, void* stream);
 
 int stove_sum_chunks(const float* parts, float* out, size_t n, int chunks, void* stream);
 
@@ -248,6 +255,9 @@
 int stove_flat_adam(float* params, const float* grads, float* exp_avg, float* exp_avg_sq, float* max_exp_avg_sq, size_t numel,
                     const int* seg_of4, const unsigned char* seg_trainable, float* seg_steps, int nseg, void* ws, float* grad_norm_out,
                     const float* hyper_dev, float lr, float beta1, float beta2, float eps, float max_norm, int clip, void* stream);
+int stove_flat_adam2(float* params, const float* grads, float* exp_avg, float* exp_avg_sq, float* max_exp_avg_sq, size_t numel,
+                     const int* seg_of4, const unsigned char* seg_trainable, float* seg_steps, int nseg, void* ws, float* grad_norm_out,
+                     const float* hyper_dev, float lr, float beta1, float beta2, float eps, float max_norm, int clip, void* stream);
 
 size_t stove_gemm_bf16_ws_floats(int M, int N, int splitk);
 int stove_gemm_bf16(const float* A, const float* B, const float* bias, const float* add, float* C, int M, int N, int K, int lda, int ldb, int ldc,
diff --git a/stove_amd/_lib.py b/stove_amd/_lib.py
--- a/stove_amd/_lib.py
+++ b/stove_amd/_lib.py
@@ -157,6 +157,30 @@
         fn = getattr(lib, name)
         fn.restype = res
         fn.argtypes = args
+    for name, (res, args) in FUSED_SIG.items():
+        fn = getattr(lib, name, None)
+        if fn is None:
+            if not _settings.LIB_OVERRIDE:
+                raise RuntimeError(f'{LIB_PATH} lacks {name}: rebuild it with `python -m stove_amd.build --force`')
+            continue
+        fn.restype = res
+        fn.argtypes = args
+        _FUSED.add(name)
+
+
+_P, _I, _F, _S = c_void_p, c_int, c_float, c_size_t
+FUSED_SIG = {
+    'stove_step_head': (_I, [_P, POINTER(SpnArenaPlan)] + [_P] * 9 + [_I, _P]),
+    'stove_supair_state_fwd3': (_I, [_P] * 10 + [_I, _P, _I] + [_I] * 4 + [_P]),
+    'stove_elbo_fwd2': (_I, [_P] * 9 + [_I] * 4 + [_P]),
+    'stove_flat_adam2': (_I, [_P] * 5 + [_S, _P, _P, _P, _I, _P, _P, _P, _F, _F, _F, _F, _F, _I, _P]),
+}
+_FUSED = set()
+
+
+def has(name):
+    load()
+    return name in _FUSED
 
 
 def load():
diff --git a/stove_amd/arena.py b/stove_amd/arena.py
--- a/stove_amd/arena.py
+++ b/stove_amd/arena.py
@@ -157,7 +157,11 @@
         side.wait_stream(main)
         with torch.cuda.stream(side):
             pre = {}
-            if self.has_spn:
+            cores = tuple(cores)
+            if self.has_spn and self.has_gnn and cores and _lib.has('stove_step_head'):
+                pre['spn'], pre[('gnn', cores[0])] = self._bake_spn(gather=cores[0])
+                cores = cores[1:]
+            elif self.has_spn:
                 pre['spn'] = self._bake_spn()
             if self.has_gnn:
                 for k in cores:
@@ -186,12 +190,21 @@
         return ((oc.view(24, 25, 10, 3), ow.view(12, 100, 10), orr.view(6, 100), scope, slot),
                 (bc.view(3, 1024, 6, 3), bw.view(3, 36), side, dense))
 
-    def _bake_spn(self):
+    def _bake_spn(self, gather=None):
         lib = _lib.load()
         dev = self.data.device
         with torch.cuda.device(dev):
             buf = torch.empty(18000 + 12000 + 600 + 55296 + 108, dtype=torch.float32, device=dev)
             oc, ow, orr, bc, bw = torch.split(buf, [18000, 12000, 600, 55296, 108])
+            if gather is not None:
+                src = self._gnn[gather][0]
+                dense = torch.empty(lib.stove_bg_dense_floats(), dtype=torch.float32, device=dev)
+                img = torch.empty(src.numel(), dtype=torch.float32, device=dev)
+                _lib.check(lib.stove_step_head(self.data.data_ptr(), ctypes.byref(self._spn['plan']), oc.data_ptr(), ow.data_ptr(),
+                                               orr.data_ptr(), bc.data_ptr(), bw.data_ptr(), self._spn['ints'][2].data_ptr(),
+                                               dense.data_ptr(), src.data_ptr(), img.data_ptr(), src.numel(), _lib.stream()),
+                           'stove_step_head')
+                return (oc, ow, orr, bc, bw, dense), img
             _lib.check(lib.stove_spn_bake(self.data.data_ptr(), ctypes.byref(self._spn['plan']), oc.data_ptr(), ow.data_ptr(),
                                           orr.data_ptr(), bc.data_ptr(), bw.data_ptr(), _lib.stream()), 'stove_spn_bake')
             dense = torch.empty(lib.stove_bg_dense_floats(), dtype=torch.float32, device=dev)
diff --git a/stove_amd/csrc/arena.hip b/stove_amd/csrc/arena.hip
--- a/stove_amd/csrc/arena.hip
+++ b/stove_amd/csrc/arena.hip
@@ -63,9 +63,9 @@
   for (int k = lane; k < n; k += 64) dp[k * ld] += expf(p[k * ld] - m) * inv * (g[k * ld] - dot);
 }
 
-__global__ __launch_bounds__(256) void spn_bake_k(const float* __restrict__ arena, SpnArenaPlan pl, float* __restrict__ obj_coef,
-                                                  float* __restrict__ obj_wsum, float* __restrict__ obj_wroot,
-                                                  float* __restrict__ bg_coef, float* __restrict__ bg_wroot, int n_elem_blocks) {
+__device__ __forceinline__ void spn_bake_block(const float* __restrict__ arena, const SpnArenaPlan& pl, float* __restrict__ obj_coef,
+                                               float* __restrict__ obj_wsum, float* __restrict__ obj_wroot,
+                                               float* __restrict__ bg_coef, float* __restrict__ bg_wroot, int n_elem_blocks) {
   if ((int)blockIdx.x < n_elem_blocks) {
     const int t = blockIdx.x * 256 + threadIdx.x;
     if (t < kAObjCoef) {
@@ -92,6 +92,11 @@
       softmax_col(arena + pl.bg_root, bg_wroot, kABgR * kABgG * kABgG, 1);
     }
   }
+}
+__global__ __launch_bounds__(256) void spn_bake_k(const float* __restrict__ arena, SpnArenaPlan pl, float* __restrict__ obj_coef,
+                                                  float* __restrict__ obj_wsum, float* __restrict__ obj_wroot,
+                                                  float* __restrict__ bg_coef, float* __restrict__ bg_wroot, int n_elem_blocks) {
+  spn_bake_block(arena, pl, obj_coef, obj_wsum, obj_wroot, bg_coef, bg_wroot, n_elem_blocks);
 }
 
 __global__ __launch_bounds__(256) void spn_bake_bwd_k(const float* __restrict__ arena, SpnArenaPlan pl,
@@ -142,6 +147,39 @@
   if (i < n && src[i] >= 0) garena[src[i]] += gimage[i];
 }
 
+__global__ __launch_bounds__(256) void step_head_k(const float* __restrict__ arena, SpnArenaPlan pl, float* __restrict__ obj_coef,
+                                                   float* __restrict__ obj_wsum, float* __restrict__ obj_wroot, float* __restrict__ bg_coef,
+                                                   float* __restrict__ bg_wroot, int n_elem_blocks, int n_bake, const int* __restrict__ side,
+                                                   float* __restrict__ Cf, int n_dense, const int* __restrict__ src, float* __restrict__ image,
+                                                   int n_image) {
+  if ((int)blockIdx.x < n_bake) {
+    spn_bake_block(arena, pl, obj_coef, obj_wsum, obj_wroot, bg_coef, bg_wroot, n_elem_blocks);
+    return;
+  }
+  const int blk = (int)blockIdx.x - n_bake;
+  if (blk < n_dense) {
+    const int idx = blk * 256 + threadIdx.x;
+    if (idx >= kBgDenseF) return;
+    const int m = idx & 3, j = (idx >> 2) & 15, kq = (idx >> 6) & 3, kb = (idx >> 8) & 63, t = (idx >> 14) % 3, feat = idx / (3 << 14);
+    const int p = 16 * kb + 4 * kq + m, col = 16 * t + j;
+    float v = 0.0f;
+    if (col < 36) {
+      const int r = col / 12, sd = (col / 6) & 1, g = col % 6;
+      if ((side[r * kBgPix + p] != 0) == (sd != 0)) {
+        const int gi = pl.bg_gidx[r * kABgPix + p];
+        const int leaf = gi >> 9, row = gi & 511;
+        float abc[3];
+        leaf_coef(arena[pl.bg_mu[leaf] + row * kABgG + g], arena[pl.bg_rho[leaf] + row * kABgG + g], pl.bg_vmin, pl.bg_vmax, abc);
+        v = feat == 0 ? abc[0] : (feat == 1 ? abc[1] : abc[2]);
+      }
+    }
+    Cf[idx] = v;
+    return;
+  }
+  const int i = (blk - n_dense) * 256 + threadIdx.x;
+  if (i < n_image) image[i] = src[i] >= 0 ? arena[src[i]] : 0.0f;
+}
+
 }
 
 namespace stove {
@@ -166,26 +204,10 @@
   if (threadIdx.x == 0) part[blockIdx.x] = (red[0] + red[1]) + (red[2] + red[3]);
 }
 
-__global__ __launch_bounds__(256) void flat_adam_k(float* __restrict__ p, const float* __restrict__ g, float* __restrict__ m, float* __restrict__ v,
-                                                   float* __restrict__ vmax, const int* __restrict__ seg_of4,
-                                                   const unsigned char* __restrict__ trainable, const float* __restrict__ steps,
-                                                   const int* __restrict__ flags, const float* __restrict__ part, float* __restrict__ norm_out,
-                                                   const float* __restrict__ hyper_dev, AdamHyper k, int clip, int n4) {
-  if (hyper_dev != nullptr) {
-    k.lr = hyper_dev[0]; k.b1 = hyper_dev[1]; k.b2 = hyper_dev[2]; k.eps = hyper_dev[3]; k.max_norm = hyper_dev[4];
-  }
-  __shared__ float s_norm;
-  if (threadIdx.x < 64) {
-    float t = (part[threadIdx.x] + part[threadIdx.x + 64]) + (part[threadIdx.x + 128] + part[threadIdx.x + 192]);
-    t = wave_sum(t);
-    if (threadIdx.x == 0) {
-      s_norm = sqrtf(t);
-      if (blockIdx.x == 0 && norm_out != nullptr) norm_out[0] = s_norm;
-    }
-  }
-  __syncthreads();
-  const int i = blockIdx.x * 256 + threadIdx.x;
-  if (i >= n4) return;
+__device__ __forceinline__ void flat_adam_elem(float* __restrict__ p, const float* __restrict__ g, float* __restrict__ m, float* __restrict__ v,
+                                               float* __restrict__ vmax, const int* __restrict__ seg_of4,
+                                               const unsigned char* __restrict__ trainable, const float* steps, const int* flags, float s_norm,
+                                               const AdamHyper& k, int clip, int i) {
   const int seg = seg_of4[i];
   if (trainable[seg] == 0 || flags[seg] == 0) return;
   const float coef = clip ? fminf(1.0f, k.max_norm / (s_norm + 1e-6f)) : 1.0f;
@@ -212,6 +234,65 @@
   if (vmax != nullptr) reinterpret_cast<float4*>(vmax)[i] = x4;
 }
 
+__global__ __launch_bounds__(256) void flat_adam_k(float* __restrict__ p, const float* __restrict__ g, float* __restrict__ m, float* __restrict__ v,
+                                                   float* __restrict__ vmax, const int* __restrict__ seg_of4,
+                                                   const unsigned char* __restrict__ trainable, const float* __restrict__ steps,
+                                                   const int* __restrict__ flags, const float* __restrict__ part, float* __restrict__ norm_out,
+                                                   const float* __restrict__ hyper_dev, AdamHyper k, int clip, int n4) {
+  if (hyper_dev != nullptr) {
+    k.lr = hyper_dev[0]; k.b1 = hyper_dev[1]; k.b2 = hyper_dev[2]; k.eps = hyper_dev[3]; k.max_norm = hyper_dev[4];
+  }
+  __shared__ float s_norm;
+  if (threadIdx.x < 64) {
+    float t = (part[threadIdx.x] + part[threadIdx.x + 64]) + (part[threadIdx.x + 128] + part[threadIdx.x + 192]);
+    t = wave_sum(t);
+    if (threadIdx.x == 0) {
+      s_norm = sqrtf(t);
+      if (blockIdx.x == 0 && norm_out != nullptr) norm_out[0] = s_norm;
+    }
+  }
+  __syncthreads();
+  const int i = blockIdx.x * 256 + threadIdx.x;
+  if (i >= n4) return;
+  flat_adam_elem(p, g, m, v, vmax, seg_of4, trainable, steps, flags, s_norm, k, clip, i);
+}
+
+__global__ __launch_bounds__(256) void flat_adam_tick_k(float* __restrict__ p, const float* __restrict__ g, float* __restrict__ m,
+                                                        float* __restrict__ v, float* __restrict__ vmax, const int* __restrict__ seg_of4,
+                                                        const unsigned char* __restrict__ trainable, float* steps, int* flags,
+                                                        const float* __restrict__ part, float* __restrict__ norm_out,
+                                                        const float* __restrict__ hyper_dev, AdamHyper k, int clip, int n4, int nseg, int sticky,
+                                                        unsigned* ticket) {
+  if (hyper_dev != nullptr) {
+    k.lr = hyper_dev[0]; k.b1 = hyper_dev[1]; k.b2 = hyper_dev[2]; k.eps = hyper_dev[3]; k.max_norm = hyper_dev[4];
+  }
+  __shared__ float s_norm;
+  __shared__ int s_last;
+  if (threadIdx.x < 64) {
+    float t = (part[threadIdx.x] + part[threadIdx.x + 64]) + (part[threadIdx.x + 128] + part[threadIdx.x + 192]);
+    t = wave_sum(t);
+    if (threadIdx.x == 0) {
+      s_norm = sqrtf(t);
+      if (blockIdx.x == 0 && norm_out != nullptr) norm_out[0] = s_norm;
+    }
+  }
+  __syncthreads();
+  const int i = blockIdx.x * 256 + threadIdx.x;
+  if (i < n4) flat_adam_elem(p, g, m, v, vmax, seg_of4, trainable, steps, flags, s_norm, k, clip, i);
+  __syncthreads();
+  if (threadIdx.x == 0) {
+    __threadfence();
+    s_last = atomicAdd(ticket, 1u) == gridDim.x - 1 ? 1 : 0;
+  }
+  __syncthreads();
+  if (!s_last) return;
+  for (int s = threadIdx.x; s < nseg; s += 256) {
+    if (trainable[s] != 0 && flags[s] != 0) steps[s] += 1.0f;
+    if (!sticky) flags[s] = 0;
+  }
+  if (threadIdx.x == 0) *ticket = 0u;
+}
+
 __global__ void adam_tick_k(const unsigned char* __restrict__ trainable, float* __restrict__ steps, int* __restrict__ flags, int nseg, int sticky) {
   const int s = blockIdx.x * blockDim.x + threadIdx.x;
   if (s >= nseg) return;
diff --git a/stove_amd/csrc/capi.hip b/stove_amd/csrc/capi.hip
--- a/stove_amd/csrc/capi.hip
+++ b/stove_amd/csrc/capi.hip
@@ -1107,6 +1107,16 @@
 int stove_arena_gather(const float* arena, const int32_t* src, float* image, int n, void* stream) {
   if (n == 0) return 0;
   STOVE_LAUNCH(arena_gather_k, dim3((n + 255) / 256), dim3(256), 0, (hipStream_t)stream, arena, src, image, n);
+  STOVE_LAUNCH_CHECK();
+  return 0;
+}
+
+int stove_step_head(const float* arena, const StoveSpnArenaPlan* plan, float* obj_coef, float* obj_wsum, float* obj_wroot, float* bg_coef,
+                    float* bg_wroot, const int32_t* bg_side, float* bg_dense, const int32_t* src, float* image, int n, void* stream) {
+  STOVE_VALIDATE(step_head(arena, plan, obj_coef, obj_wsum, obj_wroot, bg_coef, bg_wroot, bg_side, bg_dense, src, image, n));
+  const int nb = (kAObjCoef + kABgCoef + 255) / 256, n_bake = nb + kASoftBlocks, n_dense = (kBgDenseF + 255) / 256;
+  STOVE_LAUNCH(step_head_k, dim3(n_bake + n_dense + (n + 255) / 256), dim3(256), 0, (hipStream_t)stream, arena, arena_plan(plan), obj_coef,
+               obj_wsum, obj_wroot, bg_coef, bg_wroot, nb, n_bake, bg_side, bg_dense, n_dense, src, image, n);
   STOVE_LAUNCH_CHECK();
   return 0;
 }
@@ -1403,7 +1413,7 @@
   return 0;
 }
 
-size_t stove_flat_adam_ws_bytes(int nseg) { return (size_t)nseg * sizeof(int) + ADAM_SCAN_BLOCKS * sizeof(float); }
+size_t stove_flat_adam_ws_bytes(int nseg) { return (size_t)nseg * sizeof(int) + ADAM_SCAN_BLOCKS * sizeof(float) + sizeof(unsigned); }
 
 int stove_flat_adam(float* params, const float* grads, float* exp_avg, float* exp_avg_sq, float* max_exp_avg_sq, size_t numel,
                     const int* seg_of4, const unsigned char* seg_trainable, float* seg_steps, int nseg, void* ws, float* grad_norm_out,
@@ -1425,6 +1435,25 @@
   return 0;
 }
 
+int stove_flat_adam2(float* params, const float* grads, float* exp_avg, float* exp_avg_sq, float* max_exp_avg_sq, size_t numel,
+                     const int* seg_of4, const unsigned char* seg_trainable, float* seg_steps, int nseg, void* ws, float* grad_norm_out,
+                     const float* hyper_dev, float lr, float beta1, float beta2, float eps, float max_norm, int clip, void* stream) {
+  if (numel == 0 || nseg == 0) return 0;
+  STOVE_VALIDATE(flat_adam(params, grads, exp_avg, exp_avg_sq, numel, seg_of4, seg_trainable, seg_steps, nseg, ws));
+  AdamHyper k;
+  k.lr = lr; k.b1 = beta1; k.b2 = beta2; k.eps = eps; k.max_norm = max_norm;
+  const int n4 = (int)(numel / 4);
+  hipStream_t st = (hipStream_t)stream;
+  float* part = reinterpret_cast<float*>(ws);
+  int* flags = reinterpret_cast<int*>(part + ADAM_SCAN_BLOCKS);
+  unsigned* ticket = reinterpret_cast<unsigned*>(flags + nseg);
+  STOVE_LAUNCH(grad_scan_k, dim3(ADAM_SCAN_BLOCKS), dim3(256), 0, st, grads, seg_of4, flags, part, n4);
+  STOVE_LAUNCH(flat_adam_tick_k, dim3((n4 + 255) / 256), dim3(256), 0, st, params, grads, exp_avg, exp_avg_sq, max_exp_avg_sq, seg_of4,
+               seg_trainable, seg_steps, flags, (const float*)part, grad_norm_out, hyper_dev, k, clip & 1, n4, nseg, (clip >> 1) & 1, ticket);
+  STOVE_LAUNCH_CHECK();
+  return 0;
+}
+
 static ZpConst zp_const(const float* span_low) {
   ZpConst k;
   for (int d = 0; d < 8; ++d) {
@@ -1457,6 +1486,18 @@
   }
   STOVE_LAUNCH(supair_state_fwd_k, dim3((M + 255) / 256), dim3(256), 0, st, (const float*)zc, (const long long*)idx, zfix, hits, zl, sl,
                init6, n, T, o, skip, fix, init_ld, lat_noise, lat_dim);
+  STOVE_LAUNCH_CHECK();
+  return 0;
+}
+
+int stove_supair_state_fwd3(const float* codes, const float* span_low, float* zc, float* pos, long long* idx, float* zfix,
+                            unsigned char* hits, float* zl, float* sl, float* init, int init_ld, const float* lat_noise, int lat_dim,
+                            int n, int T, int skip, int fix, void* stream) {
+  STOVE_VALIDATE(supair_state_fwd3(codes, span_low, zc, pos, idx, zfix, hits, zl, sl, init, init_ld, lat_noise, lat_dim, n, T, skip));
+  if (n == 0) return 0;
+  const size_t lds = (size_t)T * 3 * 3 * sizeof(float);
+  STOVE_LAUNCH(supair_state3_fused_k, dim3(n), dim3(256), lds, (hipStream_t)stream, codes, zp_const(span_low), zc, pos, idx, zfix, hits, zl, sl,
+               init, T, skip, fix, init_ld, lat_noise, lat_dim);
   STOVE_LAUNCH_CHECK();
   return 0;
 }
@@ -1521,6 +1562,15 @@
   STOVE_LAUNCH(elbo_part_k, dim3(n), dim3(256), 0, st, zs, mean, std_, zdyn, lik, trans_std(trans_std16), part_ws, T, o, skip);
   STOVE_LAUNCH_CHECK();
   STOVE_LAUNCH(elbo_final_k, dim3(1), dim3(256), 0, st, (const float*)part_ws, out3, n, T, skip);
+  STOVE_LAUNCH_CHECK();
+  return 0;
+}
+
+int stove_elbo_fwd2(const float* zs, const float* mean, const float* std_, const float* zdyn, const float* lik, const float* trans_std16,
+                    float* part_ws, unsigned* ticket, float* out3, int n, int T, int o, int skip, void* stream) {
+  STOVE_VALIDATE(elbo_fwd2(zs, mean, std_, zdyn, lik, trans_std16, part_ws, ticket, out3, n, T, o, skip));
+  STOVE_LAUNCH(elbo_fwd_fused_k, dim3(n), dim3(256), 0, (hipStream_t)stream, zs, mean, std_, zdyn, lik, trans_std(trans_std16), part_ws, ticket,
+               out3, T, o, skip);
   STOVE_LAUNCH_CHECK();
   return 0;
 }
diff --git a/stove_amd/csrc/match.hip b/stove_amd/csrc/match.hip
--- a/stove_amd/csrc/match.hip
+++ b/stove_amd/csrc/match.hip
@@ -332,13 +332,7 @@
 }
 
 template <int F>
-__global__ __launch_bounds__(64) void match3_table_k(const float* __restrict__ feat, long long* __restrict__ idx_out, int B, int T) {
-  extern __shared__ float mlds[];
-  const int b = blockIdx.x, lane = threadIdx.x;
-  const int n_feat = T * 3 * F;
-  int* ibuf = reinterpret_cast<int*>(mlds + n_feat);
-  for (int i = lane; i < n_feat; i += 64) mlds[i] = feat[(size_t)b * n_feat + i];
-  __syncthreads();
+__device__ __forceinline__ void match3_table_wave(const float* mlds, int* ibuf, int T, int lane) {
   const int chunk = (T - 1 + 63) / 64;
   const int t0 = 1 + lane * chunk, t1 = t0 + chunk < T ? t0 + chunk : T;
   auto table = [&](int t, float (&D)[3][3]) {
@@ -398,6 +392,17 @@
     ibuf[t * 3 + 1] = p.p1;
     ibuf[t * 3 + 2] = p.p2;
   }
+}
+
+template <int F>
+__global__ __launch_bounds__(64) void match3_table_k(const float* __restrict__ feat, long long* __restrict__ idx_out, int B, int T) {
+  extern __shared__ float mlds[];
+  const int b = blockIdx.x, lane = threadIdx.x;
+  const int n_feat = T * 3 * F;
+  int* ibuf = reinterpret_cast<int*>(mlds + n_feat);
+  for (int i = lane; i < n_feat; i += 64) mlds[i] = feat[(size_t)b * n_feat + i];
+  __syncthreads();
+  match3_table_wave<F>(mlds, ibuf, T, lane);
   __syncthreads();
   for (int i = lane; i < T * 3; i += 64) idx_out[(size_t)b * T * 3 + i] = ibuf[i];
 }
diff --git a/stove_amd/csrc/state.hip b/stove_amd/csrc/state.hip
--- a/stove_amd/csrc/state.hip
+++ b/stove_amd/csrc/state.hip
@@ -42,12 +42,10 @@
   return hit;
 }
 
-__global__ void supair_state_fwd_k(const float* __restrict__ zc, const long long* __restrict__ idx, float* __restrict__ zfix,
-                                   unsigned char* __restrict__ hits, float* __restrict__ zl, float* __restrict__ sl,
-                                   float* __restrict__ init6, int n, int T, int o, int skip, int fix, int init_ld,
-                                   const float* __restrict__ lat_noise, int lat_dim) {
-  const int i = blockIdx.x * blockDim.x + threadIdx.x;
-  if (i >= n * T * o) return;
+__device__ __forceinline__ void supair_state_fwd_elem(const float* zc, const long long* idx, float* __restrict__ zfix,
+                                                      unsigned char* __restrict__ hits, float* __restrict__ zl, float* __restrict__ sl,
+                                                      float* __restrict__ init6, int i, int T, int o, int skip, int fix, int init_ld,
+                                                      const float* __restrict__ lat_noise, int lat_dim) {
   const int k = i % o, t = (i / o) % T, b = i / (o * T);
   float cur[8], pv[8];
   const int hit = fixed_state(zc, idx, b, t, k, T, o, fix, cur);
@@ -80,6 +78,40 @@
       sl[r + d] = s6[d];
     }
   }
+}
+__global__ void supair_state_fwd_k(const float* __restrict__ zc, const long long* __restrict__ idx, float* __restrict__ zfix,
+                                   unsigned char* __restrict__ hits, float* __restrict__ zl, float* __restrict__ sl,
+                                   float* __restrict__ init6, int n, int T, int o, int skip, int fix, int init_ld,
+                                   const float* __restrict__ lat_noise, int lat_dim) {
+  const int i = blockIdx.x * blockDim.x + threadIdx.x;
+  if (i >= n * T * o) return;
+  supair_state_fwd_elem(zc, idx, zfix, hits, zl, sl, init6, i, T, o, skip, fix, init_ld, lat_noise, lat_dim);
+}
+
+__global__ __launch_bounds__(256) void supair_state3_fused_k(const float* __restrict__ codes, ZpConst kc, float* zc, float* __restrict__ pos,
+                                                             long long* idx, float* __restrict__ zfix, unsigned char* __restrict__ hits,
+                                                             float* __restrict__ zl, float* __restrict__ sl, float* __restrict__ init6, int T,
+                                                             int skip, int fix, int init_ld, const float* __restrict__ lat_noise, int lat_dim) {
+  extern __shared__ float st3_lds[];
+  const int b = blockIdx.x, M = T * 3;
+  int* ibuf = reinterpret_cast<int*>(st3_lds + M * 2);
+  for (int e = threadIdx.x; e < M * 8; e += 256) {
+    const int i = b * M * 8 + e;
+    const int d = i & 7;
+    const float v = fmaf(kc.span[d], sigmoidf_(codes[i]), kc.low[d]);
+    zc[i] = v;
+    if (d == 2 || d == 3) {
+      pos[(i >> 3) * 2 + d - 2] = v;
+      st3_lds[(e >> 3) * 2 + d - 2] = v;
+    }
+  }
+  __syncthreads();
+  if (threadIdx.x < 64) match3_table_wave<2>(st3_lds, ibuf, T, (int)threadIdx.x);
+  __syncthreads();
+  for (int e = threadIdx.x; e < M; e += 256) idx[(size_t)b * M + e] = ibuf[e];
+  __syncthreads();
+  for (int e = threadIdx.x; e < M; e += 256)
+    supair_state_fwd_elem(zc, idx, zfix, hits, zl, sl, init6, b * M + e, T, 3, skip, fix, init_ld, lat_noise, lat_dim);
 }
 
 __device__ __forceinline__ void g6_at(const float* __restrict__ g_zl, const float* __restrict__ g_sl, const float* __restrict__ g_init6,
@@ -250,9 +282,9 @@
 struct TransStd {
   float s[16];
 };
-__global__ __launch_bounds__(256) void elbo_part_k(const float* __restrict__ zs, const float* __restrict__ mean, const float* __restrict__ stdv,
-                                                   const float* __restrict__ zdyn, const float* __restrict__ lik, TransStd ts_,
-                                                   float* __restrict__ part, int T, int o, int skip) {
+__device__ __forceinline__ void elbo_part_block(const float* __restrict__ zs, const float* __restrict__ mean, const float* __restrict__ stdv,
+                                                const float* __restrict__ zdyn, const float* __restrict__ lik, const TransStd& ts_,
+                                                float* part, int T, int o, int skip) {
   const int b = blockIdx.x, Ts = T - skip, rows = Ts * o;
   float tr = 0.0f, lq = 0.0f, lk = 0.0f, ls = 0.0f;
   for (int r = threadIdx.x; r < rows; r += blockDim.x) {
@@ -287,11 +319,18 @@
   __syncthreads();
   if (threadIdx.x < 4) part[b * 4 + threadIdx.x] = (red[threadIdx.x][0] + red[threadIdx.x][1]) + (red[threadIdx.x][2] + red[threadIdx.x][3]);
 }
-__global__ __launch_bounds__(256) void elbo_final_k(const float* __restrict__ part, float* __restrict__ out, int n, int T, int skip) {
+__global__ __launch_bounds__(256) void elbo_part_k(const float* __restrict__ zs, const float* __restrict__ mean, const float* __restrict__ stdv,
+                                                   const float* __restrict__ zdyn, const float* __restrict__ lik, TransStd ts_,
+                                                   float* __restrict__ part, int T, int o, int skip) {
+  elbo_part_block(zs, mean, stdv, zdyn, lik, ts_, part, T, o, skip);
+}
+template <bool DEVICE_LOADS>
+__device__ __forceinline__ void elbo_final_block(const float* part, float* __restrict__ out, int n, int T, int skip) {
   float a[4] = {0, 0, 0, 0};
   for (int b = threadIdx.x; b < n; b += blockDim.x)
 #pragma unroll
-    for (int c = 0; c < 4; ++c) a[c] += part[b * 4 + c];
+    for (int c = 0; c < 4; ++c)
+      a[c] += DEVICE_LOADS ? __hip_atomic_load(part + b * 4 + c, __ATOMIC_RELAXED, __HIP_MEMORY_SCOPE_AGENT) : part[b * 4 + c];
   __shared__ float red[4][4];
 #pragma unroll
   for (int c = 0; c < 4; ++c) {
@@ -308,6 +347,23 @@
     out[1] = s[2] / nt;
     out[2] = s[3] / nt;
   }
+}
+__global__ __launch_bounds__(256) void elbo_final_k(const float* __restrict__ part, float* __restrict__ out, int n, int T, int skip) {
+  elbo_final_block<false>(part, out, n, T, skip);
+}
+__global__ __launch_bounds__(256) void elbo_fwd_fused_k(const float* __restrict__ zs, const float* __restrict__ mean, const float* __restrict__ stdv,
+                                                        const float* __restrict__ zdyn, const float* __restrict__ lik, TransStd ts_, float* part,
+                                                        unsigned* ticket, float* __restrict__ out, int T, int o, int skip) {
+  elbo_part_block(zs, mean, stdv, zdyn, lik, ts_, part, T, o, skip);
+  __shared__ int s_last;
+  __threadfence();
+  __syncthreads();
+  if (threadIdx.x == 0) s_last = atomicAdd(ticket, 1u) == gridDim.x - 1 ? 1 : 0;
+  __syncthreads();
+  if (!s_last) return;
+  __threadfence();
+  elbo_final_block<true>(part, out, (int)gridDim.x, T, skip);
+  if (threadIdx.x == 0) *ticket = 0u;
 }
 __global__ __launch_bounds__(256) void elbo_bwd_k(const float* __restrict__ zs, const float* __restrict__ mean, const float* __restrict__ stdv,
                                                   const float* __restrict__ zdyn, TransStd ts_, const float* __restrict__ gout, float* __restrict__ g_zs,
diff --git a/stove_amd/csrc/validate.h b/stove_amd/csrc/validate.h
--- a/stove_amd/csrc/validate.h
+++ b/stove_amd/csrc/validate.h
@@ -208,4 +208,39 @@
   return 0;
 }
 
-}
+inline int step_head(const float* arena, const StoveSpnArenaPlan* plan, const float* obj_coef, const float* obj_wsum, const float* obj_wroot,
+                     const float* bg_coef, const float* bg_wroot, const int32_t* bg_side, const float* bg_dense, const int32_t* src,
+                     const float* image, int n) {
+  if (n < 0 || plan == nullptr || bg_side == nullptr || null_any(arena, obj_coef, obj_wsum, obj_wroot, bg_coef, bg_wroot, bg_dense))
+    return kStoveInvalidValue;
+  if (null_any(plan->obj_mu, plan->obj_rho, plan->obj_sum, plan->bg_mu, plan->bg_rho, plan->bg_gidx)) return kStoveInvalidValue;
+  if (n > 0 && (src == nullptr || image == nullptr)) return kStoveInvalidValue;
+  return 0;
+}
+inline int supair_state_fwd3(const float* codes, const float* span_low, const float* zc, const float* pos, const long long* idx,
+                             const float* zfix, const unsigned char* hits, const float* zl, const float* sl, const float* init, int init_ld,
+                             const float* lat_noise, int lat_dim, int n, int T, int skip) {
+  if (n < 0 || lat_dim < 0 || init_ld < 6 + (lat_noise != nullptr ? lat_dim : 0)) return kStoveInvalidValue;
+  if (n == 0) return 0;
+  if (T < 2 || skip < 1 || skip >= T || (size_t)T * 9 * sizeof(float) > 64 * 1024) return kStoveInvalidValue;
+  if ((long long)n * T * 24 > 0x7fffffffLL) return kStoveInvalidValue;
+  if (idx == nullptr || hits == nullptr || null_any(codes, span_low, zc, pos, zfix, zl, sl, init)) return kStoveInvalidValue;
+  if (misaligned16(zc)) return kStoveInvalidValue;
+  return 0;
+}
+inline int elbo_fwd2(const float* zs, const float* mean, const float* std_, const float* zdyn, const float* lik, const float* trans_std16,
+                     const float* part_ws, const unsigned* ticket, const float* out3, int n, int T, int o, int skip) {
+  if (n < 1 || o < 1 || skip < 1 || skip >= T) return kStoveInvalidValue;
+  if (ticket == nullptr || null_any(zs, mean, std_, zdyn, lik, trans_std16, part_ws, out3)) return kStoveInvalidValue;
+  return 0;
+}
+inline int flat_adam(const float* params, const float* grads, const float* exp_avg, const float* exp_avg_sq, size_t numel, const int* seg_of4,
+                     const unsigned char* seg_trainable, const float* seg_steps, int nseg, const void* ws) {
+  if (nseg < 0 || numel % 4 != 0 || numel / 4 > 0x7fffffffULL) return kStoveInvalidValue;
+  if (ws == nullptr || seg_of4 == nullptr || seg_trainable == nullptr || null_any(params, grads, exp_avg, exp_avg_sq, seg_steps))
+    return kStoveInvalidValue;
+  if (misaligned16(params) || misaligned16(grads) || misaligned16(exp_avg) || misaligned16(exp_avg_sq)) return kStoveInvalidValue;
+  return 0;
+}
+
+}
diff --git a/stove_amd/ops.py b/stove_amd/ops.py
--- a/stove_amd/ops.py
+++ b/stove_amd/ops.py
@@ -877,9 +877,15 @@
             idx = torch.empty(n, T, o, dtype=torch.int64, device=dev)
             hits = torch.empty(n, T, o, dtype=torch.uint8, device=dev)
             zl, sl, init6 = f(n, Ts, o, 6), f(n, Ts, o, 6), f(n, o, ld)
-            check(lib.stove_supair_state_fwd2(ptr(codes), kc, ptr(zc), ptr(pos), ptr(idx), ptr(zfix), ptr(hits), ptr(zl), ptr(sl),
-                                              ptr(init6), ld, ptr(lat_noise) if lat_noise is not None else None, lat_dim, n, T, o, skip,
-                                              int(bool(fix)), MATCH_MODES[mode], stream()), 'stove_supair_state_fwd2')
+            noise_ptr = ptr(lat_noise) if lat_noise is not None else None
+            if o == 3 and mode == '3_only' and n * T * 24 < 2 ** 31 and T * 36 <= 65536 and _lib.has('stove_supair_state_fwd3'):
+                check(lib.stove_supair_state_fwd3(ptr(codes), kc, ptr(zc), ptr(pos), ptr(idx), ptr(zfix), ptr(hits), ptr(zl), ptr(sl),
+                                                  ptr(init6), ld, noise_ptr, lat_dim, n, T, skip, int(bool(fix)), stream()),
+                      'stove_supair_state_fwd3')
+            else:
+                check(lib.stove_supair_state_fwd2(ptr(codes), kc, ptr(zc), ptr(pos), ptr(idx), ptr(zfix), ptr(hits), ptr(zl), ptr(sl),
+                                                  ptr(init6), ld, noise_ptr, lat_dim, n, T, o, skip,
+                                                  int(bool(fix)), MATCH_MODES[mode], stream()), 'stove_supair_state_fwd2')
         ctx.save_for_backward(zc, idx, hits, zfix)
         ctx.init_ld = ld
         ctx.cfg = (tuple(span_low), n, T, o, skip, codes.shape)
@@ -932,6 +938,20 @@
         return g_zfix, g_zs, None, None, None, None
 
 
+_ELBO_TICKETS = {}
+
+
+def _elbo_ticket(dev):
+    if not _lib.has('stove_elbo_fwd2'):
+        return None
+    t = _ELBO_TICKETS.get(dev)
+    if t is None:
+        if torch.cuda.is_current_stream_capturing():
+            return None
+        t = _ELBO_TICKETS[dev] = torch.zeros(1, dtype=torch.int32, device=dev)
+    return t
+
+
 class _ElboFn(torch.autograd.Function):
 
     @staticmethod
@@ -943,8 +963,13 @@
         with torch.cuda.device(dev):
             part = torch.empty(n * 4, dtype=torch.float32, device=dev)
             out3 = torch.empty(3, dtype=torch.float32, device=dev)
-            check(lib.stove_elbo_fwd(ptr(zs), ptr(mean), ptr(std), ptr(zdyn), ptr(lik), ts, ptr(part), ptr(out3), n, T, o, skip, stream()),
-                  'stove_elbo_fwd')
+            ticket = _elbo_ticket(dev)
+            if ticket is not None:
+                check(lib.stove_elbo_fwd2(ptr(zs), ptr(mean), ptr(std), ptr(zdyn), ptr(lik), ts, ptr(part), ptr(ticket), ptr(out3), n, T, o,
+                                          skip, stream()), 'stove_elbo_fwd2')
+            else:
+                check(lib.stove_elbo_fwd(ptr(zs), ptr(mean), ptr(std), ptr(zdyn), ptr(lik), ts, ptr(part), ptr(out3), n, T, o, skip, stream()),
+                      'stove_elbo_fwd')
         ctx.save_for_backward(zs, mean, std, zdyn)
         ctx.cfg = (tuple(trans_std), n, T, o, skip, lik.shape)
         stats = out3[1:]
diff --git a/stove_amd/optim.py b/stove_amd/optim.py
--- a/stove_amd/optim.py
+++ b/stove_amd/optim.py
@@ -58,13 +58,15 @@
             self._steps += 1
         ar.drop_prefetched()
         with torch.cuda.device(ar.data.device):
-            _lib.check(_lib.load().stove_flat_adam(
+            lib = _lib.load()
+            fn, what = (lib.stove_flat_adam2, 'stove_flat_adam2') if _lib.has('stove_flat_adam2') else (lib.stove_flat_adam, 'stove_flat_adam')
+            _lib.check(fn(
                 ar.data.data_ptr(), ar.grad.data_ptr(), self._flat['exp_avg'].data_ptr(), self._flat['exp_avg_sq'].data_ptr(),
                 None if vmax is None else vmax.data_ptr(), ar.numel, self._seg_of4.data_ptr(), self._trainable_dev().data_ptr(),
                 self._seg_steps.data_ptr(), len(ar.params), self._ws.data_ptr(), self._norm.data_ptr(),
                 None if hyper_dev is None else hyper_dev.data_ptr(), float(group['lr']), float(group['betas'][0]),
                 float(group['betas'][1]), float(group['eps']), float(max_norm) if max_norm is not None else 0.0,
-                (1 if max_norm is not None else 0) | (2 if self.strict_zero_grad else 0), _lib.stream()), 'stove_flat_adam')
+                (1 if max_norm is not None else 0) | (2 if self.strict_zero_grad else 0), _lib.stream()), what)
         return self._norm if max_norm is not None else None
 
     def count_step(self):
```

After: 8.884 million. 0.982x the previous value.
